# ssi-research/FQSS

Measured on AMD Instinct MI355X. Metric: QAT-step samples/sec + SI-SDR, ConvTasNet 2spk 8kHz W8A8, higher is better.
Workload: dtype f32

## Files before the change

fqss_amd/_lib.py:

```python
import ctypes as C
import os

_HERE = os.path.dirname(os.path.abspath(__file__))
SO_PATH = os.environ.get("FQSS_LIB") or os.path.join(_HERE, "csrc", "libfqss_hip.so")

P, I64, I32, F32, F64 = C.c_void_p, C.c_int64, C.c_int, C.c_float, C.c_double

_PROTOS = {
    "fqss_version": [],
    "fqss_last_error": [],
    "fqss_selftest_div": [P, I64, F32, P, P],
    "fqss_actq_fwd": [P, P, P, I64, I64, I64, I64, I64, I32, P, I32, P, P, P, P],
    "fqss_obs_reset": [P, I64, P],
    "fqss_observer_ema": [P, P, P, F64, P],
    "fqss_actq_bwd": [P, P, P, I64, I64, I64, I64, I64, I32, P, I32, P, P, P, P, I64, P],
    "fqss_gluq_fwd": [P, P, I64, I64, I64, I64, I64, I32, P, P, P, P],
    "fqss_gluq_bwd": [P, P, P, I64, I64, I64, I64, I64, I64, I32, P, P, P, P],
    "fqss_actq_bwd_colbias": [P, P, P, I64, I32, I64, I64, I64, I32, P, I32, P, P, P, P, P],
    "fqss_actq2_bwd_colbias": [P, P, P, I64, I32, I64, I64, I64, P, P, P, P, P, P, P, P],
    "fqss_minmax": [P, I64, I64, I64, P, P],
    "fqss_wq_observe": [P, I64, I64, I64, P, P, P],
    "fqss_wq_fwd": [P, P, P, I64, I64, I64, P, P, P],
    "fqss_wq_bwd": [P, P, P, P, P, I64, I64, I64, P, P, I32, P],
    "fqss_gacc_flush": [P, P, P, P, P],
    "fqss_gacc_flush_multi": [P, I32, P],
    "fqss_wq_multi_fwd": [P, I32, I32, P],
    "fqss_wq_multi_bwd": [P, I32, I32, P],
    "fqss_pwconv_fwd": [P, P, P, P, I32, I32, I32, I32, I64, I64, P],
    "fqss_pwconv_fwd_x3": [P, P, P, P, I32, I32, I32, I32, I64, I64, P],
    "fqss_pwconv_fwd_x3s": [P, P, P, P, I32, I32, I32, I32, I64, I64, P],
    "fqss_pwconv_fwd_wq": [P, P, P, P, P, I32, I32, I32, I32, I64, I64, P],
    "fqss_conv1d_s1_fwd": [P, P, P, P, I32, I32, I32, I32, I32, I32, I32, I32, I64, I64, I64, P],
    "fqss_conv1d_s1_bwd_w": [P, P, P, I32, I32, I32, I32, I32, I32, I32, I32, I64, I64, P],
    "fqss_halo_pack": [P, P, I64, I64, I64, I64, I64, I64, I64, I32, I32, I64, I64, P],
    "fqss_phase_pack": [P, P, I64, I64, I64, I64, I64, I64, I64, I32, I32, I32, I64, I64, P],
    "fqss_phase_unpack": [P, P, I64, I64, I64, I64, I64, I64, I64, I32, I32, I32, I64, I64, I64, I32, P, P],
    "fqss_conv2_fwd_wq": [P, P, P, P, P, I32, I32, I32, I32, I32, I32, I32, I32, I64, I64, I64, P],
    "fqss_conv2_fwd_x3s": [P, P, P, P, I32, I32, I32, I32, I32, I32, I32, I32, I64, I64, I64, P],
    "fqss_conv2_bwd_x_wq": [P, P, P, P, I32, I32, I32, I32, I32, I32, I32, I32, I64, I64, I64, P],
    "fqss_conv2_bwd_w": [P, P, P, I32, I32, I32, I32, I32, I32, I32, I32, I64, I64, P],
    "fqss_pwconv_bwd_x": [P, P, P, I32, I32, I32, I32, I64, I64, P],
    "fqss_pwconv_bwd_w": [P, P, P, I32, I32, I32, I32, I64, I64, P],
    "fqss_wq_codes": [P, P, P, P, P, I32, I32, P, P, P],
    "fqss_qpw_fwd": [P, P, P, P, P, P, P, P, I32, I32, I32, I32, I64, I64, P],
    "fqss_qpw_bwd_x": [P, P, P, P, I32, I32, I32, I32, I64, I64, P],
    "fqss_qpw_bwd_x_add": [P, P, P, P, P, I32, I32, I32, I32, I64, I64, I64, P],
    "fqss_qpw_bwd_w": [P, P, P, P, P, I32, I32, I32, I32, I64, I64, P],
    "fqss_qpw_fwdq": [P, P, P, P, P, P, P, P, P, P, I32, P, P, P, P, P, P, P, I32, I32, I32, I32, I32, I64, I64, I64, I64, I64, P, P],
    "fqss_qpw_fwdq_add": [P, P, P, P, P, P, P, P, P, P, P, P, P, P, P, P, I32, I32, I32, I32, I32, I64, I64, I64, I64, I64, P, P, P],
    "fqss_add_chain_ok": [I64, I64, I32, I32],
    "fqss_add_chain_bwd": [P, I32, P, I64, P, I64, P, I64, P, I64, P, P, I64, I64, I32, I64, I64, I64, I64, P],
    "fqss_qpw_stat_slots": [I32, I32],
    "fqss_dwq_stat_slots": [I32, I32],
    "fqss_qpw_fwd2": [P, P, P, P, P, P, P, P, P, P, I32, I32, I32, I32, I32, I64, I64, I64, P],
    "fqss_qpw_bwd_x2": [P, P, P, P, P, I32, I32, I32, I32, I32, I64, I64, I64, P],
    "fqss_qpw_bwd_w2": [P, P, P, P, P, P, I32, I32, I32, I32, I32, I64, I64, I64, P],
    "fqss_qpw_bwd_w_group_ws": [P, I32],
    "fqss_qpw_bwd_w_group": [P, I32, P, I64, P],
    "fqss_decode": [P, P, I64, I64, I64, I64, P, P, P],
    "fqss_gnq_fwd": [P, P, P, P, P, P, P, P, I32, I32, I32, I64, I64, I64, F32, P, P, P, P, I32, P],
    "fqss_gnq_bwd": [P, P, P, P, P, P, P, P, P, P, I32, I32, I32, I64, I64, I64, P, P, P, P, P],
    "fqss_ewq_bwd_p": [P, P, P, P, P, P, F32, P, P, I64, I64, I64, I64, I64, I64, I32, P, P, P, P, I32,
                       P, I64, I32, P, P, P, P, I64, P, I64, I32, P, P, P, P, I64, P],
    "fqss_gnq_bwd_p": [P, P, P, P, P, P, P, P, P, P, I32, I32, I32, I64, I64, I64, P, P, P, P, P, I64, I32, P, P, P, P],
    "fqss_dwq_fwd": [P, P, P, P, P, P, P, I32, I32, I32, I32, I32, I32, I64, I64, I64, I32, P, P, P, P, P],
    "fqss_dwq_bwd_z": [P, P, P, P, P, P, P, I32, I32, I32, I32, I32, I32, I64, I64, I64, I32, P, P, P, P, P, P],
    "fqss_ewq_fwd": [P, P, P, P, P, P, P, F32, P, P, I64, I64, I64, I64, I64, I64, I64, I32, P, P, P, P],
    "fqss_ewq_bwd": [P, P, P, P, P, P, P, F32, P, P, I64, I64, I64, I64, I64, I64, I64, I32, P, P, P, P, P],
    "fqss_dwq_bwd_w": [P, P, P, P, P, I32, I32, I32, I32, I32, I32, I64, I64, P],
    "fqss_mulq_fwd": [P, P, P, P, P, P, P, P, I32, I32, I32, I32, I64, I64, I64, I64, P, P, P],
    "fqss_mulq_bwd": [P, P, P, P, P, P, P, P, P, I32, I32, I32, I32, I64, I64, I64, I64, I64, P, P, P, P, I64, I32, P, P, P, P],
    "fqss_dwq_bwd": [P, P, P, P, P, P, P, P, I32, I32, I32, I32, I32, I32, I64, I64, I64, I32, P, P, P, P, P, P],
    "fqss_dwq_bwd_gn": [P, P, P, P, P, P, P, P, I32, I32, I32, I32, I32, I32, I64, I64, I64, I32, P, P, P, P, P, P, P, P],
    "fqss_gnq_bwd_rows": [P, P, P, P, P, P, P, I32, I32, I32, I64, I64, P, P, P, P, P],
    "fqss_gnq_bwd_apply": [P, P, P, P, P, P, P, P, P, P, I32, I32, I32, I64, I64, I64, P, P, P, P, I64, I32, P, P, P, P],
    "fqss_split3_planes": [P, P, I64, P],
    "fqss_tgemm": [P, P, I32, I32, I32, I32, I64, I32, P, P, P, F32, P, P, I32, P, P, I32, P, P, I64, P, P, I64, P],
    "fqss_tgemm_tiled": [P, P, I32, I32, I32, I32, I64, I32, P, P, P, F32, P, P, I32, P, P, I32, P, P, I64, P, P, I64, P],
    "fqss_tgemm_tiled_ok": [I32, I32, I32],
    "fqss_split3_tiles": [P, P, I32, I32, P],
    "fqss_bn_moments": [P, P, I32, I32, I32, I64, P],
    "fqss_bn_apply": [P, P, P, P, I32, I32, I32, I64, I64, P],
    "fqss_bn_bwd_reduce": [P, P, P, I32, I32, I32, I64, I64, P],
    "fqss_bn_bwd_apply": [P, P, P, P, P, P, I32, I32, I32, I64, I64, I64, P],
    "fqss_tdw": [P, P, P, P, F32, P, P, P, P, P, I32, I32, I32, I32, I32, I32, I64, I64, P],
    "fqss_tstats": [P, I32, I32, I32, I64, P, P],
    "fqss_dwconv_fwd": [P, P, P, P, I32, I32, I32, I32, I32, I32, I64, I64, P],
    "fqss_dwconv_bwd_x": [P, P, P, I32, I32, I32, I32, I32, I32, I64, I64, P],
    "fqss_dwconv_bwd_w": [P, P, P, I32, I32, I32, I32, I32, I32, I64, I64, P],
    "fqss_gn_fwd": [P, P, P, P, P, I32, I32, I32, I64, I64, F32, P, P],
    "fqss_gn_fwd_tail": [P, P, P, P, I32, I32, I32, I64, I64, F32, P, I32, P, P, I64, P],
    "fqss_gn_bwd": [P, P, P, P, P, P, P, I32, I32, I32, I64, I64, I64, P, P],
    "fqss_gnq_fwd_f": [P, P, P, P, P, P, I32, I32, I32, I64, I64, I64, F32, P, P, P, P],
    "fqss_gnq_bwd_f": [P, P, P, P, P, P, P, P, I32, I32, I32, I64, I64, I64, P, P, P, P, P],
    "fqss_axpby": [P, P, F32, F32, P, I64, I64, I64, I64, I64, P],
    "fqss_mul_bcast_fwd": [P, P, P, I32, I32, I32, I32, I64, I64, I64, P],
    "fqss_mul_bcast_bwd": [P, P, P, P, P, I32, I32, I32, I32, I64, I64, I64, I64, I64, P],
    "fqss_splitter2": [P, P, I32, I64, P, P],
    "fqss_splitter2_raw": [P, P, I32, I64, P, P],
    "fqss_frames_conv_fwd": [P, P, P, I32, I32, I32, I64, I32, I32, I32, I64, P],
    "fqss_frames_conv_add_fwd": [P, P, P, I64, P, I32, I32, I32, I64, I32, I32, I32, I64, P],
    "fqss_ola_convtr_fwd": [P, P, P, I32, I32, I32, I64, I32, I32, I64, P],
    "fqss_frames_wgrad1": [P, P, P, I32, I32, I32, I64, I64, I32, I32, P],
    "fqss_frames_wgrad1s": [P, P, I64, P, I64, I32, I32, I32, I64, I64, I32, I32, P],
    "fqss_frames_wgrad1_q": [P, P, P, P, P, I32, I32, I32, I64, I64, I32, I32, P],
    "fqss_ola_convtr_fwd_q": [P, P, P, P, P, I32, I32, I32, I64, I32, I32, I64, P],
    "fqss_ola_convtr_mul_fwd": [P, P, P, P, I32, I32, I32, I32, I64, I64, I32, I32, I64, P],
    "fqss_frames_wgrad": [P, P, P, I32, I32, I32, I32, I64, I64, I32, I32, P],
    "fqss_kd_loss": [P, P, P, I32, I64, F32, P, P, P, P, P, P],
    "fqss_kd_moments": [P, P, P, I32, I64, P, P],
    "fqss_pit_sisdr_loss": [P, P, I32, I64, P, P, P, P, P, P],
    "fqss_kd_loss_per_sample": [P, P, P, I32, I64, F32, I32, F32, P, P, P, P, P, P],
    "fqss_sumsq": [P, I64, P, P],
    "fqss_set_deterministic": [I32, P, I64, P],
    "fqss_det_finish": [P, I64, P, P],
    "fqss_adam_clip": [P, P, P, P, I64, P, F32, F32, F32, F32, F32, F32, P, P, P, P],
    "fqss_rowlin_fwd": [P, P, P, P, I64, I32, I32, I64, I64, I64, P],
    "fqss_rowlin_fwd_w3": [P, P, P, P, I64, I32, I32, I64, I64, P],
    "fqss_rowlin_bwd_x": [P, P, P, I64, I32, I32, I64, I64, I64, P],
    "fqss_rowlin_bwd_w": [P, P, P, I64, I32, I32, I64, I64, I64, P],
    "fqss_rowlin_bwd_w_batched": [P, P, P, I64, I32, I32, I64, I64, I64, I32, I64, I64, I64, P],
    "fqss_colsum": [P, P, I64, I32, I64, P],
    "fqss_layernorm_fwd": [P, P, P, P, P, I64, I32, I64, I64, F64, P],
    "fqss_layernorm_bwd": [P, P, P, P, P, P, P, I64, I32, I64, I64, I64, P],
    "fqss_layernormq_fwd": [P, P, P, P, P, P, I64, I32, I64, I64, I64, F64, P, P, P],
    "fqss_layernormq_bwd": [P, P, P, P, P, P, P, P, I64, I32, I64, I64, I64, P, P, P, P],
    "fqss_unary_fwd": [P, P, I64, I32, F64, P],
    "fqss_unary_rows_fwd": [P, P, I64, I32, I64, I64, I32, F64, P],
    "fqss_unary2_fwd": [P, P, I64, I32, F64, F64, P],
    "fqss_unary_bwd": [P, P, P, I64, I32, F64, P],
    "fqss_permute4": [P, P, I64, I64, I64, I32, I64, I64, I64, P],
    "fqss_permute4_ld": [P, P, I64, I64, I64, I32, I64, I64, I64, I64, P],
    "fqss_dp_segment_fwd": [P, P, I32, I32, I64, I64, I32, I32, P],
    "fqss_dp_segment_bwd": [P, P, I32, I32, I64, I64, I32, I32, P],
    "fqss_dp_merge_fwd": [P, P, P, I32, I32, I32, I32, I32, I64, I64, P],
    "fqss_dp_merge_bwd": [P, P, P, I32, I32, I32, I32, I32, I64, I64, I64, P],
    "fqss_ola2_fwd": [P, P, I64, I64, I64, P],
    "fqss_ola2_bwd": [P, P, I64, I64, I64, P],
    "fqss_attn_fwd": [P, P, P, P, P, I32, I32, I32, I32, I64, I64, I64, I64, P, P, P],
    "fqss_attn_bwd": [P, P, P, P, P, P, P, P, P, I32, I32, I32, I32, I64, I64, I64, I64, I64, I64, I64, I64, P],
    "fqss_add_layernorm_fwd": [P, P, P, P, P, P, P, P, I64, I32, I64, I64, I64, I64, I64, F64, P, P, P],
    "fqss_add_layernorm_bwd": [P, P, P, P, P, P, P, P, P, I64, I32, I64, I64, I64, I64, P, P, P, P],
    "fqss_addq_layernorm_fwd": [P, P, P, P, P, P, P, P, I64, I32, I64, I64, I64, I64, I64, F64, P, P, P, P, P],
    "fqss_addq_layernorm_bwd": [P, P, P, P, P, P, P, P, P, I64, I32, I64, I64, I64, I64, P, P, P, P, P, P, P],
    "fqss_addq_layernorm_fwd_map": [P, P, P, P, P, P, P, P, I64, I32, I64, I64, I64, F64, P, P, P, P, I64, I64, I64, I64, I64, P],
    "fqss_addq_layernorm_bwd_map": [P, P, P, P, P, P, P, P, I64, I32, I64, I64, P, P, P, P, P, P, I64, I64, I64, I64, I64, P],
    "fqss_mha_prep_fwd": [P, P, P, P, I64, I32, I64, F64, P, P],
    "fqss_mha_prep_fwd_c": [P, P, P, P, I64, I32, I64, F64, P, P],
    "fqss_mha_prep_bwd": [P, P, P, P, P, I64, I32, I64, I64, F64, P, P, P],
    "fqss_lstm_fwd": [P, P, P, P, P, P, I32, I32, I32, P],
    "fqss_lstm_bwd": [P, P, P, P, P, I32, I32, I32, P],
    "fqss_lstm_gate_fn": [P, P, P, I64, P],
    "fqss_lstm_bwd_b": [P, P, P, P, P, P, I32, I32, I32, P],
    "fqss_lstm_bwd_b4": [P, P, P, P, P, P, I32, I32, I32, P],
    "fqss_gnrows_fwd": [P, P, P, P, P, P, I64, I32, I64, I64, I32, I32, I32, F64, P],
    "fqss_gnrows_bwd": [P, P, P, P, P, P, P, P, I64, I32, I64, I64, I64, I32, I32, I32, P],
    "fqss_bcast_add": [P, P, P, I64, I64, I32, P],
    "fqss_bcast_sum": [P, P, I64, I64, I32, P],
# ... 184 lines not shown
```

fqss_amd/csrc/desc_api.hip:

```cpp
#include <cstring>

#include "fqss_dev.h"

using namespace fqss;

namespace {

struct Rows {
    void* p;
    int64_t B, C, M, ld;
};

bool rows3(const FqssTensor* t, int dtype, Rows& r, const char*& why) {
    if (t == nullptr || t->data == nullptr) { why = "null tensor"; return false; }
    if (t->dtype != dtype) { why = "wrong dtype"; return false; }
    if (t->ndim < 2 || t->ndim > 3) { why = "tensor must be [B][C][M] or [rows][cols]"; return false; }
    const int n = t->ndim;
    if (t->stride[n - 1] != 1) { why = "innermost stride must be 1"; return false; }
    for (int i = 0; i < n; ++i)
        if (t->shape[i] < 0) { why = "negative extent"; return false; }
    r.p = t->data;
    r.M = t->shape[n - 1];
    r.C = t->shape[n - 2];
    r.B = n == 3 ? t->shape[0] : 1;
// ... 38 lines not shown
}

extern "C" int fqss_add_fq_fwd(const FqssTensor* a, const FqssQParams* qa, const FqssTensor* b, const FqssQParams* qb, float sb,
                               FqssTensor* y, FqssTensor* y_out, const FqssQParams* q, void* ws, size_t ws_bytes,
                               fqss_stream_t stream) {
    (void)ws; (void)ws_bytes;
    FQSS_REQUIRE(qa && q && qa->qmin && qa->qmax && q->qmin && q->qmax, "null quantizer");
    DESC_ROWS(ra, a, FQSS_DT_U8);
    DESC_ROWS(ry, y, FQSS_DT_U8);
    FQSS_REQUIRE(same_shape(ra, ry), "a / y shapes differ");
    Rows rb{}, ro{};
    const bool b_codes = b != nullptr && b->dtype == FQSS_DT_U8;
    if (b != nullptr) {
        DESC_ROWS(rb_, b, b_codes ? FQSS_DT_U8 : FQSS_DT_F32);
        FQSS_REQUIRE(same_shape(ra, rb_), "a / b shapes differ");
        FQSS_REQUIRE(!b_codes || (qb && qb->qmin && qb->qmax), "coded b needs its quantizer");
        rb = rb_;
    }
    if (y_out != nullptr) {
        DESC_ROWS(ro_, y_out, FQSS_DT_F32);
        FQSS_REQUIRE(same_shape(ra, ro_), "a / y_out shapes differ");
        ro = ro_;
    }
    return fqss_ewq_fwd((const uint8_t*)ra.p, qa->qmin, qa->qmax, b_codes ? (const uint8_t*)rb.p : nullptr, b_codes ? qb->qmin : nullptr,
                        b_codes ? qb->qmax : nullptr, (b != nullptr && !b_codes) ? (const float*)rb.p : nullptr, sb, (uint8_t*)ry.p,
                        (float*)ro.p, ra.B * ra.C, ra.M, ra.ld, rb.ld, rb.ld, ry.ld, ro.ld, q->act, q->slope, q->qmin, q->qmax, stream);
}

extern "C" int fqss_add_fq_bwd(const FqssTensor* a, const FqssQParams* qa, const FqssTensor* b, const FqssQParams* qb, float sb,
                               const FqssTensor* g, FqssTensor* gz, const FqssQParams* q, const FqssProducer* pa, const FqssProducer* pb,
                               void* ws, size_t ws_bytes, fqss_stream_t stream) {
    (void)ws; (void)ws_bytes;
    FQSS_REQUIRE(qa && q && qa->qmin && qa->qmax && q->qmin && q->qmax && q->gacc, "null quantizer / gacc");
    DESC_ROWS(ra, a, FQSS_DT_U8);
    DESC_ROWS(rg, g, FQSS_DT_F32);
    FQSS_REQUIRE(same_shape(ra, rg), "a / g shapes differ");
    Rows rb{}, rz{};
    const bool b_codes = b != nullptr && b->dtype == FQSS_DT_U8;
    if (b != nullptr) {
        DESC_ROWS(rb_, b, b_codes ? FQSS_DT_U8 : FQSS_DT_F32);
        FQSS_REQUIRE(same_shape(ra, rb_), "a / b shapes differ");
        FQSS_REQUIRE(!b_codes || (qb && qb->qmin && qb->qmax), "coded b needs its quantizer");
        rb = rb_;
    }
    if (gz != nullptr) {
        DESC_ROWS(rz_, gz, FQSS_DT_F32);
        FQSS_REQUIRE(same_shape(ra, rz_), "a / gz shapes differ");
        rz = rz_;
    }
    if (pa == nullptr && pb == nullptr) {
        FQSS_REQUIRE(gz != nullptr, "gz missing");
        return fqss_ewq_bwd((const uint8_t*)ra.p, qa->qmin, qa->qmax, b_codes ? (const uint8_t*)rb.p : nullptr, b_codes ? qb->qmin : nullptr,
                            b_codes ? qb->qmax : nullptr, (b != nullptr && !b_codes) ? (const float*)rb.p : nullptr, sb, (const float*)rg.p,
                            (float*)rz.p, ra.B * ra.C, ra.M, ra.ld, rb.ld, rb.ld, rg.ld, rz.ld, q->act, q->slope, q->qmin, q->qmax, q->gacc,
                            stream);
    }
    FQSS_REQUIRE(b == nullptr || b_codes, "fused producers need a coded (or absent) b");
    Rows pz[2] = {{}, {}}, po[2] = {{}, {}};
    const FqssProducer* ps[2] = {pa, pb};
    for (int i = 0; i < 2; ++i) {
        if (ps[i] == nullptr) continue;
        FQSS_REQUIRE(ps[i]->gacc != nullptr, "producer gacc missing");
        DESC_ROWS(z_, ps[i]->z, FQSS_DT_F32);
        DESC_ROWS(o_, ps[i]->out, FQSS_DT_F32);
        FQSS_REQUIRE(same_shape(ra, z_) && same_shape(ra, o_), "producer shapes differ from a");
        pz[i] = z_;
        po[i] = o_;
    }
    FQSS_REQUIRE(gz != nullptr || (pa != nullptr && (b == nullptr || pb != nullptr)), "gz may only be NULL when every operand is fused");
    return fqss_ewq_bwd_p((const uint8_t*)ra.p, qa->qmin, qa->qmax, b_codes ? (const uint8_t*)rb.p : nullptr, b_codes ? qb->qmin : nullptr,
                          b_codes ? qb->qmax : nullptr, sb, (const float*)rg.p, (float*)rz.p, ra.B * ra.C, ra.M, ra.ld, rb.ld, rg.ld, rz.ld,
                          q->act, q->slope, q->qmin, q->qmax, q->gacc, (int)ra.C, (const float*)pz[0].p, pz[0].ld, pa ? pa->act : 0,
                          pa ? pa->slope : nullptr, pa ? pa->gacc : nullptr, pa ? pa->gbias : nullptr, (float*)po[0].p, po[0].ld,
                          (const float*)pz[1].p, pz[1].ld, pb ? pb->act : 0, pb ? pb->slope : nullptr, pb ? pb->gacc : nullptr,
                          pb ? pb->gbias : nullptr, (float*)po[1].p, po[1].ld, stream);
}

extern "C" int fqss_pwconv_fq_fwd(const FqssTensor* x, const FqssQParams* qx, const FqssWCodes* w, const float* bias1, const float* bias2,
                                  FqssTensor* z1, FqssTensor* z2, FqssTensor* y1, FqssTensor* y2, const FqssQParams* q1,
                                  const FqssQParams* q2, void* ws, size_t ws_bytes, fqss_stream_t stream) {
    FQSS_REQUIRE(qx && qx->qmin && qx->qmax && q1 && q1->qmin && q1->qmax, "null quantizer");
    FQSS_REQUIRE(w && w->idx && w->dw && w->rw && w->Co > 0 && w->Ci > 0, "null weight codes");
    DESC_ROWS(rx, x, FQSS_DT_U8);
    DESC_ROWS(rz1, z1, FQSS_DT_F32);
    DESC_ROWS(ry1, y1, FQSS_DT_U8);
    FQSS_REQUIRE(rx.C == w->Ci, "x channels != Ci");
    FQSS_REQUIRE(rz1.B == rx.B && rz1.M == rx.M && same_shape(rz1, ry1), "z1 / y1 shapes");
    const int Co1 = (int)rz1.C;
    int Co2 = 0;
    Rows rz2{}, ry2{};
    if (z2 != nullptr || y2 != nullptr) {
        FQSS_REQUIRE(z2 && y2 && q2 && q2->qmin && q2->qmax, "second layer: z2, y2 and q2 all needed");
        DESC_ROWS(rz2_, z2, FQSS_DT_F32);
        DESC_ROWS(ry2_, y2, FQSS_DT_U8);
        FQSS_REQUIRE(rz2_.B == rx.B && rz2_.M == rx.M && same_shape(rz2_, ry2_), "z2 / y2 shapes");
        rz2 = rz2_;
        ry2 = ry2_;
        Co2 = (int)rz2.C;
    }
    FQSS_REQUIRE(Co1 + Co2 == w->Co, "z1 + z2 channels != Co of the weight codes");
    int64_t* stats = nullptr;
    if (ws != nullptr && Co2 == 0) {
        const int64_t need = ws_bytes_of("pwconv_fq_fwd", rx.B, Co1, rx.M);
        if (need > 0) {
            FQSS_REQUIRE((int64_t)ws_bytes >= need, "workspace smaller than fqss_workspace_bytes(\"pwconv_fq_fwd\")");
            stats = (int64_t*)ws;
        }
    }
    return fqss_qpw_fwdq((const uint8_t*)rx.p, w->idx, w->dw, w->rw, bias1, bias2, qx->qmin, qx->qmax, (float*)rz1.p, (float*)rz2.p, q1->act,
                         q1->slope, q1->qmin, q1->qmax, Co2 ? q2->qmin : nullptr, Co2 ? q2->qmax : nullptr, (uint8_t*)ry1.p, (uint8_t*)ry2.p,
                         (int)rx.B, w->Ci, Co1, Co2, (int)rx.M, rx.ld, rz1.ld, rz2.ld, ry1.ld, ry2.ld, stats, stream);
}

extern "C" int fqss_gln_fq_fwd(const FqssTensor* x, const FqssQParams* qx, const float* gamma, const float* beta, float eps, FqssTensor* y,
                               FqssTensor* y_out, float* mean_rstd, const FqssQParams* q, void* ws, size_t ws_bytes, const int64_t* stats,
                               int nslots, fqss_stream_t stream) {
    FQSS_REQUIRE(qx && qx->qmin && qx->qmax && q && q->qmin && q->qmax && gamma && beta && mean_rstd, "null argument");
    DESC_ROWS(rx, x, FQSS_DT_U8);
    DESC_ROWS(ry, y, FQSS_DT_U8);
    FQSS_REQUIRE(same_shape(rx, ry), "x / y shapes differ");
    Rows ro{};
    if (y_out != nullptr) {
        DESC_ROWS(ro_, y_out, FQSS_DT_F32);
        FQSS_REQUIRE(same_shape(rx, ro_), "x / y_out shapes differ");
        ro = ro_;
    }
    if (stats == nullptr)
        FQSS_REQUIRE(ws != nullptr && (int64_t)ws_bytes >= ws_bytes_of("gln_fq_fwd", rx.B, rx.C, rx.M),
                     "workspace smaller than fqss_workspace_bytes(\"gln_fq_fwd\")");
    return fqss_gnq_fwd((const uint8_t*)rx.p, qx->qmin, qx->qmax, gamma, beta, (uint8_t*)ry.p, (float*)ro.p, mean_rstd, (int)rx.B, (int)rx.C,
                        (int)rx.M, rx.ld, ry.ld, ro.ld, eps, q->qmin, q->qmax, ws, stats, nslots, stream);
}

extern "C" int fqss_tgemm_desc(const FqssTGemmDesc* d, fqss_stream_t stream) {
    FQSS_REQUIRE(d && d->planes && d->planes->data && d->planes->dtype == FQSS_DT_U16 && d->planes->ndim == 3 && d->planes->shape[0] == 3,
                 "planes must be a [3][Co][Ci] u16 tensor");
    const int Co = (int)d->planes->shape[1], Ci = (int)d->planes->shape[2];
    FQSS_REQUIRE(d->planes->stride[2] == 1 && d->planes->stride[1] == Ci && d->planes->stride[0] == (int64_t)Co * Ci, "planes must be dense");
    DESC_ROWS(rx, d->x, FQSS_DT_F32);
    FQSS_REQUIRE(rx.C == Ci, "x channels != Ci");
    DESC_ROWS(c1, d->c1, FQSS_DT_F32);
    FQSS_REQUIRE(c1.B == rx.B && c1.M == rx.M && c1.C == (d->M1 < Co ? d->M1 : Co), "c1 shape");
    Rows c2{}, r1{}, r2{};
    if (d->M1 < Co) {
        DESC_ROWS(c2_, d->c2, FQSS_DT_F32);
        FQSS_REQUIRE(c2_.B == rx.B && c2_.M == rx.M && c2_.C == Co - d->M1, "c2 shape");
        c2 = c2_;
    }
    if (d->r1 != nullptr) {
        DESC_ROWS(r1_, d->r1, FQSS_DT_F32);
        FQSS_REQUIRE(same_shape(r1_, c1) && r1_.ld == c1.ld, "r1 must have the layout of c1");
        r1 = r1_;
    }
    if (d->r2 != nullptr) {
        DESC_ROWS(r2_, d->r2, FQSS_DT_F32);
        FQSS_REQUIRE(same_shape(r2_, c2) && r2_.ld == c2.ld, "r2 must have the layout of c2");
        r2 = r2_;
    }
    return fqss_tgemm((const uint16_t*)d->planes->data, (const float*)rx.p, (int)rx.B, Ci, Co, (int)rx.M, rx.ld, d->pro, d->pro_stats,
                      d->pro_gamma, d->pro_beta, d->pro_eps, d->pro_slope, d->bias, d->act, d->slope, d->stats_out, d->M1, (float*)c1.p,
                      (const float*)r1.p, c1.ld, (float*)c2.p, (const float*)r2.p, c2.ld, stream);
}
```

fqss_amd/csrc/fqss_dev.h:

```cpp
#pragma once
#include <hip/hip_runtime.h>
#include <stdint.h>

#include "fqss.h"

namespace fqss {

void set_error(const char* fmt, ...);
int launch_status(const char* what);

#define FQSS_REQUIRE(cond, msg)                          \
    do {                                                 \
        if (!(cond)) {                                   \
            ::fqss::set_error("%s: %s", __func__, msg);  \
            return FQSS_EINVAL;                          \
        }                                                \
    } while (0)

static inline bool aligned16(const void* p) { return (reinterpret_cast<uintptr_t>(p) & 15u) == 0; }
static inline int64_t cdiv(int64_t a, int64_t b) { return (a + b - 1) / b; }

static inline dim3 grid_rows(int64_t rows, int64_t cols, int vec, int64_t max_blocks = 8192) {
    int64_t gx = cdiv(cols, 256 * (int64_t)vec);
    if (gx < 1) gx = 1;
// ... 119 lines not shown
            v[i] = s;
        }
    }
    __syncthreads();
}

template <int N>
__device__ __forceinline__ void block_sum_f32w(const float (&p)[N], float* smem, double (&out)[N]) {
    const int lane = threadIdx.x & 63, w = threadIdx.x >> 6, nw = blockDim.x >> 6;
#pragma unroll
    for (int i = 0; i < N; ++i) {
        const float s = wave_sum63(p[i]);
        if (lane == 63) smem[i * nw + w] = s;
    }
    __syncthreads();
    if (threadIdx.x == 0) {
#pragma unroll
        for (int i = 0; i < N; ++i) {
            double s = (double)smem[i * nw];
            for (int k = 1; k < nw; ++k) s += (double)smem[i * nw + k];
            out[i] = s;
        }
    }
    __syncthreads();
}

struct QRange {
    float lo, delta, inv;
};
__device__ __forceinline__ QRange load_qrange(const float* qmin, const float* qmax) {
    const float lo = *qmin, hi = *qmax;
    QRange r;
    r.lo = lo;
    r.delta = (hi - lo) / 255.0f;
    r.inv = 1.0f / r.delta;
    return r;
}
__device__ __forceinline__ float div_by(float a, float b, float y) {
    const float q = a * y;
    const float r = fmaf(-b, q, a);
    return fmaf(r, y, q);
}
template <typename T>
__device__ __forceinline__ T sgpr(T v) {
    asm("" : "+s"(v));
    return v;
}
__device__ __forceinline__ void store16(float* p, const float4& v) {
    typedef float f32x4s __attribute__((ext_vector_type(4)));
    const f32x4s t = {v.x, v.y, v.z, v.w};
    asm volatile("global_store_dwordx4 %0, %1, off\n\ts_nop 1" : : "v"(p), "v"(t) : "memory");
}
__device__ __forceinline__ float act_neg_scale(int act, float slope) {
    return act == FQSS_ACT_PRELU ? slope : (act == FQSS_ACT_RELU ? 0.0f : 1.0f);
}
__device__ __forceinline__ float act_apply(float z, int act, float slope) {
    return z > 0.0f ? z : act_neg_scale(act, slope) * z;
}
__device__ __forceinline__ float act_bwd(float z, float gt, int act, float slope, bool valid, float& p_slope) {
    const bool neg = !(z > 0.0f);
    p_slope += (act == FQSS_ACT_PRELU && valid && neg) ? z * gt : 0.0f;
    return neg ? act_neg_scale(act, slope) * gt : gt;
}
__device__ __forceinline__ float act_apply_br(float z, int act, float slope) {
    if (act == FQSS_ACT_PRELU) return z > 0.0f ? z : slope * z;
    if (act == FQSS_ACT_RELU) return z > 0.0f ? z : 0.0f;
    return z;
}
__device__ __forceinline__ float act_bwd_br(float z, float gt, int act, float slope, bool valid, float& p_slope) {
    if (act == FQSS_ACT_PRELU) {
        const bool pos = z > 0.0f;
        if (valid && !pos) p_slope += z * gt;
        return pos ? gt : slope * gt;
    }
    if (act == FQSS_ACT_RELU) return (z > 0.0f) ? gt : 0.0f;
    return gt;
}
__device__ __forceinline__ float fq_asym(float t, const QRange& r, float& c, float& u, bool& inr) {
    u = div_by(t - r.lo, r.delta, r.inv);
    const float X = rintf(u);
    inr = (X >= 0.0f) && (X <= 255.0f);
    c = __builtin_amdgcn_fmed3f(X, 0.0f, 255.0f);
    return r.delta * c + r.lo;
}

__device__ __forceinline__ float fq_code(float t, const QRange& r) {
    return __builtin_amdgcn_fmed3f(rintf(div_by(t - r.lo, r.delta, r.inv)), 0.0f, 255.0f);
}
__device__ __forceinline__ unsigned int pack_code(float c, unsigned int byte, unsigned int word) {
    return __builtin_amdgcn_cvt_pk_u8_f32(c, byte, word);
}
__device__ __forceinline__ void code_stats4(unsigned int word, unsigned int& s, unsigned int& ss) {
    s = __builtin_amdgcn_udot4(word, 0x01010101u, s, false);
    ss = __builtin_amdgcn_udot4(word, word, ss, false);
}

#endif

constexpr int kDetSlots = 3;
struct DetCtl { long long* shadow[kDetSlots]; const float* base[kDetSlots]; long long n[kDetSlots]; };
typedef int (*det_setter_t)(const DetCtl*);
void det_register(det_setter_t fn);
#if defined(__HIPCC__) && defined(FQSS_USES_GRAD_ADD)
static __constant__ DetCtl d_det_ctl;
namespace {
struct DetRegistrar {
    DetRegistrar() {
        det_register([](const DetCtl* c) { return (int)hipMemcpyToSymbol(HIP_SYMBOL(d_det_ctl), c, sizeof(DetCtl)); });
    }
} det_registrar_;
}
__device__ __forceinline__ bool det_preload() { return d_det_ctl.shadow[0] != nullptr; }
__device__ __forceinline__ void grad_add(float* addr, float v);
__device__ __forceinline__ void grad_add(float* addr, float v, bool det_on) {
    if (det_on) grad_add(addr, v);
    else atomicAdd(addr, v);
}
__device__ __forceinline__ void grad_add(float* addr, float v) {
    if (d_det_ctl.shadow[0] != nullptr && fabsf(v) < 0x1p33f) {
        const DetCtl c = d_det_ctl;
#pragma unroll
        for (int s = 0; s < kDetSlots; ++s) {
            long long* const sh = c.shadow[s];
            const long long i = addr - c.base[s];
            if (sh != nullptr && (unsigned long long)i < (unsigned long long)c.n[s]) {
                const double dv = (double)v;
                const long long hi = __double2ll_rn(dv * 0x1p30);
                const long long lo = __double2ll_rn((dv - (double)hi * 0x1p-30) * 0x1p80);
                if (hi != 0) atomicAdd(reinterpret_cast<unsigned long long*>(sh + 2 * i), (unsigned long long)hi);
                if (lo != 0) atomicAdd(reinterpret_cast<unsigned long long*>(sh + 2 * i + 1), (unsigned long long)lo);
                return;
            }
        }
    }
    atomicAdd(addr, v);
}
#endif
}
```

fqss_amd/csrc/fused_q.hip:

```cpp
#include <cstdlib>
#include <type_traits>

#define FQSS_USES_GRAD_ADD
#include "fqss_dev.h"

namespace fqss {

constexpr int kGnSlots = 64;
constexpr int kSlots = FQSS_GACC_SLOTS;

__device__ __forceinline__ float dec(unsigned int c, const QRange& r) { return r.delta * (float)c + r.lo; }
__device__ __forceinline__ void dec4(unsigned int w, const QRange& r, float (&v)[4]) {
    v[0] = dec(w & 255u, r);
    v[1] = dec((w >> 8) & 255u, r);
    v[2] = dec((w >> 16) & 255u, r);
    v[3] = dec(w >> 24, r);
}

__global__ __launch_bounds__(256) void k_decode(const uint8_t* __restrict__ c, float* __restrict__ out, int64_t rows,
                                                 int64_t cols, int64_t ld_c, int64_t ld_o, const float* qmin,
                                                 const float* qmax) {
    const QRange r = load_qrange(qmin, qmax);
    const int64_t cstep = (int64_t)gridDim.x * 256 * 4;
    for (int64_t row = blockIdx.y; row < rows; row += gridDim.y)
// ... 85 lines not shown
        const float scale = rstd * gamma[c];
        const float shift = fmaf(-scale, mean, beta[c]);
        for (int c0 = c_first; c0 < M; c0 += cstep) {
            const uint4 v = (c0 == c_first) ? v0 : *reinterpret_cast<const uint4*>(xr + c0);
            const unsigned int w[4] = {v.x, v.y, v.z, v.w};
            unsigned int o[4];
#pragma unroll
            for (int q = 0; q < 4; ++q) {
                float xv[4], cq[4];
                dec4(w[q], rx, xv);
                unsigned int pk = 0;
#pragma unroll
                for (int e = 0; e < 4; ++e) {
                    cq[e] = fq_code(fmaf(xv[e], scale, shift), ry);
                    pk = pack_code(cq[e], e, pk);
                }
                o[q] = pk;
                if (yout != nullptr && c0 + 4 * q < M)
                    *reinterpret_cast<float4*>(yout + (int64_t)row * ld_o + c0 + 4 * q) =
                        make_float4(ry.delta * cq[0] + ry.lo, ry.delta * cq[1] + ry.lo, ry.delta * cq[2] + ry.lo, ry.delta * cq[3] + ry.lo);
            }
            *reinterpret_cast<uint4*>(yc + (int64_t)row * ld_yc + c0) = make_uint4(o[0], o[1], o[2], o[3]);
        }
    }
}

template <int RPW>
__global__ __launch_bounds__(256) void k_gnq_apply_t(const uint8_t* __restrict__ xc, const float* __restrict__ gamma,
                                                      const float* __restrict__ beta, uint8_t* __restrict__ yc,
                                                      float* __restrict__ yout, float* __restrict__ mean_rstd,
                                                      const long long* __restrict__ ws, int nslots, float eps, int B, int C,
                                                      int M, int64_t ld_xc, int64_t ld_yc, int64_t ld_o, const float* qmin_x,
                                                      const float* qmax_x, const float* qmin, const float* qmax) {
    __shared__ long long red[2 * 4];
    __shared__ float mr[2];
    __shared__ __attribute__((aligned(16))) uint8_t tab[RPW][256];
    const QRange rx = load_qrange(qmin_x, qmax_x), ry = load_qrange(qmin, qmax);
    const int row0 = blockIdx.x * RPW;
    const int b = row0 / C, c0 = row0 - b * C;
    const int m_first = threadIdx.x * 16;
    uint4 v0[RPW];
#pragma unroll
    for (int r = 0; r < RPW; ++r) {
        v0[r] = make_uint4(0, 0, 0, 0);
        if (m_first < M) v0[r] = *reinterpret_cast<const uint4*>(xc + (int64_t)(row0 + r) * ld_xc + m_first);
    }
    gnq_sample_stats(ws, nslots, b, (int64_t)C * M, eps, rx, red, mr);
    if (c0 == 0 && threadIdx.x == 0) {
        mean_rstd[2 * b] = mr[0];
        mean_rstd[2 * b + 1] = mr[1];
    }
    const float mean = mr[0], rstd = mr[1];
    const float xt = dec(threadIdx.x, rx);
#pragma unroll
    for (int r = 0; r < RPW; ++r) {
        const float scale = rstd * gamma[c0 + r];
        const float shift = fmaf(-scale, mean, beta[c0 + r]);
        tab[r][threadIdx.x] = (uint8_t)fq_code(fmaf(xt, scale, shift), ry);
    }
    __syncthreads();
#pragma unroll
    for (int r = 0; r < RPW; ++r) {
        const uint8_t* xr = xc + (int64_t)(row0 + r) * ld_xc;
        uint8_t* yr = yc + (int64_t)(row0 + r) * ld_yc;
        for (int m = m_first; m < M; m += 4096) {
            const uint4 v = (m == m_first) ? v0[r] : *reinterpret_cast<const uint4*>(xr + m);
            const unsigned int w[4] = {v.x, v.y, v.z, v.w};
            unsigned int o[4];
#pragma unroll
            for (int q = 0; q < 4; ++q) {
                const unsigned int t0 = tab[r][w[q] & 255u], t1 = tab[r][(w[q] >> 8) & 255u], t2 = tab[r][(w[q] >> 16) & 255u],
                                   t3 = tab[r][w[q] >> 24];
                o[q] = t0 | (t1 << 8) | (t2 << 16) | (t3 << 24);
                if (yout != nullptr && m + 4 * q < M)
                    *reinterpret_cast<float4*>(yout + (int64_t)(row0 + r) * ld_o + m + 4 * q) =
                        make_float4(ry.delta * (float)t0 + ry.lo, ry.delta * (float)t1 + ry.lo, ry.delta * (float)t2 + ry.lo,
                                    ry.delta * (float)t3 + ry.lo);
            }
            *reinterpret_cast<uint4*>(yr + m) = make_uint4(o[0], o[1], o[2], o[3]);
        }
    }
}

__device__ __forceinline__ void gn_coef_from_sums(const double (&sv)[2], float mean, float rstd, int C, int M, double& c2d, double& c3d) {
    const double md = (double)mean, rd = (double)rstd;
    const double inv_n = 1.0 / ((double)C * (double)M);
    c2d = (sv[1] * md - sv[0]) * rd * rd * rd * inv_n;
    c3d = -c2d * md - sv[1] * rd * inv_n;
}

__global__ __launch_bounds__(256) void k_gnq_bwd_rows(const uint8_t* __restrict__ xc, const float* __restrict__ g,
                                                       const float* __restrict__ gamma, const float* __restrict__ beta,
                                                       const float* __restrict__ mean_rstd, int C, int M, int64_t ld_xc,
                                                       int64_t ld_g, double* ws, const float* qmin_x, const float* qmax_x,
                                                       const float* qmin, const float* qmax, double* gacc) {
    __shared__ float redf[4 * 4];
    const QRange rx = load_qrange(qmin_x, qmax_x), ry = load_qrange(qmin, qmax);
    const int b = blockIdx.y, c = blockIdx.x;
    const int64_t row = (int64_t)b * C + c;
    const float mean = mean_rstd[2 * b], rstd = mean_rstd[2 * b + 1];
    const float scale = rstd * gamma[c];
    const float shift = fmaf(-scale, mean, beta[c]);
    const uint8_t* xr = xc + row * ld_xc;
    const float* gr = g + row * ld_g;
    float ds = 0.f, db = 0.f, p_du = 0.f, p_out = 0.f;
    for (int m0 = threadIdx.x * 4; m0 < M; m0 += 4096) {
        unsigned int wq_[4];
        float4 gq[4];
#pragma unroll
        for (int i = 0; i < 4; ++i) {
            const int m = m0 + 1024 * i;
            if (m < M) {
                wq_[i] = *reinterpret_cast<const unsigned int*>(xr + m);
                gq[i] = *reinterpret_cast<const float4*>(gr + m);
            }
        }
#pragma unroll
        for (int i = 0; i < 4; ++i) {
            const int m = m0 + 1024 * i;
            if (m >= M) break;
            const unsigned int w = wq_[i];
            const float gv[4] = {gq[i].x, gq[i].y, gq[i].z, gq[i].w};
#pragma unroll
            for (int e = 0; e < 4; ++e) {
                if (m + e < M) {
                    const float x = dec((w >> (8 * e)) & 255u, rx);
                    const float z = fmaf(x, scale, shift);
                    float cq, u;
                    bool inr;
                    (void)fq_asym(z, ry, cq, u, inr);
                    const float gz = inr ? div_by(gv[e] * ry.delta, ry.delta, ry.inv) : 0.0f;
                    p_du += gv[e] * (inr ? (cq - u) : cq);
                    p_out += inr ? 0.0f : gv[e];
                    ds = fmaf(gz, x, ds);
                    db += gz;
                }
            }
        }
    }
    double v[4];
    {
        const float pf[4] = {ds, db, p_du, p_out};
        block_sum_f32w<4>(pf, redf, v);
    }
    if (threadIdx.x == 0) {
        ws[2 * row] = v[0];
        ws[2 * row + 1] = v[1];
        double* slot = gacc + 3 * (row % kSlots);
        const double dmax = v[2] / 255.0;
        atomicAdd(&slot[0], v[3] - dmax);
        atomicAdd(&slot[1], dmax);
    }
}

struct GnProducer {
    const float* pz; int64_t ld_pz;
    int act; const float* slope;
    const float *qmin, *qmax;
    double* gacc; float* gbias;
};

template <bool FUSE>
__global__ __launch_bounds__(256) void k_gnq_bwd_apply(const uint8_t* __restrict__ xc, const float* __restrict__ g,
                                                        const float* __restrict__ gamma, const float* __restrict__ beta,
                                                        const float* __restrict__ mean_rstd, float* __restrict__ gx, int B,
                                                        int C, int M, int64_t ld_xc, int64_t ld_g, int64_t ld_gx,
                                                        const double* ws, const float* qmin_x, const float* qmax_x,
                                                        const float* qmin, const float* qmax, GnProducer P, float* ggamma,
                                                        float* gbeta) {
    __shared__ float predf[4 * 4];
    const bool det_on = det_preload();
    const QRange rp = FUSE ? load_qrange(P.qmin, P.qmax) : QRange{0.f, 1.f, 1.f};
    const float pslope = (FUSE && P.act == FQSS_ACT_PRELU) ? *P.slope : 0.0f;
    float p_du = 0.f, p_out = 0.f, p_slope = 0.f, p_bias = 0.f;
    const QRange rx = load_qrange(qmin_x, qmax_x), ry = load_qrange(qmin, qmax);
    const int c = blockIdx.x, b = blockIdx.y;
    const int64_t row = (int64_t)b * C + c;
    const float mean = mean_rstd[2 * b], rstd = mean_rstd[2 * b + 1];
    const float scale = rstd * gamma[c];
    const float shift = fmaf(-scale, mean, beta[c]);
    __shared__ double cred[2 * 4];
    __shared__ float c23[2];
    float c2, c3;
    auto gamma_beta_grads = [&]() {
        double gg = 0.0, gb = 0.0;
        for (int bb = 0; bb < B; ++bb) {
            const double ds = ws[2 * ((int64_t)bb * C + c)], db = ws[2 * ((int64_t)bb * C + c) + 1];
            gg += (ds - db * (double)mean_rstd[2 * bb]) * (double)mean_rstd[2 * bb + 1];
            gb += db;
        }
        ggamma[c] += (float)gg;
        gbeta[c] += (float)gb;
    };
    {
        double sv[2] = {0.0, 0.0};
        for (int cc = threadIdx.x; cc < C; cc += 256) {
            const double gmm = (double)gamma[cc];
            sv[0] += gmm * ws[2 * ((int64_t)b * C + cc)];
            sv[1] += gmm * ws[2 * ((int64_t)b * C + cc) + 1];
        }
        block_sum<double, 2>(sv, cred);
        if (threadIdx.x == 0) {
            double c2d, c3d;
            gn_coef_from_sums(sv, mean, rstd, C, M, c2d, c3d);
            c23[0] = (float)c2d;
            c23[1] = (float)c3d;
            if (b == 0) gamma_beta_grads();
        }
        __syncthreads();
        c2 = c23[0];
        c3 = c23[1];
    }
    const uint8_t* xr = xc + row * ld_xc;
    const float* gr = g + row * ld_g;
    const float* pzr = FUSE ? P.pz + row * P.ld_pz : nullptr;
    float* orow = gx + row * ld_gx;
    for (int m0 = threadIdx.x * 4; m0 < M; m0 += 4096) {
        unsigned int wq_[4];
        float4 gq[4], pq[4];
#pragma unroll
        for (int i = 0; i < 4; ++i) {
            const int m = m0 + 1024 * i;
            if (m < M) {
                wq_[i] = *reinterpret_cast<const unsigned int*>(xr + m);
                gq[i] = *reinterpret_cast<const float4*>(gr + m);
                if (FUSE) pq[i] = *reinterpret_cast<const float4*>(pzr + m);
            }
        }
#pragma unroll
        for (int i = 0; i < 4; ++i) {
            const int m = m0 + 1024 * i;
            if (m >= M) break;
            const float gv[4] = {gq[i].x, gq[i].y, gq[i].z, gq[i].w};
            const float pzv[4] = {FUSE ? pq[i].x : 0.f, FUSE ? pq[i].y : 0.f, FUSE ? pq[i].z : 0.f, FUSE ? pq[i].w : 0.f};
            float xv[4], o[4];
            dec4(wq_[i], rx, xv);
#pragma unroll
            for (int e = 0; e < 4; ++e) {
                const float x = xv[e];
                const float z = fmaf(x, scale, shift);
                float cq, u;
                bool inr;
                (void)fq_asym(z, ry, cq, u, inr);
                const float gz = inr ? div_by(gv[e] * ry.delta, ry.delta, ry.inv) : 0.0f;
                o[e] = fmaf(gz, scale, fmaf(x, c2, c3));
                if (FUSE) {
                    const bool valid = (m + e < M);
                    const float gj = valid ? o[e] : 0.0f;
                    const float t = act_apply(pzv[e], P.act, pslope);
                    float pc, pu;
                    bool pin;
                    (void)fq_asym(t, rp, pc, pu, pin);
                    const float gt = pin ? div_by(gj * rp.delta, rp.delta, rp.inv) : 0.0f;
                    p_du += gj * (pin ? (pc - pu) : pc);
                    p_out += pin ? 0.0f : gj;
                    const float gzj = act_bwd(pzv[e], gt, P.act, pslope, valid, p_slope);
                    o[e] = gzj;
                    p_bias += valid ? gzj : 0.0f;
                }
            }
            *reinterpret_cast<float4*>(orow + m) = make_float4(o[0], o[1], o[2], o[3]);
        }
    }
    if (FUSE) {
        double v[4];
        {
            const float pf[4] = {p_du, p_out, p_slope, p_bias};
            block_sum_f32w<4>(pf, predf, v);
        }
        if (threadIdx.x == 0 && P.gbias != nullptr) grad_add(&P.gbias[c], (float)v[3], det_on);
        if (threadIdx.x == 0) {
            double* slot = P.gacc + 3 * (row % kSlots);
            const double dmax = v[0] / 255.0;
            atomicAdd(&slot[0], v[1] - dmax);
            atomicAdd(&slot[1], dmax);
            if (P.act == FQSS_ACT_PRELU) atomicAdd(&slot[2], v[2]);
        }
    }
}

constexpr int kTaps = 8;

__device__ __forceinline__ unsigned int load_codes4(const uint8_t* __restrict__ xr, int s0, int ld) {
    const int a0 = s0 & ~3;
    const unsigned int sh = (unsigned int)(s0 - a0);
    const unsigned int lo = (a0 >= 0 && a0 < ld) ? *reinterpret_cast<const unsigned int*>(xr + a0) : 0u;
    if (sh == 0) return lo;
    const unsigned int hi = (a0 + 4 >= 0 && a0 + 4 < ld) ? *reinterpret_cast<const unsigned int*>(xr + a0 + 4) : 0u;
    return __builtin_amdgcn_alignbyte(hi, lo, sh);
}

__device__ __forceinline__ unsigned int load_codes4_clamped(const uint8_t* __restrict__ xr, int s0, int M) {
    unsigned int w = 0;
#pragma unroll
    for (int j = 0; j < 4; ++j) {
        const int p = min(max(s0 + j, 0), M - 1);
        w |= (unsigned int)xr[p] << (8 * j);
    }
    return w;
}

__device__ __forceinline__ unsigned int load_codes4_unaligned(const uint8_t* __restrict__ p) {
    unsigned int w;
    __builtin_memcpy(&w, p, 4);
    return w;
}

__device__ __forceinline__ void dwq_z4(const uint8_t* __restrict__ xr, int m, int M, int ld_c, const float* wk, int K,
                                        int dil, int pad, float bv, const QRange& rx, float (&z)[4]) {
    float acc[4] = {0.f, 0.f, 0.f, 0.f};
    if (m - pad >= 0 && m + 3 + pad < M) {
#pragma unroll
        for (int k = 0; k < kTaps; ++k) {
            if (k < K) {
                float v[4];
                dec4(load_codes4_unaligned(xr + (m + k * dil - pad)), rx, v);
#pragma unroll
                for (int j = 0; j < 4; ++j) acc[j] = fmaf(wk[k], v[j], acc[j]);
            }
        }
    } else {
        unsigned int wv[kTaps];
#pragma unroll
        for (int k = 0; k < kTaps; ++k)
            if (k < K) wv[k] = load_codes4_clamped(xr, m + k * dil - pad, M);
#pragma unroll
        for (int k = 0; k < kTaps; ++k) {
            if (k < K) {
                const int s0 = m + k * dil - pad;
                float v[4];
#pragma unroll
                for (int j = 0; j < 4; ++j) v[j] = (s0 + j >= 0 && s0 + j < M) ? dec((wv[k] >> (8 * j)) & 255u, rx) : 0.0f;
#pragma unroll
                for (int j = 0; j < 4; ++j) acc[j] = fmaf(wk[k], v[j], acc[j]);
            }
        }
    }
#pragma unroll
    for (int j = 0; j < 4; ++j) z[j] = acc[j] + bv;
}

template <int KT>
__global__ __launch_bounds__(256) void k_dwq_fwd(const uint8_t* __restrict__ xc, const float* __restrict__ w,
// ... 1446 lines not shown
```

fqss_amd/csrc/qgemm.hip:

```cpp
#include <cstdlib>
#include <type_traits>

#define FQSS_USES_GRAD_ADD
#include "fqss_dev.h"

namespace fqss {

typedef float f32x16 __attribute__((ext_vector_type(16)));
typedef __bf16 bf16x8 __attribute__((ext_vector_type(8)));
typedef short s16x4 __attribute__((ext_vector_type(4)));
typedef short s16x8 __attribute__((ext_vector_type(8)));

constexpr int QBM = 128, QBN = 64, QBK = 32;
constexpr int LDK = 40;
constexpr int LDN = 96;
constexpr int LDT = 36;
constexpr int WGRAD_BLOCKS = 256;

__device__ __forceinline__ unsigned short f2bf_trunc(float f) { return (unsigned short)(__float_as_uint(f) >> 16); }
__device__ __forceinline__ float bf_trunc(float f) { return __uint_as_float(__float_as_uint(f) & 0xFFFF0000u); }
__device__ __forceinline__ unsigned int bf_rne_word(float f) {
    const unsigned int u = __float_as_uint(f);
    return u + 0x7FFFu + ((u >> 16) & 1u);
}

__device__ __forceinline__ void split3(float g, unsigned short& b1, unsigned short& b2, unsigned short& b3) {
    const float h1 = bf_trunc(g);
    const float r1 = g - h1;
    const float h2 = bf_trunc(r1);
    const float r2 = r1 - h2;
    b1 = f2bf_trunc(h1);
    b2 = f2bf_trunc(h2);
    b3 = f2bf_trunc(r2);
}

typedef float f32x4 __attribute__((ext_vector_type(4)));
typedef uint32_t u32x4 __attribute__((ext_vector_type(4)));
typedef uint32_t u32x2 __attribute__((ext_vector_type(2)));
struct QStage {
    f32x4 a[4];
    f32x4 b[2];
    u32x2 bq;
    int kch;
};
__device__ __forceinline__ void q_load16(f32x4& d, const void* p) { asm volatile("global_load_dwordx4 %0, %1, off" : "=v"(d) : "v"(p) : "memory"); }
__device__ __forceinline__ void q_load8(u32x2& d, const void* p) { asm volatile("global_load_dwordx2 %0, %1, off" : "=v"(d) : "v"(p) : "memory"); }
template <int MODE, int N>
__device__ __forceinline__ void q_wait(QStage& st) {
    if constexpr (MODE == 0)
        asm volatile("s_waitcnt vmcnt(%2)" : "+v"(st.a[0]), "+v"(st.bq) : "n"(N) : "memory");
    else if constexpr (MODE == 1)
        asm volatile("s_waitcnt vmcnt(%3)" : "+v"(st.a[0]), "+v"(st.b[0]), "+v"(st.b[1]) : "n"(N) : "memory");
    else
        asm volatile("s_waitcnt vmcnt(%6)"
                     : "+v"(st.a[0]), "+v"(st.a[1]), "+v"(st.a[2]), "+v"(st.a[3]), "+v"(st.b[0]), "+v"(st.b[1])
                     : "n"(N)
                     : "memory");
}

__device__ __forceinline__ float dec(unsigned int c, const QRange& r) { return r.delta * (float)c + r.lo; }

struct QGemmArgs {
    const void* A;
    const void* B;
    float* C;
    int M, N, K;
    int64_t lda, ldb, ldc;
    int64_t sAb, sBb, sCb;
    const float* dw;
    const float* rw;
    const float* bias;
    const float* qmin_x;
    const float* qmax_x;
    int ksplit, kchunk;
    int tiles_m, tiles_n, batches;
    int M1;
    float* C2; int64_t ldc2, sC2b;
    const float* bias2;
    const void* A2; int64_t lda2, sA2b;
    int K1;
    const void* B2; int64_t ldb2, sB2b;
    unsigned char* Q1; unsigned char* Q2; int64_t ldq1, ldq2, sQ1b, sQ2b;
    const float *qy_min1, *qy_max1, *qy_min2, *qy_max2;
    int qact; const float* qslope;
    long long* stats;
    const unsigned char* AD1; const unsigned char* AD2; int64_t ldad1, ldad2;
    unsigned char* S1; unsigned char* S2; int64_t lds1, lds2;
    const float *ad_min1, *ad_max1, *ad_min2, *ad_max2;
    const float *s_min1, *s_max1, *s_min2, *s_max2;
    int imp_taps, imp_kw, imp_base, imp_row_step, imp_col_step, imp_cmax;
    float imp_inv_taps, imp_inv_kw;
};

template <int MODE, int GP = 3, bool IMP = false>
__global__ __launch_bounds__(256, 2) void k_qgemm(QGemmArgs g) {
    static_assert(!IMP || MODE == 1 || MODE == 3 || MODE == 4, "implicit convolution: float B operands");
    static_assert(MODE == 0 || MODE == 1 || MODE == 3 || MODE == 4, "unknown q-GEMM mode");
    static_assert(GP == 3 || (GP == 2 && MODE != 0 && MODE != 4), "two gradient pieces: dgrad only");
    constexpr bool ACODES = MODE < 2 || MODE == 4;
    constexpr int WMODE = MODE == 4 ? 1 : MODE;
    constexpr bool SIX = MODE == 3 && GP == 2;
    constexpr int NA = (MODE == 3) ? 3 : 1;
    constexpr int NB = (MODE == 1) ? GP : (MODE == 3 || MODE == 4) ? 3 : 1;
    constexpr int BROWS = QBK, BLD = LDN;
    constexpr int A_BYTES = NA * QBM * LDK * 2, B_BYTES = NB * BROWS * BLD * 2;
    constexpr int T_BYTES = 4 * 32 * LDT * 4;
    constexpr int SMEM = (A_BYTES + B_BYTES > T_BYTES) ? A_BYTES + B_BYTES : T_BYTES;
    __shared__ __attribute__((aligned(16))) unsigned char smem[SMEM];
    typedef unsigned short (*AsT)[QBM][LDK];
    typedef unsigned short (*BsT)[BROWS][BLD];
    AsT As = reinterpret_cast<AsT>(smem);
    BsT Bs = reinterpret_cast<BsT>(smem + A_BYTES);

    const int tid = threadIdx.x, lane = tid & 63;
    const int wave = __builtin_amdgcn_readfirstlane(tid >> 6);
    const int wm = wave >> 1, wn = wave & 1;
    const int lr = lane & 31, lh = lane >> 5;
    int panel, mt;
    if (!xcd_tile(g.tiles_n * g.batches, g.tiles_m, panel, mt)) return;
    const int b = panel / g.tiles_n;
    const int kbeg = 0, kend = g.K;
    const int i0 = mt * QBM, j0 = (panel % g.tiles_n) * QBN;

    f32x16 acc[2];
#pragma unroll
    for (int mi = 0; mi < 2; ++mi)
#pragma unroll
        for (int r = 0; r < 16; ++r) acc[mi][r] = 0.f;

    __shared__ float rowc[3][QBM];
    if constexpr (MODE == 0 || MODE == 3 || MODE == 4) {
        if (tid < QBM) {
            const int row = i0 + tid;
            const bool ok = row < g.M;
            rowc[0][tid] = ((MODE == 0 || MODE == 4) && ok) ? g.dw[row] : 1.0f;
            rowc[1][tid] = (MODE == 0 && ok) ? g.rw[row] : 0.0f;
            rowc[2][tid] = (ok && g.bias != nullptr) ? (row < g.M1 ? g.bias[row] : g.bias2[row - g.M1]) : 0.0f;
        }
    }

    constexpr int NLOADS = (MODE == 0) ? 2 : (WMODE == 1) ? 3 : 6;
    const int a_row = tid >> 1, a_k = (tid & 1) * 16;
    const int bk_row = tid >> 3, bk_n = (tid & 7) * 8;
    const int a_row_c = min(i0 + a_row, g.M - 1);

    __shared__ float dws[(MODE == 1) ? 1024 : 1];
    if constexpr (MODE == 1) {
        for (int k = tid; k < (IMP ? g.K / g.imp_taps : g.K); k += 256) dws[k] = g.dw[k];
    }

    constexpr int BEL = (MODE == 0) ? 1 : 4;
    const char* const gB1 = sgpr((const char*)g.B + (int64_t)b * g.sBb * BEL);
    const char* const gB2 = (MODE == 0) ? gB1 : sgpr((const char*)g.B2 + (int64_t)b * g.sB2b * BEL);
    const int64_t gldb1 = sgpr(g.ldb), gldb2 = (MODE == 0) ? gldb1 : sgpr(g.ldb2);
    auto load_tiles = [&](QStage& st, int k0) {
        if constexpr (ACODES) {
            q_load16(st.a[0], (const signed char*)g.A + (int64_t)a_row_c * g.lda + min(k0 + a_k, g.K - 16));
        } else {
            const float* A = (const float*)g.A + (int64_t)b * g.sAb + (int64_t)a_row_c * g.lda;
#pragma unroll
            for (int q = 0; q < 4; ++q) q_load16(st.a[q], A + min(k0 + a_k + 4 * q, g.K - 4));
        }
        const int kk = min(k0 + bk_row, g.K - 1);
        if constexpr (IMP) {
            int ci = (int)((float)kk * g.imp_inv_taps);
            int t = kk - ci * g.imp_taps;
            if (t < 0) { ci -= 1; t += g.imp_taps; }
            if (t >= g.imp_taps) { ci += 1; t -= g.imp_taps; }
            int th = (int)((float)t * g.imp_inv_kw);
            int tw = t - th * g.imp_kw;
            if (tw < 0) { th -= 1; tw += g.imp_kw; }
            if (tw >= g.imp_kw) { th += 1; tw -= g.imp_kw; }
            st.kch = ci;
            const float* Bp = (const float*)gB1 + (int64_t)ci * gldb1 + (g.imp_base + th * g.imp_row_step + tw * g.imp_col_step);
            const int c0 = min(j0 + bk_n, g.imp_cmax);
            q_load16(st.b[0], Bp + c0);
            q_load16(st.b[1], Bp + c0 + 4);
        } else if constexpr (MODE == 0) {
            const unsigned char* Bp = (const unsigned char*)gB1 + (int64_t)kk * gldb1;
            q_load8(st.bq, Bp + min(j0 + bk_n, (int)gldb1 - 8));
        } else {
            const bool h1 = kk < g.K1;
            const int ldk = (int)(h1 ? gldb1 : gldb2);
            const float* Bp = (const float*)(h1 ? gB1 : gB2) + (int64_t)(h1 ? kk : kk - g.K1) * ldk;
            q_load16(st.b[0], Bp + min(j0 + bk_n, ldk - 4));
            q_load16(st.b[1], Bp + min(j0 + bk_n + 4, ldk - 4));
        }
    };

    auto store_codes = [&](unsigned short* dst, const unsigned int* w, auto nw_tag, bool is_signed, bool zero) {
        constexpr int NW = decltype(nw_tag)::value;
        unsigned int o[2 * NW];
#pragma unroll
        for (int q = 0; q < NW; ++q) {
            float f[4];
#pragma unroll
            for (int e = 0; e < 4; ++e) {
                const unsigned int byte = (w[q] >> (8 * e)) & 0xFFu;
                f[e] = zero ? 0.0f : (is_signed ? (float)(int)(signed char)byte : (float)byte);
            }
            o[2 * q] = __builtin_amdgcn_perm(__float_as_uint(f[1]), __float_as_uint(f[0]), 0x07060302u);
            o[2 * q + 1] = __builtin_amdgcn_perm(__float_as_uint(f[3]), __float_as_uint(f[2]), 0x07060302u);
        }
#pragma unroll
        for (int h = 0; h < NW / 2; ++h)
            *reinterpret_cast<uint4*>(dst + 8 * h) = make_uint4(o[4 * h], o[4 * h + 1], o[4 * h + 2], o[4 * h + 3]);
    };

    auto store_split3 = [&](unsigned short* d1, unsigned short* d2, unsigned short* d3, const f32x4* v, float scale,
                            bool do_scale, bool zero, auto nq_tag) {
        constexpr int NQ = decltype(nq_tag)::value;
        unsigned int o1[2 * NQ], o2[2 * NQ], o3[2 * NQ];
#pragma unroll
        for (int q = 0; q < NQ; ++q) {
            float h0[4], r1[4], r2[4];
#pragma unroll
            for (int e = 0; e < 4; ++e) {
                float t = do_scale ? scale * v[q][e] : v[q][e];
                if (zero) t = 0.0f;
                h0[e] = t;
                r1[e] = t - bf_trunc(t);
                r2[e] = r1[e] - bf_trunc(r1[e]);
// ... 34 lines not shown
        }
        *reinterpret_cast<uint4*>(d1) = make_uint4(o1[0], o1[1], o1[2], o1[3]);
        *reinterpret_cast<uint4*>(d2) = make_uint4(o2[0], o2[1], o2[2], o2[3]);
    };

    auto store_tiles = [&](QStage& st, int k0) {
        q_wait<WMODE, NLOADS>(st);
        const bool kz = (k0 + bk_row) >= g.K;
        if constexpr (ACODES) {
            const unsigned int w[4] = {__float_as_uint(st.a[0][0]), __float_as_uint(st.a[0][1]), __float_as_uint(st.a[0][2]),
                                       __float_as_uint(st.a[0][3])};
            store_codes(&As[0][a_row][a_k], w, std::integral_constant<int, 4>{}, true, false);
        } else {
            store_split3(&As[0][a_row][a_k], &As[1][a_row][a_k], &As[2][a_row][a_k], st.a, 1.0f, false, false,
                         std::integral_constant<int, 4>{});
        }
        if constexpr (MODE == 0) {
            const unsigned int w[2] = {st.bq[0], st.bq[1]};
            store_codes(&Bs[0][bk_row][bk_n], w, std::integral_constant<int, 2>{}, false, kz);
        } else {
            const float sc = (MODE == 1) ? dws[IMP ? st.kch : min(k0 + bk_row, g.K - 1)] : 1.0f;
            if constexpr (NB == 2)
                store_split2(&Bs[0][bk_row][bk_n], &Bs[1][bk_row][bk_n], st.b, sc, kz);
            else
                store_split3(&Bs[0][bk_row][bk_n], &Bs[1][bk_row][bk_n], &Bs[2][bk_row][bk_n], st.b, sc, MODE == 1, kz,
                             std::integral_constant<int, 2>{});
        }
    };

    const int nkt = (kend - kbeg + QBK - 1) / QBK;
    const int gq = lane >> 4, li = lane & 15, tq = li >> 2, tp = li & 3;
    auto compute_tile = [&]() {
#pragma unroll
        for (int ks = 0; ks < 2; ++ks) {
#pragma unroll
            for (int sp = 0; sp < NA * NB; ++sp) {
                const int ia = (NA == 3) ? 2 - (sp / NB) : 0, ib = (NB > 1) ? NB - 1 - (sp % NB) : 0;
                if (SIX && ia + ib >= 3) continue;
                bf16x8 af[2], bfr;
#pragma unroll
                for (int mi = 0; mi < 2; ++mi)
                    af[mi] = *reinterpret_cast<const bf16x8*>(&As[ia][wm * 64 + mi * 32 + lr][ks * 16 + 8 * lh]);
                {
                    const int kr = ks * 16 + 8 * (gq >> 1) + tq;
                    const int nc = wn * 32 + 16 * (gq & 1) + 4 * tp;
                    union { bf16x8 v; s16x4 h[2]; } u;
                    u.h[0] = __builtin_amdgcn_ds_read_tr16_b64_v4i16(
                        (s16x4 __attribute__((address_space(3)))*)(&Bs[ib][kr][nc]));
                    u.h[1] = __builtin_amdgcn_ds_read_tr16_b64_v4i16(
                        (s16x4 __attribute__((address_space(3)))*)(&Bs[ib][kr + 4][nc]));
                    bfr = u.v;
                }
#pragma unroll
                for (int mi = 0; mi < 2; ++mi)
                    acc[mi] = __builtin_amdgcn_mfma_f32_32x32x16_bf16(af[mi], bfr, acc[mi], 0, 0, 0);
            }
        }
    };
    QStage stA, stB;
    __syncthreads();
    load_tiles(stA, 0);
    load_tiles(stB, QBK);
    store_tiles(stA, 0);
    load_tiles(stA, 2 * QBK);
    __syncthreads();
    for (int kt = 0; kt < nkt; kt += 2) {
        compute_tile();
        __syncthreads();
        if (kt + 1 < nkt) {
            store_tiles(stB, (kt + 1) * QBK);
            load_tiles(stB, (kt + 3) * QBK);
            __syncthreads();
            compute_tile();
            __syncthreads();
            if (kt + 2 < nkt) {
                store_tiles(stA, (kt + 2) * QBK);
                load_tiles(stA, (kt + 4) * QBK);
                __syncthreads();
            }
        }
    }
    q_wait<WMODE, 0>(stA);
    q_wait<WMODE, 0>(stB);

    float dx = 0.f, mnx = 0.f;
    if constexpr (MODE == 0) {
        const float lo = *g.qmin_x, hi = *g.qmax_x;
        dx = (hi - lo) / 255.0f;
        mnx = lo;
    }
    float* Cb = g.C + (int64_t)b * g.sCb;
    float* C2b = (g.C2 != nullptr) ? g.C2 + (int64_t)b * g.sC2b : nullptr;
    __shared__ uint32_t Qt[(MODE == 0) ? 4 : 1][32][8];
    const bool quant = (MODE == 0) && g.Q1 != nullptr;
    unsigned int st_s = 0, st_ss = 0;
    QRange ry1{}, ry2{};
    QRange rad1{}, rad2{}, rs1{}, rs2{};
    float qslope = 0.0f;
    if (quant) {
        ry1 = load_qrange(g.qy_min1, g.qy_max1);
        ry2 = (g.Q2 != nullptr) ? load_qrange(g.qy_min2, g.qy_max2) : ry1;
        qslope = (g.qact == FQSS_ACT_PRELU) ? *g.qslope : 0.0f;
        if (g.S1 != nullptr) { rad1 = load_qrange(g.ad_min1, g.ad_max1); rs1 = load_qrange(g.s_min1, g.s_max1); }
        if (g.S2 != nullptr) { rad2 = load_qrange(g.ad_min2, g.ad_max2); rs2 = load_qrange(g.s_min2, g.s_max2); }
    }
    {
        __syncthreads();
        float(*Tt)[LDT] = reinterpret_cast<float(*)[LDT]>(smem + wave * 32 * LDT * 4);
        const bool has_bias = g.bias != nullptr;
        const float qns = act_neg_scale(g.qact, qslope);
        const int c4 = (lane & 7) * 4;
        const int col = j0 + wn * 32 + c4;
        auto tile_epilogue = [&](int mi, auto PER_ROW) {
            const int rowt = i0 + wm * 64 + mi * 32;
            const bool tfirst = rowt < g.M1;
            uint4 ad16 = make_uint4(0u, 0u, 0u, 0u);
            const unsigned char* const adp = (MODE == 0 && quant) ? (tfirst ? g.AD1 : g.AD2) : nullptr;
            if constexpr (MODE == 0) {
                if (adp != nullptr) {
                    const int64_t ldad = tfirst ? g.ldad1 : g.ldad2;
                    const int orow = rowt + (lane >> 1) - (tfirst ? 0 : g.M1), ocol = j0 + wn * 32 + 16 * (lane & 1);
                    const int rows_o = tfirst ? g.M1 : g.M - g.M1;
                    if (rowt + (lane >> 1) < g.M && ocol < ldad)
                        ad16 = *reinterpret_cast<const uint4*>(adp + ((int64_t)b * rows_o + orow) * ldad + ocol);
                }
            }
#pragma unroll
            for (int r = 0; r < 16; ++r) {
                const int rl = (r & 3) + 8 * (r >> 2) + 4 * lh;
                const int rb = wm * 64 + mi * 32 + rl;
                const float S = acc[mi][r];
                float v = S;
                if constexpr (MODE == 0) {
                    v = rowc[0][rb] * (dx * S + mnx * rowc[1][rb]);
                    if (has_bias) v = v + rowc[2][rb];
                } else if constexpr (MODE == 3) {
                    if (has_bias) v = S + rowc[2][rb];
                } else if constexpr (MODE == 4) {
                    v = rowc[0][rb] * S;
                    if (has_bias) v = v + rowc[2][rb];
                }
                Tt[rl][lr] = v;
            }
            const QRange ry = tfirst ? ry1 : ry2;
#pragma unroll
            for (int pass = 0; pass < 4; ++pass) {
                const int rl = pass * 8 + (lane >> 3);
                const int row = rowt + rl;
                float4 t = *reinterpret_cast<const float4*>(&Tt[rl][c4]);
                if constexpr (MODE == 1) {
                    if (C2b != nullptr && row < g.M && col < g.N) {
                        const float4 r = *reinterpret_cast<const float4*>(C2b + (int64_t)row * g.ldc2 + col);
                        t.x += r.x; t.y += r.y; t.z += r.z; t.w += r.w;
                    }
                }
                if (row < g.M && col < g.N) {
                    const bool first = decltype(PER_ROW)::value ? row < g.M1 : tfirst;
                    const int64_t ldc = first ? g.ldc : g.ldc2;
                    float* dst = (first ? Cb + (int64_t)row * ldc : C2b + (int64_t)(row - g.M1) * ldc) + col;
                    if (col + 3 < g.N || col + 3 < ldc) {
                        store16(dst, t);
                    } else {
                        dst[0] = t.x;
                        if (col + 1 < g.N) dst[1] = t.y;
                        if (col + 2 < g.N) dst[2] = t.z;
                    }
                }
                if constexpr (MODE == 0) {
                    if (quant) {
                        const float tv[4] = {t.x, t.y, t.z, t.w};
                        uint32_t pk = 0;
#pragma unroll
                        for (int e = 0; e < 4; ++e) pk = pack_code(fq_code(tv[e] > 0.0f ? tv[e] : qns * tv[e], ry), e, pk);
                        Qt[wave][rl][lane & 7] = pk;
                        if (g.stats != nullptr) {
                            const int nl = g.N - col;
                            const uint32_t live = (row < g.M && nl > 0) ? (nl >= 4 ? 0xFFFFFFFFu : (0xFFFFFFFFu >> (8 * (4 - nl)))) : 0u;
                            code_stats4(pk & live, st_s, st_ss);
                        }
                    }
                }
            }
            if constexpr (MODE == 0) {
                if (quant) {
                    const int rl = lane >> 1, hf = lane & 1;
                    const int qcol = j0 + wn * 32 + 16 * hf;
                    const uint4 c16 = *reinterpret_cast<const uint4*>(&Qt[wave][rl][4 * hf]);
                    const int64_t ldq = tfirst ? g.ldq1 : g.ldq2;
                    if (rowt + rl < g.M && qcol < ldq) {
                        unsigned char* qb = tfirst ? g.Q1 + (int64_t)b * g.sQ1b + (int64_t)(rowt + rl) * ldq
                                                   : g.Q2 + (int64_t)b * g.sQ2b + (int64_t)(rowt + rl - g.M1) * ldq;
                        *reinterpret_cast<uint4*>(qb + qcol) = c16;
                    }
                    if (adp != nullptr) {
                        const QRange ra = tfirst ? rad1 : rad2, rs = tfirst ? rs1 : rs2;
                        const unsigned int wa[4] = {ad16.x, ad16.y, ad16.z, ad16.w}, wy[4] = {c16.x, c16.y, c16.z, c16.w};
                        unsigned int o[4];
#pragma unroll
                        for (int w4 = 0; w4 < 4; ++w4) {
                            unsigned int pk = 0;
#pragma unroll
                            for (int e = 0; e < 4; ++e) {
                                float z = dec((wa[w4] >> (8 * e)) & 255u, ra);
                                z = z + 1.0f * dec((wy[w4] >> (8 * e)) & 255u, ry);
                                pk = pack_code(fq_code(z, rs), e, pk);
                            }
                            o[w4] = pk;
                        }
                        const int64_t lds_ = tfirst ? g.lds1 : g.lds2;
                        const int rows_o = tfirst ? g.M1 : g.M - g.M1;
                        if (rowt + rl < g.M && qcol < lds_) {
                            unsigned char* sb_ = (tfirst ? g.S1 : g.S2) + ((int64_t)b * rows_o + (rowt + rl - (tfirst ? 0 : g.M1))) * lds_;
                            *reinterpret_cast<uint4*>(sb_ + qcol) = make_uint4(o[0], o[1], o[2], o[3]);
                        }
                    }
                }
            }
        };
        if (MODE != 0 || (g.M1 & 31) == 0 || g.M1 >= g.M) {
#pragma unroll
            for (int mi = 0; mi < 2; ++mi) tile_epilogue(mi, std::false_type{});
        } else {
#pragma unroll
            for (int mi = 0; mi < 2; ++mi) tile_epilogue(mi, std::true_type{});
        }
        if constexpr (MODE == 0) {
            if (quant && g.stats != nullptr) {
                __shared__ unsigned int sst[2][4];
                st_s = wave_sum(st_s);
                st_ss = wave_sum(st_ss);
                if (lane == 0) { sst[0][wave] = st_s; sst[1][wave] = st_ss; }
                __syncthreads();
                if (tid == 0) {
                    long long* slot = g.stats + 2 * (((int64_t)b * g.tiles_m + mt) * g.tiles_n + (panel % g.tiles_n));
                    slot[0] = (long long)sst[0][0] + sst[0][1] + sst[0][2] + sst[0][3];
                    slot[1] = (long long)sst[1][0] + sst[1][1] + sst[1][2] + sst[1][3];
                }
            }
        }
    }
}

typedef float f32x4 __attribute__((ext_vector_type(4)));
typedef uint32_t u32x4 __attribute__((ext_vector_type(4)));
__device__ __forceinline__ void wg_load16(f32x4& d, const void* p) {
    asm volatile("global_load_dwordx4 %0, %1, off" : "=v"(d) : "v"(p) : "memory");
}
__device__ __forceinline__ void wg_load16(u32x4& d, const void* p) {
    asm volatile("global_load_dwordx4 %0, %1, off" : "=v"(d) : "v"(p) : "memory");
}

constexpr int W2_TM = 64, W2_TN = 128, W2_TK = 64, W2_LD = 72, W2_RING = 4;
struct W2Stage {
    f32x4 a[2];
    u32x4 b;
};
template <int N>
__device__ __forceinline__ void w2_wait(W2Stage& st) {
    asm volatile("s_waitcnt vmcnt(%3)" : "+v"(st.a[0]), "+v"(st.a[1]), "+v"(st.b) : "n"(N) : "memory");
}

template <int GP>
__global__ __launch_bounds__(512, 1) void k_qwgrad2(QGemmArgs g) {
    __shared__ __attribute__((aligned(16))) unsigned short As[2][GP][W2_TM][W2_LD];
    __shared__ __attribute__((aligned(16))) unsigned short Bs[2][W2_TN][W2_LD];
    __shared__ float rsum[W2_TM];
    const int tid = threadIdx.x, lane = tid & 63;
    const int wave = __builtin_amdgcn_readfirstlane(tid >> 6);
    const int wr = wave >> 2, wc = wave & 3, lr = lane & 31, lh = lane >> 5;
    int slice, t;
    if (!xcd_tile(g.batches * g.ksplit, g.tiles_m * g.tiles_n, slice, t)) return;
    const int b = slice / g.ksplit, ks_id = slice % g.ksplit;
    const int kbeg = ks_id * g.kchunk, kend = min(g.K, kbeg + g.kchunk);
    const int row0 = (t / g.tiles_n) * W2_TM, col0 = (t % g.tiles_n) * W2_TN;
    const int nst = (kend - kbeg + W2_TK - 1) / W2_TK;

    const int ar = tid >> 4, ac = (tid & 15) * 4;
    const int br = tid >> 2, bc = (tid & 3) * 16;
    const float* Ap[2];
    bool aok[2];
#pragma unroll
    for (int i = 0; i < 2; ++i) {
        const int row = row0 + ar + 32 * i;
        aok[i] = row < g.M;
        const int rc = aok[i] ? row : 0;
        Ap[i] = (rc < g.M1) ? (const float*)g.A + (int64_t)b * g.sAb + (int64_t)rc * g.lda
                            : (const float*)g.A2 + (int64_t)b * g.sA2b + (int64_t)(rc - g.M1) * g.lda2;
    }
    const unsigned char* Bp = (const unsigned char*)g.B + (int64_t)b * g.sBb + (int64_t)min(col0 + br, g.N - 1) * g.ldb;
    const int ka_last = (kend - 1) & ~3, kb_last = (kend - 1) & ~15;

    auto load = [&](W2Stage& st, int s) {
        const int k = kbeg + s * W2_TK;
#pragma unroll
        for (int i = 0; i < 2; ++i) wg_load16(st.a[i], Ap[i] + min(k + ac, ka_last));
        wg_load16(st.b, Bp + min(k + bc, kb_last));
    };
    float rs_part[2] = {0.f, 0.f};
    auto convert_store = [&](W2Stage& st, int s) {
        const int buf = s & 1;
        const int k = kbeg + s * W2_TK + ac;
#pragma unroll
        for (int i = 0; i < 2; ++i) {
            float x[4];
#pragma unroll
            for (int e = 0; e < 4; ++e) x[e] = (aok[i] && k + e < kend) ? st.a[i][e] : 0.0f;
            rs_part[i] += (x[0] + x[1]) + (x[2] + x[3]);
            uint32_t o1[2], o2[2], o3[2];
#pragma unroll
            for (int e = 0; e < 2; ++e) {
                const float a0 = x[2 * e], a1 = x[2 * e + 1];
                const float r0 = a0 - bf_trunc(a0), r1 = a1 - bf_trunc(a1);
                o1[e] = __builtin_amdgcn_perm(__float_as_uint(a1), __float_as_uint(a0), 0x07060302u);
                if constexpr (GP == 3) {
                    const float s0 = r0 - bf_trunc(r0), s1 = r1 - bf_trunc(r1);
                    o2[e] = __builtin_amdgcn_perm(__float_as_uint(r1), __float_as_uint(r0), 0x07060302u);
                    o3[e] = __builtin_amdgcn_perm(__float_as_uint(s1), __float_as_uint(s0), 0x07060302u);
                } else {
                    o2[e] = __builtin_amdgcn_perm(bf_rne_word(r1), bf_rne_word(r0), 0x07060302u);
                }
            }
            const int row = ar + 32 * i;
// ... 316 lines not shown
        asm volatile("s_waitcnt vmcnt(0)" ::: "memory");
    }
    __syncthreads();
}

template <int GP>
__global__ __launch_bounds__(512, 1) void k_qwgrad_group(WGroupArgs ga) {
    __shared__ __attribute__((aligned(16))) unsigned short As_raw[2 * GP * W2_TM * W2_LD];
    __shared__ __attribute__((aligned(16))) unsigned short Bs_raw[2 * 256 * W2_LD];
    __shared__ float rsum[W2_TM];
    __shared__ unsigned ticket_s;
    const int L = blockIdx.x, xcd = L % kXcds, slot = L / kXcds;
    const int team = (slot / WGR_TEAM) * kXcds + xcd, member = slot % WGR_TEAM;
    int u0 = team * ga.chunk;
    const int u1 = min(ga.total, u0 + ga.chunk);
    while (u0 < u1) {
        int jn = 0;
        for (int q = 1; q < ga.njobs; ++q) jn = (ga.j[q].ubeg <= u0) ? q : jn;
        const WJob& J = ga.j[jn];
        const int rel = u0 - J.ubeg, grp = rel / J.nstages, s0 = rel - grp * J.nstages;
        const int n = min(J.nstages - s0, u1 - u0);
        const int g0 = J.ubeg + grp * J.nstages;
        const int t_first = g0 / ga.chunk, nparts = (g0 + J.nstages - 1) / ga.chunk - t_first + 1, part = team - t_first;
        u0 += n;
        const int tile = grp * WGR_TEAM + member;
        if (tile >= J.ntiles) continue;
        if (J.wide) wgr_segment<GP, true>(ga, J, tile, s0, n, nparts, part, As_raw, Bs_raw, rsum, &ticket_s);
        else wgr_segment<GP, false>(ga, J, tile, s0, n, nparts, part, As_raw, Bs_raw, rsum, &ticket_s);
    }
}

__global__ __launch_bounds__(256) void k_wq_codes(const float* __restrict__ w, signed char* __restrict__ idx,
                                                   signed char* __restrict__ idxT, float* dw, float* rw, int Co, int Ci,
                                                   const float* __restrict__ qmin, const float* __restrict__ qmax) {
    __shared__ float red[4];
    const int co = blockIdx.x;
    const float a = fmaxf(fabsf(qmin[co]), fabsf(qmax[co]));
    const float delta = (2.0f * a) / 255.0f;
    float s = 0.0f;
    for (int ci = threadIdx.x; ci < Ci; ci += 256) {
        const float X = rintf(w[(int64_t)co * Ci + ci] / delta);
        const float q = fminf(fmaxf(X, -128.0f), 127.0f);
        idx[(int64_t)co * Ci + ci] = (signed char)q;
        idxT[(int64_t)ci * Co + co] = (signed char)q;
        s += q;
    }
    float v[1] = {s};
    block_sum<float, 1>(v, red);
    if (threadIdx.x == 0) {
        dw[co] = delta;
        rw[co] = v[0];
    }
}

}

using namespace fqss;

static int grad_pieces() {
    const char* e = getenv("FQSS_GRAD_PIECES");
    return (e != nullptr && e[0] == '2') ? 2 : 3;
}

extern "C" int fqss_wq_codes(const float* w, int8_t* idx, int8_t* idxT, float* dw, float* rw, int Co, int Ci,
                             const float* qmin, const float* qmax, fqss_stream_t stream) {
    FQSS_REQUIRE(w && idx && idxT && dw && rw && qmin && qmax && Co > 0 && Ci > 0, "bad args");
    hipLaunchKernelGGL(k_wq_codes, dim3((unsigned)Co), dim3(256), 0, (hipStream_t)stream, w, (signed char*)idx,
                       (signed char*)idxT, dw, rw, Co, Ci, qmin, qmax);
    return launch_status("fqss_wq_codes");
}

struct QpwQuant {
    int act; const float* slope; const float *min1, *max1, *min2, *max2; uint8_t *yc1, *yc2; int64_t ld1, ld2;
    long long* stats;
    const FqssAddAfter *add1, *add2;
};

static int qpw_fwd_impl(const char* who, const uint8_t* xc, const int8_t* wi, const float* dw, const float* rw, const float* bias1,
                        const float* bias2, const float* qmin_x, const float* qmax_x, float* z1, float* z2, int B, int Ci, int Co1,
                        int Co2, int M, int64_t ld_xc, int64_t ld_z1, int64_t ld_z2, fqss_stream_t stream,
                        const QpwQuant* qq = nullptr) {
    if (B == 0 || M == 0) return FQSS_OK;
    const int Co = Co1 + Co2;
    FQSS_REQUIRE(xc && wi && dw && rw && qmin_x && qmax_x && z1 && (Co2 == 0 || z2), "null tensor");
    FQSS_REQUIRE(B >= 0 && Ci > 0 && Co1 > 0 && Co2 >= 0 && M >= 0 && ld_xc >= M && ld_z1 >= M && (Co2 == 0 || ld_z2 >= M), "bad shape");
    FQSS_REQUIRE(Ci % 16 == 0 && Ci <= 512 && ld_xc % 16 == 0 && aligned16(xc) && aligned16(wi),
                 "q-GEMM needs Ci % 16 == 0, Ci <= 512 (exact fp32 integer sum) and 16-B aligned code rows");
    FQSS_REQUIRE(aligned16(z1) && ld_z1 % 4 == 0 && (Co2 == 0 || (aligned16(z2) && ld_z2 % 4 == 0)), "output rows must be 16-B aligned");
    FQSS_REQUIRE((bias1 == nullptr) == (bias2 == nullptr) || Co2 == 0, "paired layers: both or neither with bias");
    if (qq != nullptr) FQSS_REQUIRE(Co2 == 0 || Co1 % 32 == 0, "fused quantizer of a pair needs Co1 % 32 == 0");
    QGemmArgs g{};
    g.A = wi; g.B = xc; g.C = z1; g.M = Co; g.N = M; g.K = Ci;
    g.lda = Ci; g.ldb = ld_xc; g.ldc = ld_z1;
    g.sAb = 0; g.sBb = (int64_t)Ci * ld_xc; g.sCb = (int64_t)Co1 * ld_z1;
    g.M1 = Co1; g.C2 = z2; g.ldc2 = ld_z2; g.sC2b = (int64_t)Co2 * ld_z2; g.bias2 = bias2; g.K1 = Ci;
    g.dw = dw; g.rw = rw; g.bias = bias1; g.qmin_x = qmin_x; g.qmax_x = qmax_x; g.ksplit = 1; g.kchunk = Ci;
    if (qq != nullptr) {
        FQSS_REQUIRE(qq->min1 && qq->max1 && qq->yc1 && (Co2 == 0 || (qq->min2 && qq->max2 && qq->yc2)), "fused quantizer: null pointer");
        FQSS_REQUIRE(qq->ld1 % 16 == 0 && qq->ld1 >= M && aligned16(qq->yc1) && (Co2 == 0 || (qq->ld2 % 16 == 0 && qq->ld2 >= M && aligned16(qq->yc2))),
                     "output code rows must be 16-B aligned");
        FQSS_REQUIRE(qq->act != FQSS_ACT_PRELU || qq->slope, "PReLU needs a slope");
        g.Q1 = qq->yc1; g.Q2 = qq->yc2; g.ldq1 = qq->ld1; g.ldq2 = qq->ld2;
        g.sQ1b = (int64_t)Co1 * qq->ld1; g.sQ2b = (int64_t)Co2 * qq->ld2;
        g.qy_min1 = qq->min1; g.qy_max1 = qq->max1; g.qy_min2 = qq->min2; g.qy_max2 = qq->max2;
        g.qact = qq->act; g.qslope = qq->slope;
        FQSS_REQUIRE(!qq->stats || Co2 == 0, "output statistics: single-output launches only");
        g.stats = qq->stats;
        const FqssAddAfter* ad[2] = {qq->add1, qq->add2};
        for (int i = 0; i < 2; ++i) {
            const FqssAddAfter* a = ad[i];
            if (a == nullptr) continue;
            FQSS_REQUIRE(i == 0 || Co2 > 0, "fused AddQ behind a second output that does not exist");
            FQSS_REQUIRE(qq->act == FQSS_ACT_NONE, "fused AddQ: the conv in front of it has no activation (Conv1dQ)");
            FQSS_REQUIRE(a->a && a->y && a->amin && a->amax && a->qmin && a->qmax, "fused AddQ: null pointer");
            FQSS_REQUIRE(a->ld_a % 16 == 0 && a->ld_a >= M && a->ld_y % 16 == 0 && a->ld_y >= M && aligned16(a->a) && aligned16(a->y),
                         "fused AddQ: code rows must be 16-B aligned");
            if (i == 0) {
                g.AD1 = a->a; g.ldad1 = a->ld_a; g.S1 = a->y; g.lds1 = a->ld_y;
                g.ad_min1 = a->amin; g.ad_max1 = a->amax; g.s_min1 = a->qmin; g.s_max1 = a->qmax;
            } else {
                g.AD2 = a->a; g.ldad2 = a->ld_a; g.S2 = a->y; g.lds2 = a->ld_y;
                g.ad_min2 = a->amin; g.ad_max2 = a->amax; g.s_min2 = a->qmin; g.s_max2 = a->qmax;
            }
        }
    }
    g.tiles_n = (int)cdiv(M, QBN); g.tiles_m = (int)cdiv(Co, QBM); g.batches = B;
    hipLaunchKernelGGL((k_qgemm<0>), dim3(xcd_grid((int64_t)g.tiles_n * B, g.tiles_m)), dim3(256), 0, (hipStream_t)stream, g);
    return launch_status(who);
}

extern "C" int fqss_qpw_fwd(const uint8_t* xc, const int8_t* wi, const float* dw, const float* rw, const float* bias,
                            const float* qmin_x, const float* qmax_x, float* z, int B, int Ci, int Co, int M,
                            int64_t ld_xc, int64_t ld_z, fqss_stream_t stream) {
    return qpw_fwd_impl("fqss_qpw_fwd", xc, wi, dw, rw, bias, nullptr, qmin_x, qmax_x, z, nullptr, B, Ci, Co, 0, M, ld_xc, ld_z, 0, stream);
}

extern "C" int fqss_qpw_fwd2(const uint8_t* xc, const int8_t* wi, const float* dw, const float* rw, const float* bias1,
                             const float* bias2, const float* qmin_x, const float* qmax_x, float* z1, float* z2, int B, int Ci,
                             int Co1, int Co2, int M, int64_t ld_xc, int64_t ld_z1, int64_t ld_z2, fqss_stream_t stream) {
    FQSS_REQUIRE(Co2 > 0, "second layer missing");
    return qpw_fwd_impl("fqss_qpw_fwd2", xc, wi, dw, rw, bias1, bias2, qmin_x, qmax_x, z1, z2, B, Ci, Co1, Co2, M, ld_xc, ld_z1, ld_z2, stream);
}

extern "C" int fqss_qpw_fwdq(const uint8_t* xc, const int8_t* wi, const float* dw, const float* rw, const float* bias1,
                             const float* bias2, const float* qmin_x, const float* qmax_x, float* z1, float* z2, int act,
                             const float* slope, const float* qmin1, const float* qmax1, const float* qmin2, const float* qmax2,
                             uint8_t* yc1, uint8_t* yc2, int B, int Ci, int Co1, int Co2, int M, int64_t ld_xc, int64_t ld_z1,
                             int64_t ld_z2, int64_t ld_yc1, int64_t ld_yc2, int64_t* stats1, fqss_stream_t stream) {
    QpwQuant qq{act, slope, qmin1, qmax1, qmin2, qmax2, yc1, yc2, ld_yc1, ld_yc2, (long long*)stats1, nullptr, nullptr};
    return qpw_fwd_impl("fqss_qpw_fwdq", xc, wi, dw, rw, bias1, bias2, qmin_x, qmax_x, z1, z2, B, Ci, Co1, Co2, M, ld_xc, ld_z1, ld_z2,
                        stream, &qq);
}

extern "C" int fqss_qpw_fwdq_add(const uint8_t* xc, const int8_t* wi, const float* dw, const float* rw, const float* bias1,
                                 const float* bias2, const float* qmin_x, const float* qmax_x, float* z1, float* z2, const float* qmin1,
                                 const float* qmax1, const float* qmin2, const float* qmax2, uint8_t* yc1, uint8_t* yc2, int B, int Ci,
                                 int Co1, int Co2, int M, int64_t ld_xc, int64_t ld_z1, int64_t ld_z2, int64_t ld_yc1, int64_t ld_yc2,
                                 const FqssAddAfter* add1, const FqssAddAfter* add2, fqss_stream_t stream) {
    QpwQuant qq{FQSS_ACT_NONE, nullptr, qmin1, qmax1, qmin2, qmax2, yc1, yc2, ld_yc1, ld_yc2, nullptr, add1, add2};
    return qpw_fwd_impl("fqss_qpw_fwdq_add", xc, wi, dw, rw, bias1, bias2, qmin_x, qmax_x, z1, z2, B, Ci, Co1, Co2, M, ld_xc, ld_z1,
                        ld_z2, stream, &qq);
}

static int qpw_bwd_x_impl(const char* who, const float* gz1, const float* gz2, const int8_t* wiT, const float* dw, float* gx, int B,
                          int Ci, int Co1, int Co2, int M, int64_t ld_gz1, int64_t ld_gz2, int64_t ld_gx, fqss_stream_t stream,
                          const float* addend = nullptr, int64_t ld_add = 0) {
    if (B == 0 || M == 0) return FQSS_OK;
    const int Co = Co1 + Co2;
    FQSS_REQUIRE(gz1 && wiT && dw && gx && (Co2 == 0 || gz2), "null tensor");
    FQSS_REQUIRE(B >= 0 && Ci > 0 && Co1 > 0 && Co2 >= 0 && M >= 0 && ld_gz1 >= M && ld_gx >= M, "bad shape");
    FQSS_REQUIRE(Co1 % 16 == 0 && Co2 % 16 == 0 && ld_gz1 % 4 == 0 && aligned16(gz1) && aligned16(wiT) && ld_gz1 >= ((M + 3) & ~3),
                 "q-GEMM dgrad needs Co % 16 == 0 and 16-B aligned gradient rows");
    FQSS_REQUIRE(Co2 == 0 || (ld_gz2 % 4 == 0 && aligned16(gz2) && ld_gz2 >= ((M + 3) & ~3)), "second gradient: 16-B aligned rows");
    FQSS_REQUIRE(aligned16(gx) && ld_gx % 4 == 0, "output rows must be 16-B aligned");
    FQSS_REQUIRE(Co <= 1024, "dgrad stages delta_w of at most 1024 output channels in LDS");
    if (B == 0 || M == 0) return FQSS_OK;
    QGemmArgs g{};
    g.A = wiT; g.B = gz1; g.C = gx; g.M = Ci; g.N = M; g.K = Co;
    g.lda = Co; g.ldb = ld_gz1; g.ldc = ld_gx;
    g.sAb = 0; g.sBb = (int64_t)Co1 * ld_gz1; g.sCb = (int64_t)Ci * ld_gx;
    g.M1 = Ci; g.K1 = Co1; g.B2 = gz2; g.ldb2 = ld_gz2; g.sB2b = (int64_t)Co2 * ld_gz2;
    g.dw = dw; g.ksplit = 1; g.kchunk = Co;
    if (addend != nullptr) {
        FQSS_REQUIRE(aligned16(addend) && ld_add % 4 == 0 && ld_add >= ((M + 3) & ~3), "addend rows must be 16-B aligned and padded to 4");
        g.C2 = const_cast<float*>(addend); g.ldc2 = ld_add; g.sC2b = (int64_t)Ci * ld_add;
    }
    g.tiles_n = (int)cdiv(M, QBN); g.tiles_m = (int)cdiv(Ci, QBM); g.batches = B;
    if (grad_pieces() == 3)
        hipLaunchKernelGGL((k_qgemm<1, 3>), dim3(xcd_grid((int64_t)g.tiles_n * B, g.tiles_m)), dim3(256), 0, (hipStream_t)stream, g);
    else
        hipLaunchKernelGGL((k_qgemm<1, 2>), dim3(xcd_grid((int64_t)g.tiles_n * B, g.tiles_m)), dim3(256), 0, (hipStream_t)stream, g);
    return launch_status(who);
}

extern "C" int fqss_qpw_bwd_x(const float* gz, const int8_t* wiT, const float* dw, float* gx, int B, int Ci, int Co,
                              int M, int64_t ld_gz, int64_t ld_gx, fqss_stream_t stream) {
    return qpw_bwd_x_impl("fqss_qpw_bwd_x", gz, nullptr, wiT, dw, gx, B, Ci, Co, 0, M, ld_gz, 0, ld_gx, stream);
}

extern "C" int fqss_qpw_bwd_x_add(const float* gz, const int8_t* wiT, const float* dw, const float* addend, float* gx, int B, int Ci, int Co,
                                  int M, int64_t ld_gz, int64_t ld_add, int64_t ld_gx, fqss_stream_t stream) {
    FQSS_REQUIRE(addend, "null addend");
    return qpw_bwd_x_impl("fqss_qpw_bwd_x_add", gz, nullptr, wiT, dw, gx, B, Ci, Co, 0, M, ld_gz, 0, ld_gx, stream, addend, ld_add);
}

extern "C" int fqss_qpw_bwd_x2(const float* gz1, const float* gz2, const int8_t* wiT, const float* dw, float* gx, int B, int Ci,
                               int Co1, int Co2, int M, int64_t ld_gz1, int64_t ld_gz2, int64_t ld_gx, fqss_stream_t stream) {
    FQSS_REQUIRE(Co2 > 0, "second layer missing");
    return qpw_bwd_x_impl("fqss_qpw_bwd_x2", gz1, gz2, wiT, dw, gx, B, Ci, Co1, Co2, M, ld_gz1, ld_gz2, ld_gx, stream);
}

static int qpw_bwd_w_impl(const char* who, const float* gz1, const float* gz2, const uint8_t* xc, const float* qmin_x,
                          const float* qmax_x, float* gw, int B, int Ci, int Co1, int Co2, int M, int64_t ld_gz1, int64_t ld_gz2,
                          int64_t ld_xc, fqss_stream_t stream) {
    if (B == 0 || M == 0) return FQSS_OK;
    const int Co = Co1 + Co2;
    FQSS_REQUIRE(gz1 && xc && qmin_x && qmax_x && gw && (Co2 == 0 || gz2), "null tensor");
    FQSS_REQUIRE(B >= 0 && Ci > 0 && Co1 > 0 && Co2 >= 0 && M >= 0 && ld_gz1 >= M && ld_xc >= M, "bad shape");
    FQSS_REQUIRE(ld_gz1 % 4 == 0 && ld_xc % 16 == 0 && aligned16(gz1) && aligned16(xc) && ld_gz1 >= ((M + 3) & ~3),
                 "q-GEMM wgrad needs 16-B aligned gradient and code rows");
    FQSS_REQUIRE(Co2 == 0 || (ld_gz2 % 4 == 0 && aligned16(gz2) && ld_gz2 >= ((M + 3) & ~3)), "second gradient: 16-B aligned rows");
    if (B == 0 || M == 0) return FQSS_OK;
    QGemmArgs g{};
    g.A = gz1; g.B = xc; g.C = gw; g.M = Co; g.N = Ci; g.K = M;
    g.lda = ld_gz1; g.ldb = ld_xc; g.ldc = Ci;
    g.sAb = (int64_t)Co1 * ld_gz1; g.sBb = (int64_t)Ci * ld_xc; g.sCb = 0;
    g.M1 = Co1; g.A2 = gz2; g.lda2 = ld_gz2; g.sA2b = (int64_t)Co2 * ld_gz2; g.K1 = M;
    g.qmin_x = qmin_x; g.qmax_x = qmax_x;
    const int64_t tiles = cdiv(Co, 64) * cdiv(Ci, 128) * B;
    int want = (int)((WGRAD_BLOCKS + tiles / 2) / tiles);
    if (want < 1) want = 1;
    g.tiles_n = (int)cdiv(Ci, 128); g.tiles_m = (int)cdiv(Co, 64); g.batches = B;
    const int kchunk = (int)cdiv(cdiv(M, want), W2_RING * W2_TK) * W2_RING * W2_TK;
    g.kchunk = kchunk;
    g.ksplit = (int)cdiv(M, kchunk);
    if (grad_pieces() == 3)
        hipLaunchKernelGGL(k_qwgrad2<3>, dim3(xcd_grid((int64_t)B * g.ksplit, (int64_t)g.tiles_m * g.tiles_n)), dim3(512), 0, (hipStream_t)stream, g);
    else
        hipLaunchKernelGGL(k_qwgrad2<2>, dim3(xcd_grid((int64_t)B * g.ksplit, (int64_t)g.tiles_m * g.tiles_n)), dim3(512), 0, (hipStream_t)stream, g);
    return launch_status(who);
}

extern "C" int fqss_qpw_bwd_w(const float* gz, const uint8_t* xc, const float* qmin_x, const float* qmax_x, float* gw,
                              int B, int Ci, int Co, int M, int64_t ld_gz, int64_t ld_xc, fqss_stream_t stream) {
    return qpw_bwd_w_impl("fqss_qpw_bwd_w", gz, nullptr, xc, qmin_x, qmax_x, gw, B, Ci, Co, 0, M, ld_gz, 0, ld_xc, stream);
}
// ... 190 lines not shown
```

fqss_amd/kernels.py:

```python
import os

import torch

from . import _lib

Q_BYPASS, Q_OBSERVE, Q_QUANT = 0, 1, 2
ACT_NONE, ACT_PRELU, ACT_RELU = 0, 1, 2
ACT_GELU = 3
ACT_POST_RELU = 4

GACC_DOUBLES = 2048 * 3
USE_X3 = True
LD_ALIGN = 16


def _p(t):
    return None if t is None else t.data_ptr()


import ctypes as _C

DESC_ABI = os.environ.get("FQSS_FLAT_ABI", "0") == "0"
_DT = {torch.float32: _lib.DT_F32, torch.uint8: _lib.DT_U8, torch.int8: _lib.DT_I8, torch.float64: _lib.DT_F64, torch.int16: _lib.DT_U16,
       torch.int64: _lib.DT_I64}
# ... 322 lines not shown
    gz, B, Co, M, ld_gz = _bcm(gz)
    gx = empty_act((B, Ci, M), gz.device)
    _lib.call("fqss_pwconv_bwd_x", _p(gz), _p(w), _p(gx), B, Ci, Co, M, ld_gz, rowmat(gx)[2], _stream())
    return gx


def pwconv_bwd_w(gz, x, gw):
    _need_gpu(gz, x, gw)
    gz, B, Co, M, ld_gz = _bcm(gz)
    x, _, Ci, _, ld_x = _bcm(x)
    assert gw.is_contiguous() and gw.numel() == Co * Ci
    _lib.call("fqss_pwconv_bwd_w", _p(gz), _p(x), _p(gw), B, Ci, Co, M, ld_gz, ld_x, _stream())


class WCodes:
    __slots__ = ("idx", "idxT", "dw", "rw", "Co", "Ci")


def wq_codes(w, qmin, qmax):
    _need_gpu(w, qmin, qmax)
    Co, Ci = w.shape[0], w.shape[1]
    assert w.numel() == Co * Ci and w.is_contiguous()
    c = WCodes()
    c.Co, c.Ci = Co, Ci
    c.idx = torch.empty(Co, Ci, device=w.device, dtype=torch.int8)
    c.idxT = torch.empty(Ci, Co, device=w.device, dtype=torch.int8)
    c.dw = torch.empty(Co, device=w.device, dtype=torch.float32)
    c.rw = torch.empty(Co, device=w.device, dtype=torch.float32)
    _lib.call("fqss_wq_codes", _p(w), _p(c.idx), _p(c.idxT), _p(c.dw), _p(c.rw), Co, Ci, _p(qmin), _p(qmax), _stream())
    return c


def q_eligible(Ci, Co):
    return _lib.BACKEND != "cpu" and Ci % 16 == 0 and Co % 16 == 0 and Ci <= 512


def qpw_fwd(xc, wc, bias, qmin_x, qmax_x):
    B, Ci, M = xc.shape
    rm = rowmat(xc)
    assert rm is not None and rm[2] % 16 == 0
    z = empty_act((B, wc.Co, M), xc.device)
    _lib.call("fqss_qpw_fwd", _p(xc), _p(wc.idx), _p(wc.dw), _p(wc.rw), _p(bias), _p(qmin_x), _p(qmax_x), _p(z),
              B, Ci, wc.Co, M, rm[2], rowmat(z)[2], _stream())
    return z


def qpw_bwd_x(gz, wc, add=None):
    assert wc.idxT is not None, "this layer's codes live in a concatenated pair image: use qpw_bwd_x2"
    gz, B, Co, M, ld_gz = _bcm(gz)
    if ld_gz % 4 != 0 or gz.data_ptr() % 16 != 0:
        c = empty_act(tuple(gz.shape), gz.device)
        c.copy_(gz)
        gz, ld_gz = c, rowmat(c)[2]
    gx = empty_act((B, wc.Ci, M), gz.device)
    if add is not None:
        assert tuple(add.shape) == (B, wc.Ci, M)
        add, ld_add = _aligned_grad(add)
        _lib.call("fqss_qpw_bwd_x_add", _p(gz), _p(wc.idxT), _p(wc.dw), _p(add), _p(gx), B, wc.Ci, Co, M, ld_gz, ld_add, rowmat(gx)[2], _stream())
    else:
        _lib.call("fqss_qpw_bwd_x", _p(gz), _p(wc.idxT), _p(wc.dw), _p(gx), B, wc.Ci, Co, M, ld_gz, rowmat(gx)[2], _stream())
    return gx


def qpw_bwd_w(gz, xc, qmin_x, qmax_x, gw):
    gz, B, Co, M, ld_gz = _bcm(gz)
    if ld_gz % 4 != 0 or gz.data_ptr() % 16 != 0:
        c = empty_act(tuple(gz.shape), gz.device)
        c.copy_(gz)
        gz, ld_gz = c, rowmat(c)[2]
    Ci = xc.shape[1]
    _lib.call("fqss_qpw_bwd_w", _p(gz), _p(xc), _p(qmin_x), _p(qmax_x), _p(gw), B, Ci, Co, M, ld_gz, rowmat(xc)[2], _stream())


def qpw_fwd2(xc, wc, bias1, bias2, qmin_x, qmax_x, Co1):
    B, Ci, M = xc.shape
    rm = rowmat(xc)
    assert rm is not None and Ci == wc.Ci and 0 < Co1 < wc.Co
    z1, z2 = empty_act((B, Co1, M), xc.device), empty_act((B, wc.Co - Co1, M), xc.device)
    _lib.call("fqss_qpw_fwd2", _p(xc), _p(wc.idx), _p(wc.dw), _p(wc.rw), _p(bias1), _p(bias2), _p(qmin_x), _p(qmax_x), _p(z1), _p(z2),
              B, Ci, Co1, wc.Co - Co1, M, rm[2], rowmat(z1)[2], rowmat(z2)[2], _stream())
    return z1, z2


def qpw_fwdq(xc, wc, bias1, bias2, qmin_x, qmax_x, Co1, act, slope, r1, r2=None, stats=None, adds=None):
    B, Ci, M = xc.shape
    rm = rowmat(xc)
    Co2 = wc.Co - Co1
    assert rm is not None and Ci == wc.Ci and Co2 >= 0 and (Co2 == 0) == (r2 is None)
    z1, yc1 = empty_act((B, Co1, M), xc.device), empty_codes((B, Co1, M), xc.device)
    z2 = yc2 = None
    if Co2:
        z2, yc2 = empty_act((B, Co2, M), xc.device), empty_codes((B, Co2, M), xc.device)
    if adds is not None and any(a is not None for a in adds):
        assert act == ACT_NONE and stats is None and (adds[1] is None or Co2)
        sums, recs = [], []
        for a, Co in zip(adds, (Co1, Co2)):
            if a is None:
                sums.append(None); recs.append(None)
                continue
            ac, amin, amax, qmin, qmax = a
            assert tuple(ac.shape) == (B, Co, M) and rowmat(ac) is not None
            sc = empty_codes((B, Co, M), xc.device)
            r = _lib.FqssAddAfter()
            r.a, r.ld_a, r.amin, r.amax, r.qmin, r.qmax, r.y, r.ld_y = _p(ac), rowmat(ac)[2], _p(amin), _p(amax), _p(qmin), _p(qmax), _p(sc), rowmat(sc)[2]
            sums.append(sc); recs.append(r)
        _lib.call("fqss_qpw_fwdq_add", _p(xc), _p(wc.idx), _p(wc.dw), _p(wc.rw), _p(bias1), _p(bias2), _p(qmin_x), _p(qmax_x), _p(z1), _p(z2),
                  _p(r1[0]), _p(r1[1]), _p(r2[0]) if r2 else None, _p(r2[1]) if r2 else None, _p(yc1), _p(yc2),
                  B, Ci, Co1, Co2, M, rm[2], rowmat(z1)[2], rowmat(z2)[2] if Co2 else 0, rowmat(yc1)[2], rowmat(yc2)[2] if Co2 else 0,
                  _ref(recs[0]) if recs[0] is not None else None, _ref(recs[1]) if recs[1] is not None else None, _stream())
        return ((z1, z2, yc1, yc2) if Co2 else (z1, yc1)) + (tuple(sums),)
    if DESC_ABI:
        w = _lib.FqssWCodes()
        w.idx, w.idxT, w.dw, w.rw, w.Co, w.Ci = _p(wc.idx), _p(wc.idxT), _p(wc.dw), _p(wc.rw), wc.Co, wc.Ci
        dx, dz1, dz2, dy1, dy2 = _desc(xc), _desc(z1), _desc(z2), _desc(yc1), _desc(yc2)
        qx, q1 = _qparams(qmin_x, qmax_x), _qparams(r1[0], r1[1], act, slope)
        q2 = _qparams(r2[0], r2[1], act, slope) if r2 else None
        ws, nws = (_p(stats.ws), stats.ws.numel() * stats.ws.element_size()) if stats is not None else (None, 0)
        _lib.call("fqss_pwconv_fq_fwd", _ref(dx), _ref(qx), _ref(w), _p(bias1), _p(bias2), _ref(dz1), _ref(dz2), _ref(dy1), _ref(dy2),
                  _ref(q1), _ref(q2), ws, nws, _stream())
        return (z1, z2, yc1, yc2) if Co2 else (z1, yc1)
    _lib.call("fqss_qpw_fwdq", _p(xc), _p(wc.idx), _p(wc.dw), _p(wc.rw), _p(bias1), _p(bias2), _p(qmin_x), _p(qmax_x), _p(z1), _p(z2),
              act, _p(slope), _p(r1[0]), _p(r1[1]), _p(r2[0]) if r2 else None, _p(r2[1]) if r2 else None, _p(yc1), _p(yc2),
              B, Ci, Co1, Co2, M, rm[2], rowmat(z1)[2], rowmat(z2)[2] if Co2 else 0, rowmat(yc1)[2], rowmat(yc2)[2] if Co2 else 0,
              _p(stats.ws) if stats is not None else None, _stream())
    return (z1, z2, yc1, yc2) if Co2 else (z1, yc1)


def qpw_bwd_x2(gz1, gz2, wc):
    gz1, ld1 = _aligned_grad(gz1)
    gz2, ld2 = _aligned_grad(gz2)
    B, Co1, M = gz1.shape
    Co2 = gz2.shape[1]
    assert Co1 + Co2 == wc.Co and gz2.shape[0] == B and gz2.shape[2] == M
    gx = empty_act((B, wc.Ci, M), gz1.device)
    _lib.call("fqss_qpw_bwd_x2", _p(gz1), _p(gz2), _p(wc.idxT), _p(wc.dw), _p(gx), B, wc.Ci, Co1, Co2, M, ld1, ld2, rowmat(gx)[2], _stream())
    return gx


def qpw_bwd_w2(gz1, gz2, xc, qmin_x, qmax_x, gw):
    gz1, ld1 = _aligned_grad(gz1)
    gz2, ld2 = _aligned_grad(gz2)
    B, Co1, M = gz1.shape
    Co2 = gz2.shape[1]
    Ci = xc.shape[1]
    assert gw.is_contiguous() and gw.numel() == (Co1 + Co2) * Ci
    _lib.call("fqss_qpw_bwd_w2", _p(gz1), _p(gz2), _p(xc), _p(qmin_x), _p(qmax_x), _p(gw), B, Ci, Co1, Co2, M, ld1, ld2, rowmat(xc)[2],
              _stream())


class WgradQueue:

    def __init__(self):
        self.jobs, self.ws = [], None

    def push(self, gz1, gz2, xc, qmin_x, qmax_x, gw):
        gz1, ld1 = _aligned_grad(gz1)
        ld2 = 0
        if gz2 is not None:
            gz2, ld2 = _aligned_grad(gz2)
        assert gw.is_contiguous()
        if any(j[5].data_ptr() == gw.data_ptr() for j in self.jobs):
            if gz2 is not None:
                qpw_bwd_w2(gz1, gz2, xc, qmin_x, qmax_x, gw)
            else:
                qpw_bwd_w(gz1, xc, qmin_x, qmax_x, gw)
            return
        self.jobs.append((gz1, gz2, xc, qmin_x, qmax_x, gw, ld1, ld2))

    def flush(self):
        if not self.jobs:
            return
        n = len(self.jobs)
        arr = (_lib.FqssWgradJob * n)()
        for j, (gz1, gz2, xc, lo, hi, gw, ld1, ld2) in zip(arr, self.jobs):
            B, Co1, M = gz1.shape
            j.gz1, j.gz2, j.xc, j.qmin_x, j.qmax_x, j.gw = _p(gz1), _p(gz2), _p(xc), _p(lo), _p(hi), _p(gw)
            j.B, j.Ci, j.Co1, j.Co2, j.M = B, xc.shape[1], Co1, (gz2.shape[1] if gz2 is not None else 0), M
            j.ld_gz1, j.ld_gz2, j.ld_xc = ld1, ld2, rowmat(xc)[2]
            assert gw.numel() == (j.Co1 + j.Co2) * j.Ci
        need = _lib.query("fqss_qpw_bwd_w_group_ws", arr, n)
        if need < 0:
            raise _lib.FqssError("fqss_qpw_bwd_w_group_ws: " + _lib.load().fqss_last_error().decode())
        if self.ws is None or self.ws.numel() < need:
            self.ws = torch.zeros(need, dtype=torch.uint8, device=self.jobs[0][0].device)
        _lib.call("fqss_qpw_bwd_w_group", arr, n, _p(self.ws), self.ws.numel(), _stream())
        self.jobs = []


def _codes3(xc):
    rm = rowmat(xc)
    assert xc.dim() == 3 and rm is not None and rm[2] % 16 == 0 and xc.data_ptr() % 16 == 0, "bad code layout"
    return xc.shape[0], xc.shape[1], xc.shape[2], rm[2]


def decode(xc, qmin, qmax):
    rm = rowmat(xc)
    out = empty_act(tuple(xc.shape), xc.device)
    _lib.call("fqss_decode", _p(xc), _p(out), rm[0], rm[1], rm[2], rowmat(out)[2], _p(qmin), _p(qmax), _stream())
    return out


class CodeStats:
    __slots__ = ("ws", "nslots")

    def __init__(self, ws, nslots):
        self.ws, self.nslots = ws, nslots


_STAT_SLOTS = {}


def stat_slots(kind, C, M):
    key = (kind, C, M)
    v = _STAT_SLOTS.get(key)
    if v is None:
        v = _STAT_SLOTS[key] = _lib.query("fqss_qpw_stat_slots" if kind == "qpw" else "fqss_dwq_stat_slots", C, M)
    return v


def new_stats(kind, B, C, M, device):
    n = stat_slots(kind, C, M)
    return CodeStats(torch.empty(B * n * 2, device=device, dtype=torch.int64), n) if n else None


def gnq_fwd(xc, qmin_x, qmax_x, gamma, beta, eps, qmin, qmax, write_out, stats=None):
    B, C, M, ld_xc = _codes3(xc)
    yc = empty_codes((B, C, M), xc.device)
    out = empty_act((B, C, M), xc.device)
    mean_rstd = torch.empty(B, 2, device=xc.device, dtype=torch.float32)
    ws = torch.empty(2 * 64 * B, device=xc.device, dtype=torch.int64) if stats is None else None
    _lib.call("fqss_gnq_fwd", _p(xc), _p(qmin_x), _p(qmax_x), _p(gamma), _p(beta), _p(yc), _p(out) if write_out else None,
              _p(mean_rstd), B, C, M, ld_xc, rowmat(yc)[2], rowmat(out)[2], float(eps), _p(qmin), _p(qmax), _p(ws),
              _p(stats.ws) if stats is not None else None, stats.nslots if stats is not None else 0, _stream())
    return out, yc, mean_rstd


def _aligned_grad(g):
    g, _, _, ld = as_rowmat(g)
    if ld % 4 != 0 or g.data_ptr() % 16 != 0:
        c = empty_act(tuple(g.shape), g.device)
        c.copy_(g)
        g, ld = c, rowmat(c)[2]
    return g, ld


def gnq_bwd(xc, qmin_x, qmax_x, g, gamma, beta, mean_rstd, qmin, qmax, gacc, ggamma, gbeta, producer=None):
    B, C, M, ld_xc = _codes3(xc)
    g, ld_g = _aligned_grad(g)
    gx = empty_act((B, C, M), xc.device)
    ws = torch.empty(2 * B * C + 2 * B, device=xc.device, dtype=torch.float64)
    if producer is None:
        _lib.call("fqss_gnq_bwd", _p(xc), _p(qmin_x), _p(qmax_x), _p(g), _p(gamma), _p(beta), _p(mean_rstd), _p(gx),
                  _p(ggamma), _p(gbeta), B, C, M, ld_xc, ld_g, rowmat(gx)[2], _p(qmin), _p(qmax), _p(gacc), _p(ws), _stream())
    else:
        pz, pact, pslope, pgacc, pgbias = producer
        rz = rowmat(pz)
        assert tuple(pz.shape) == (B, C, M) and rz is not None
        _lib.call("fqss_gnq_bwd_p", _p(xc), _p(qmin_x), _p(qmax_x), _p(g), _p(gamma), _p(beta), _p(mean_rstd), _p(gx),
                  _p(ggamma), _p(gbeta), B, C, M, ld_xc, ld_g, rowmat(gx)[2], _p(qmin), _p(qmax), _p(gacc), _p(ws),
                  _p(pz), rz[2], pact, _p(pslope), _p(pgacc), _p(pgbias), _stream())
    return gx


def gnq_bwd_rows(xc, qmin_x, qmax_x, g, gamma, beta, mean_rstd, qmin, qmax, gacc):
    B, C, M, ld_xc = _codes3(xc)
    g, ld_g = _aligned_grad(g)
    ws = torch.empty(2 * B * C, device=xc.device, dtype=torch.float64)
    _lib.call("fqss_gnq_bwd_rows", _p(xc), _p(qmin_x), _p(qmax_x), _p(g), _p(gamma), _p(beta), _p(mean_rstd), B, C, M, ld_xc, ld_g,
              _p(qmin), _p(qmax), _p(gacc), _p(ws), _stream())
    return g, ws


def gnq_bwd_apply(xc, qmin_x, qmax_x, g, gamma, beta, mean_rstd, qmin, qmax, ws, ggamma, gbeta, producer=None):
    B, C, M, ld_xc = _codes3(xc)
    g, ld_g = _aligned_grad(g)
    gx = empty_act((B, C, M), xc.device)
    pz, pact, pslope, pgacc, pgbias = producer if producer is not None else (None, 0, None, None, None)
    ld_pz = 0
    if pz is not None:
        rz = rowmat(pz)
        assert tuple(pz.shape) == (B, C, M) and rz is not None
        ld_pz = rz[2]
    _lib.call("fqss_gnq_bwd_apply", _p(xc), _p(qmin_x), _p(qmax_x), _p(g), _p(gamma), _p(beta), _p(mean_rstd), _p(gx), _p(ggamma),
              _p(gbeta), B, C, M, ld_xc, ld_g, rowmat(gx)[2], _p(qmin), _p(qmax), _p(ws), _p(pz), ld_pz, pact, _p(pslope), _p(pgacc),
              _p(pgbias), _stream())
    return gx


def dwq_fwd(xc, qmin_x, qmax_x, w, bias, dil, pad, act, slope, qmin, qmax, write_out, stats=None):
    B, C, M, ld_xc = _codes3(xc)
    yc = empty_codes((B, C, M), xc.device)
    out = empty_act((B, C, M), xc.device)
    _lib.call("fqss_dwq_fwd", _p(xc), _p(qmin_x), _p(qmax_x), _p(w), _p(bias), _p(yc), _p(out) if write_out else None,
              B, C, M, w.shape[-1], dil, pad, ld_xc, rowmat(yc)[2], rowmat(out)[2], act, _p(slope), _p(qmin), _p(qmax),
              _p(stats.ws) if stats is not None else None, _stream())
    return out, yc


def dwq_bwd_z(xc, qmin_x, qmax_x, w, bias, g, dil, pad, act, slope, qmin, qmax, gacc, gbias):
    B, C, M, ld_xc = _codes3(xc)
    g, ld_g = _aligned_grad(g)
    gz = empty_act((B, C, M), xc.device)
    _lib.call("fqss_dwq_bwd_z", _p(xc), _p(qmin_x), _p(qmax_x), _p(w), _p(bias), _p(g), _p(gz), B, C, M, w.shape[-1], dil,
              pad, ld_xc, ld_g, rowmat(gz)[2], act, _p(slope), _p(qmin), _p(qmax), _p(gacc), _p(gbias), _stream())
    return gz


def _codes2(xc):
    rm = rowmat(xc)
    assert rm is not None and rm[2] % 16 == 0 and xc.data_ptr() % 16 == 0, "bad code layout"
    return rm


def ewq_fwd(ac, amin, amax, bc, bmin, bmax, bf, sb, act, slope, qmin, qmax, write_out):
    rows, cols, ld_a = _codes2(ac)
    ld_b = _codes2(bc)[2] if bc is not None else 0
    ld_bf = 0
    if bf is not None:
        bf, ld_bf = _aligned_grad(bf)
    yc = empty_codes(tuple(ac.shape), ac.device)
    out = empty_act(tuple(ac.shape), ac.device)
    _lib.call("fqss_ewq_fwd", _p(ac), _p(amin), _p(amax), _p(bc), _p(bmin), _p(bmax), _p(bf), float(sb), _p(yc),
              _p(out) if write_out else None, rows, cols, ld_a, ld_b, ld_bf, rowmat(yc)[2], rowmat(out)[2], act, _p(slope),
              _p(qmin), _p(qmax), _stream())
    return out, yc


ADD_CHAIN_MAX = 24


def add_chain_ok(rows, cols, C, nlev):
    return bool(_lib.query("fqss_add_chain_ok", rows, cols, C, nlev))


def add_chain_bwd(levels, g, prod_a=None):
    ac0 = levels[0]["ac"]
    B, C, M = ac0.shape
    rows, cols, ld_a = _codes2(ac0)
    ld_b = _codes2(levels[0]["bc"])[2]
    g, ld_g = _aligned_grad(g)
    arr = (_lib.FqssAddChainLevel * len(levels))()
    outs, keep = [], []
    ld_bz = ld_bout = None
    for r, lv in zip(arr, levels):
        z, pact, pslope, pgacc, pgbias = lv["prod_b"]
        assert pact == ACT_NONE and tuple(lv["ac"].shape) == (B, C, M) and tuple(lv["bc"].shape) == (B, C, M) and tuple(z.shape) == (B, C, M)
        o = empty_act((B, C, M), ac0.device)
        outs.append(o)
        assert _codes2(lv["ac"])[2] == ld_a and _codes2(lv["bc"])[2] == ld_b
        lz, lo = rowmat(z)[2], rowmat(o)[2]
        assert (ld_bz is None or (ld_bz, ld_bout) == (lz, lo))
        ld_bz, ld_bout = lz, lo
        r.ac, r.bc, r.bz, r.bout = _p(lv["ac"]), _p(lv["bc"]), _p(z), _p(o)
        r.amin, r.amax, r.bmin, r.bmax, r.qmin, r.qmax = (_p(lv[k]) for k in ("amin", "amax", "bmin", "bmax", "qmin", "qmax"))
        r.gacc, r.bgacc, r.bgbias = _p(lv["gacc"]), _p(pgacc), _p(pgbias)
    ga = aout = az = agacc = agbias = None
    ld_ga = ld_az = ld_aout = 0
    if prod_a is not None:
        az, pact, pslope, agacc, agbias = prod_a
        assert pact == ACT_NONE and tuple(az.shape) == (B, C, M)
        aout = empty_act((B, C, M), ac0.device)
        ld_az, ld_aout = rowmat(az)[2], rowmat(aout)[2]
    else:
        ga = empty_act((B, C, M), ac0.device)
        ld_ga = rowmat(ga)[2]
    _lib.call("fqss_add_chain_bwd", arr, len(levels), _p(g), ld_g, _p(ga), ld_ga, _p(az), ld_az, _p(aout), ld_aout, _p(agacc), _p(agbias),
              rows, cols, C, ld_a, ld_b, ld_bz, ld_bout, _stream())
    return outs, (aout if prod_a is not None else ga)

# ... 1756 lines not shown
```

fqss_amd/ops.py:

```python
import os

import torch
from torch.autograd import Function

from . import kernels as K

Q_BYPASS, Q_OBSERVE, Q_QUANT = K.Q_BYPASS, K.Q_OBSERVE, K.Q_QUANT
ACT_NONE, ACT_PRELU, ACT_RELU = K.ACT_NONE, K.ACT_PRELU, K.ACT_RELU


class QCtx:
    __slots__ = ("qmode", "qmin", "qmax", "obs_ws", "gacc", "owner", "idx", "carrier", "keep_out", "prod", "no_codes", "stats", "hand", "presum", "chain", "link")

    def __init__(self, qmode=Q_BYPASS, qmin=None, qmax=None, obs_ws=None, gacc=None, owner=None):
        self.qmode, self.qmin, self.qmax, self.obs_ws, self.gacc, self.owner = qmode, qmin, qmax, obs_ws, gacc, owner
        self.idx = None
        self.carrier = False
        self.keep_out = False
        self.prod = None
        self.no_codes = False
        self.stats = None
        self.hand = None
        self.presum = None
        self.chain = False
        self.link = None


class ActCodes:
    __slots__ = ("idx", "qmin", "qmax")

    def __init__(self, idx, qmin, qmax):
        self.idx, self.qmin, self.qmax = idx, qmin, qmax


def tag_codes(y, q):
    if q.idx is not None and not CODED:
        assert not q.carrier, "codes-only carriers need the coded dataflow"
        q.idx = q.prod = q.stats = q.hand = q.presum = q.link = None
    if q.idx is not None:
        y._fqss_q = ActCodes(q.idx, q.qmin.detach(), q.qmax.detach())
        y._fqss_carrier = q.carrier
        q.idx = None
        if q.prod is not None:
            y._fqss_prod, q.prod = q.prod, None
        if q.stats is not None:
            y._fqss_stats, q.stats = q.stats, None
        if q.hand is not None:
            y._fqss_hand, q.hand = q.hand, None
        if q.presum is not None:
            y._fqss_presum, q.presum = q.presum, None
        if q.link is not None:
            y._fqss_chain, q.link = q.link, None
    return y


class _Producer:
    __slots__ = ("z", "act", "slope", "slope_param", "q", "bias_param", "bias", "fused")

    def __init__(self, z, act, slope, slope_param, q, bias_param, bias):
        self.z, self.act, self.slope, self.slope_param, self.q, self.bias_param, self.bias = z, act, slope, slope_param, q, bias_param, bias
        self.fused = False


class _GnHand:
    __slots__ = ("kind", "fwd", "rec")

    def __init__(self, kind, fwd=None):
        self.kind, self.fwd, self.rec = kind, fwd, None


FUSE_GN_BWD_DW = os.environ.get("FQSS_FUSE_GN_BWD_DW", "1") != "0"
_GN_HAND = os.environ.get("FQSS_GN_HAND", "both")
FUSE_GN = os.environ.get("FQSS_FUSE_GN", "1") != "0"
FUSE_EW = os.environ.get("FQSS_FUSE_EW", "1") != "0"
FUSE_ADD_FWD = os.environ.get("FQSS_FUSE_ADD_FWD", "1") != "0"


FUSE_ADD_CHAIN = os.environ.get("FQSS_FUSE_ADD_CHAIN", "1") != "0"


class _ChainLink:
    __slots__ = ("prev", "ac", "amin", "amax", "bc", "bmin", "bmax", "qmin", "qmax", "q", "prod_a", "prod_b", "pre", "dummy")

    def __init__(self, prev, ac, amin, amax, bc, bmin, bmax, qmin, qmax, q, prod_a, prod_b):
        self.prev, self.ac, self.amin, self.amax, self.bc, self.bmin, self.bmax = prev, ac, amin, amax, bc, bmin, bmax
        self.qmin, self.qmax, self.q, self.prod_a, self.prod_b = qmin, qmax, q, prod_a, prod_b
        self.pre = self.dummy = None


class _PreSum:
    __slots__ = ("codes", "a_idx", "owner")

    def __init__(self, codes, a_idx, owner):
        self.codes, self.a_idx, self.owner = codes, a_idx, owner
FUSE_STATS = os.environ.get("FQSS_FUSE_STATS", "1") != "0"
NEXT_IS_GROUPNORM = False
NEXT_IS_DW3 = False


NEXT_TAKES_PRODUCER = False
FUSE_MULQ_PROD = os.environ.get("FQSS_FUSE_MULQ_PROD", "1") != "0"


def _producer_args(pr):
    if pr is None or pr.q.gacc is None:
        return None
    pgb, direct = (None, True) if pr.bias is None else _grad_buf(pr.bias_param, pr.bias)
    return (pr.z, pr.act, pr.slope, pr.q.gacc, pgb) if direct else None


def codes_of(x):
    return getattr(x, "_fqss_q", None)


def is_carrier(x):
    return getattr(x, "_fqss_carrier", False)


FAST = False
CODED = True
DEBUG_POISON = bool(int(__import__("os").environ.get("FQSS_DEBUG_CARRIER", "0")))


DEFER = None


class deferred:
    def __init__(self, tables):
        self.t = tables

    def __enter__(self):
        global DEFER
        self.prev, DEFER = DEFER, self.t

    def __exit__(self, *a):
        global DEFER
        DEFER = self.prev


class fast_codes:
    def __init__(self, on=True):
        self.on = on

    def __enter__(self):
        global FAST
        self.prev, FAST = FAST, self.on

    def __exit__(self, *a):
        global FAST
        FAST = self.prev


class coded_dataflow:

    def __init__(self, on=True):
        self.on = on

    def __enter__(self):
        global CODED
        self.prev, CODED = CODED, self.on

    def __exit__(self, *a):
        global CODED
        CODED = self.prev


class poison_carriers:

    def __init__(self, on=True):
        self.on = on

    def __enter__(self):
        global DEBUG_POISON
        self.prev, DEBUG_POISON = DEBUG_POISON, self.on

    def __exit__(self, *a):
        global DEBUG_POISON
        DEBUG_POISON = self.prev


def _carrier(out):
    if DEBUG_POISON:
        out.fill_(float("nan"))
    return out


class Materialize(Function):

    @staticmethod
    def forward(ctx, x, xq):
        return K.decode(xq.idx, xq.qmin, xq.qmax)
# ... 185 lines not shown
    if q.qmode == Q_BYPASS:
        return g, None, None, None, None
    return _epilogue_bwd(z, g, ACT_NONE, None, None, q)


class _Lin:
    __slots__ = ("kind", "stride", "dil", "pad", "w_param", "b_param", "slope_param", "six", "taps", "wc_dgrad")

    def __init__(self, kind, stride=1, dil=1, pad=0, w_param=None, b_param=None, slope_param=None, six=False, taps=1):
        self.kind, self.stride, self.dil, self.pad = kind, stride, dil, pad
        self.six = six
        self.taps = taps
        self.wc_dgrad = None
        self.w_param, self.b_param, self.slope_param = w_param, b_param, slope_param


FRAME_CODES_FWD = os.environ.get("FQSS_FRAME_CODES_FWD", "1") != "0"


def _lin_fwd(L, x, w, bias):
    if L.kind == "pw":
        if L.wc_dgrad is not None and FRAME_CODES_FWD and x.dim() == 3:
            z = K.pwconv_fwd_wq(x, L.wc_dgrad, bias)
            if z is not None:
                return z
        return K.pwconv_fwd(x, w, bias, L.six)
    if L.kind == "conv1":
        return K.conv1d_s1_fwd(x, w.reshape(w.shape[0], -1), bias, L.taps, L.dil, L.pad)
    if L.kind == "dw":
        return K.dwconv_fwd(x, w, bias, L.dil, L.pad)
    if L.kind == "frames":
        assert bias is None
        return K.frames_conv_fwd(x, w, L.stride)
    if L.kind == "convtr":
        assert bias is None and w.shape[1] == 1
        return K.ola_convtr_fwd(x, w, L.stride)
    raise NotImplementedError(L.kind)


def _lin_bwd_x(L, gz, w, x_shape):
    if L.kind == "pw":
        return K.pwconv_bwd_x(gz, w, x_shape[1])
    if L.kind == "conv1":
        Co, Ci, T = w.shape[0], x_shape[1], L.taps
        wt = w.reshape(Co, Ci, T).flip(2).permute(1, 0, 2).reshape(Ci, Co * T).contiguous()
        return K.conv1d_s1_fwd(gz, wt, None, T, L.dil, L.dil * (T - 1) - L.pad)
    if L.kind == "dw":
        return K.dwconv_bwd_x(gz, w, L.dil, L.pad)
    if L.kind == "frames":
        parts = [K.ola_convtr_fwd(gz, w[:, ci, :].contiguous(), L.stride) for ci in range(x_shape[1])]
        return parts[0] if len(parts) == 1 else torch.cat(parts, dim=1)
    if L.kind == "convtr":
        return K.frames_conv_fwd(gz, w.reshape(w.shape[0], 1, w.shape[2]), L.stride)
    raise NotImplementedError(L.kind)


def _lin_bwd_w(L, gz, x, gw):
    if L.kind == "pw":
        K.pwconv_bwd_w(gz, x, gw)
    elif L.kind == "conv1":
        K.conv1d_s1_bwd_w(gz, x, gw, L.taps, L.dil, L.pad)
    elif L.kind == "dw":
        K.dwconv_bwd_w(gz, x, gw, L.dil, L.pad)
    elif L.kind == "frames":
        K.frames_wgrad(gz, x, gw, L.stride)
    elif L.kind == "convtr":
        K.frames_wgrad(x, gz, gw, L.stride)
    else:
        raise NotImplementedError(L.kind)


FRAME_CODES_DGRAD = os.environ.get("FQSS_FRAME_CODES_DGRAD", "1") != "0"
PLAIN_BIAS_SUM = os.environ.get("FQSS_PLAIN_BIAS_SUM", "1") != "0"


class LinearActQ(Function):

    @staticmethod
    def forward(ctx, x, w, bias, slope, qmin, qmax, L, act, q, xq=None, wc=None):
        ctx.xq = xq if (L.kind == "pw" and xq is not None and K.q_eligible(w.shape[1], w.shape[0])) else None
        ctx.wc = wc if (L.kind == "pw" and wc is not None and K.q_eligible(w.shape[1], w.shape[0])) else None
        ctx.plain = (q.qmode == Q_BYPASS and act == ACT_NONE)
        ctx.xq_tr = xq if (L.kind == "convtr" and xq is not None and bias is None and K.ola_convtr_ok(w, L.stride)) else None
        if ctx.xq is not None and ctx.wc is not None and _fuse_out_quant(q):
            q.stats = K.new_stats("qpw", x.shape[0], ctx.wc.Co, x.shape[-1], x.device) if (FUSE_STATS and NEXT_IS_GROUPNORM) else None
            z, q.idx = K.qpw_fwdq(ctx.xq.idx, ctx.wc, bias, None, ctx.xq.qmin, ctx.xq.qmax, ctx.wc.Co, act, slope, (q.qmin, q.qmax),
                                  stats=q.stats)
            q.carrier = True
            out = _carrier(K.empty_act(tuple(z.shape), z.device))
        else:
            if ctx.xq is not None and ctx.wc is not None:
                z = K.qpw_fwd(ctx.xq.idx, ctx.wc, bias, ctx.xq.qmin, ctx.xq.qmax)
            elif ctx.xq_tr is not None:
                z = K.ola_convtr_fwd_q(ctx.xq_tr.idx, ctx.xq_tr.qmin, ctx.xq_tr.qmax, w, L.stride)
            else:
                z = _lin_fwd(L, x, w, bias)
            out = z if ctx.plain else _epilogue_fwd(z, act, slope, q)
        ctx.prod = None
        if ((FUSE_GN and NEXT_IS_GROUPNORM) or (FUSE_MULQ_PROD and NEXT_TAKES_PRODUCER and act in (ACT_NONE, ACT_RELU, ACT_PRELU))) \
                and DEFER is not None and q.qmode == Q_QUANT and not ctx.plain and q.owner is not None \
                and getattr(q.owner, "_fqss_deferred", False):
            ctx.prod = q.prod = _Producer(z, act, slope, L.slope_param, q, L.b_param, bias)
        ctx.x_shape = x.shape
        ctx.fork = getattr(x, "_fqss_fork", None) if ((ctx.wc is not None and ctx.wc.idxT is not None) or L.kind == "convtr") else None
        ctx.save_for_backward(None if ((ctx.xq is not None and ctx.wc is not None) or ctx.xq_tr is not None) else x, w,
                              None if ctx.plain else z, slope)
        ctx.L, ctx.act, ctx.q, ctx.has_bias = L, act, q, bias is not None
        ctx.bias_like = bias
        ctx.C = z.shape[1]
        return out

    @staticmethod
    def backward(ctx, g):
        x, w, z, slope = ctx.saved_tensors
        L, act, q = ctx.L, ctx.act, ctx.q
        if ctx.prod is not None and ctx.prod.fused:
            gz, g_slope, g_min, g_max, g_bias = g, None, None, None, None
            _touch(L.slope_param if act == ACT_PRELU else None, q.owner.min_range, q.owner.max_range, L.b_param)
        elif ctx.plain and not ctx.has_bias:
            gz, g_slope, g_min, g_max, g_bias = g, None, None, None, None
        elif ctx.plain and PLAIN_BIAS_SUM and g.dim() == 3 and g.is_cuda and L.kind in ("pw", "conv1") and K.rowmat(g) is not None \
                and K.rowmat(g)[2] % 4 == 0 and g.data_ptr() % 16 == 0:
            gb, gb_direct = _grad_buf(L.b_param, ctx.bias_like)
            K.chan_sum(g, gb)
            gz, g_slope, g_min, g_max, g_bias = g, None, None, None, (None if gb_direct else gb)
        else:
            gz, g_slope, g_min, g_max, g_bias = _epilogue_bwd(
                g if ctx.plain else z, g, act, slope, L.slope_param, q, bias_param=L.b_param,
                bias_like=ctx.bias_like if ctx.has_bias else None, C=ctx.C)
        gx = None
        if ctx.needs_input_grad[0]:
            fk = ctx.fork
            other = fk[0].take(fk[1], ctx.x_shape) if (fk is not None and (ctx.wc is not None or L.kind == "convtr")) else None
            if ctx.wc is not None and other is not None:
                gx = K.qpw_bwd_x(gz, ctx.wc, add=other)
            elif L.kind == "convtr" and other is not None:
                gx = K.frames_conv_fwd(gz, w.reshape(w.shape[0], 1, w.shape[2]), L.stride, add=other)
            elif ctx.wc is not None:
                gx = K.qpw_bwd_x(gz, ctx.wc)
            elif L.kind == "pw" and L.wc_dgrad is not None and FRAME_CODES_DGRAD and gz.dim() == 3:
                gx = K.qpw_bwd_x(gz, L.wc_dgrad)
            else:
                gx = _lin_bwd_x(L, gz, w, ctx.x_shape)
        gw = None
        gwq = getattr(w, "_fqss_gwq", None)
        if ctx.needs_input_grad[1] or gwq is not None:
            gw = gwq if gwq is not None else _wgrad_temp(w)
            if ctx.xq is not None:
                wq = getattr(DEFER, "wgrad_queue", None) if (gwq is not None and getattr(w, "_fqss_gwq_done", None) is None) else None
                if wq is not None:
                    wq.push(gz, None, ctx.xq.idx, ctx.xq.qmin, ctx.xq.qmax, gw)
                else:
                    K.qpw_bwd_w(gz, ctx.xq.idx, ctx.xq.qmin, ctx.xq.qmax, gw)
            else:
                if x is None and K.frames_wgrad1_q(ctx.xq_tr.idx, ctx.xq_tr.qmin, ctx.xq_tr.qmax, gz, gw, L.stride):
                    pass
                else:
                    if x is None:
                        x = K.decode(ctx.xq_tr.idx, ctx.xq_tr.qmin, ctx.xq_tr.qmax)
                    _lin_bwd_w(L, gz, x, gw)
            _wgrad_temp_done(gw, gwq)
            if L.w_param is not None and w is L.w_param:
                L.w_param._fqss_touched = True
            if gwq is not None:
                gw = None
                done = getattr(w, "_fqss_gwq_done", None)
                if done is not None:
                    done()
        return gx, gw, g_bias, g_slope, g_min, g_max, None, None, None, None, None


class LinearActQPair(Function):

    @staticmethod
    def forward(ctx, x, b1, b2, qmin1, qmax1, qmin2, qmax2, L1, L2, q1, q2, xq, pair, sole_ew=False, adds=None):
        Co1 = pair.Co1
        if _fuse_out_quant(q1) and _fuse_out_quant(q2) and Co1 % 32 == 0:
            kadds = None
            if adds is not None and FUSE_ADD_FWD:
                kadds = tuple(None if a is None else (a[0].idx, a[0].qmin, a[0].qmax, a[1].min_range, a[1].max_range) for a in adds)
            res = K.qpw_fwdq(xq.idx, pair.wc, b1, b2, xq.qmin, xq.qmax, Co1, ACT_NONE, None, (q1.qmin, q1.qmax), (q2.qmin, q2.qmax),
                             adds=kadds)
            z1, z2, q1.idx, q2.idx = res[:4]
            if kadds is not None and len(res) == 5:
                q1.presum, q2.presum = (None if sc is None else _PreSum(sc, a[0].idx, a[1]) for sc, a in zip(res[4], adds))
            q1.carrier = q2.carrier = True
            out1 = _carrier(K.empty_act(tuple(z1.shape), z1.device))
            out2 = _carrier(K.empty_act(tuple(z2.shape), z2.device))
        else:
            z1, z2 = K.qpw_fwd2(xq.idx, pair.wc, b1, b2, xq.qmin, xq.qmax, Co1)
            out1 = _epilogue_fwd(z1, ACT_NONE, None, q1)
            out2 = _epilogue_fwd(z2, ACT_NONE, None, q2)
        ctx.save_for_backward(z1, z2)
        ctx.L, ctx.q, ctx.b, ctx.xq, ctx.pair = (L1, L2), (q1, q2), (b1, b2), xq, pair
        ctx.prods = (None, None)
        if FUSE_EW and sole_ew and all(getattr(q.owner, "_fqss_deferred", False) for q in (q1, q2)):
            ctx.prods = (_Producer(z1, ACT_NONE, None, None, q1, L1.b_param, b1), _Producer(z2, ACT_NONE, None, None, q2, L2.b_param, b2))
            q1.prod, q2.prod = ctx.prods
        return out1, out2

    @staticmethod
    def backward(ctx, g1, g2):
        z = ctx.saved_tensors
        g_in = (g1, g2)
        gs, gz, gbias, gmin, gmax = [g1, g2], [], [], [], []
        for i in range(2):
            if gs[i] is None:
                gs[i] = K.empty_act(tuple(z[i].shape), z[i].device).zero_()
            L, q, b = ctx.L[i], ctx.q[i], ctx.b[i]
            if ctx.prods[i] is not None and ctx.prods[i].fused and g_in[i] is not None:
                _touch(q.owner.min_range, q.owner.max_range, L.b_param)
                gz.append(gs[i]); gbias.append(None); gmin.append(None); gmax.append(None)
                continue
            gzi, _, g_min, g_max, g_bias = _epilogue_bwd(z[i], gs[i], ACT_NONE, None, None, q, bias_param=L.b_param,
                                                          bias_like=b, C=z[i].shape[1])
            gz.append(gzi); gbias.append(g_bias); gmin.append(g_min); gmax.append(g_max)
        gx = K.qpw_bwd_x2(gz[0], gz[1], ctx.pair.wc) if ctx.needs_input_grad[0] else None
        wq = getattr(DEFER, "wgrad_queue", None)
        if wq is not None:
            wq.push(gz[0], gz[1], ctx.xq.idx, ctx.xq.qmin, ctx.xq.qmax, ctx.pair.gw)
        else:
            K.qpw_bwd_w2(gz[0], gz[1], ctx.xq.idx, ctx.xq.qmin, ctx.xq.qmax, ctx.pair.gw)
        return gx, gbias[0], gbias[1], gmin[0], gmax[0], gmin[1], gmax[1], None, None, None, None, None, None, None, None


FUSE_GNQ_F = os.environ.get("FQSS_FUSE_GNQ_F", "1") != "0"


class GroupNormActQ(Function):

    @staticmethod
    def forward(ctx, x, gamma, beta, qmin, qmax, eps, q, gamma_param, beta_param, xq=None):
        ctx.q, ctx.gp, ctx.bp = q, gamma_param, beta_param
        ctx.coded = xq is not None and q.qmode == Q_QUANT
        ctx.prod = getattr(x, "_fqss_prod", None) if ctx.coded else None
        ctx.hand_in = ctx.hand_out = None
        if ctx.coded:
            h = getattr(x, "_fqss_hand", None)
            ctx.hand_in = h if (h is not None and h.kind == "after") else None
            q.carrier = FAST and not q.keep_out
            st = getattr(x, "_fqss_stats", None)
            out, q.idx, mean_rstd = K.gnq_fwd(xq.idx, xq.qmin, xq.qmax, gamma, beta, eps, qmin, qmax, write_out=not q.carrier, stats=st)
            ctx.save_for_backward(gamma, beta, mean_rstd, xq.idx, xq.qmin, xq.qmax, qmin, qmax)
            if FUSE_GN_BWD_DW and _GN_HAND != "after" and NEXT_IS_DW3 and q.gacc is not None and x.dim() == 3 and x.shape[-1] <= K.DWQ_ROW_MAX:
                ctx.hand_out = q.hand = _GnHand("before", dict(xc0=xq.idx, qmin0=xq.qmin, qmax0=xq.qmax, gamma=gamma, beta=beta,
                                                                mean_rstd=mean_rstd, gacc=q.gacc))
            return _carrier(out) if q.carrier else out
        ctx.fused_f = FUSE_GNQ_F and q.qmode == Q_QUANT and q.gacc is not None and x.dim() == 3 and x.is_cuda
        if ctx.fused_f:
            out, q.idx, mean_rstd = K.gnq_fwd_f(x, gamma, beta, eps, qmin, qmax, want_idx=not q.no_codes)
            q.carrier = False
            ctx.save_for_backward(x, gamma, beta, mean_rstd, qmin, qmax)
            return out
        z, mean_rstd = K.gn_fwd(x, gamma, beta, eps)
        plain = q.qmode == Q_BYPASS
        out = z if plain else _epilogue_fwd(z, ACT_NONE, None, q)
        ctx.save_for_backward(x, gamma, None if plain else z, mean_rstd)
        return out

    @staticmethod
    def backward(ctx, g):
        q = ctx.q
        if ctx.coded:
            gamma, beta, mean_rstd, xc, xmin, xmax, qmin, qmax = ctx.saved_tensors
            gg, gg_direct = _grad_buf(ctx.gp, gamma)
            gb, gb_direct = _grad_buf(ctx.bp, gamma)
            producer = _producer_args(ctx.prod) if ctx.needs_input_grad[0] else None
            if producer is not None:
                ctx.prod.fused = True
            hi, ho = ctx.hand_in, ctx.hand_out
            if hi is not None and producer is None and gg_direct and gb_direct and ctx.needs_input_grad[0]:
                gx, ws = K.gnq_bwd_rows(xc, xmin, xmax, g, gamma, beta, mean_rstd, qmin, qmax, q.gacc)
                hi.rec = dict(gamma=gamma, beta=beta, mean_rstd=mean_rstd, ws=ws, qmin=qmin, qmax=qmax, ggamma=gg, gbeta=gb)
            elif ho is not None and ho.rec is not None:
                gx = K.gnq_bwd_apply(xc, xmin, xmax, g, gamma, beta, mean_rstd, qmin, qmax, ho.rec["ws"], gg, gb, producer=producer)
                ho.rec = None
            else:
                gx = K.gnq_bwd(xc, xmin, xmax, g, gamma, beta, mean_rstd, qmin, qmax, q.gacc, gg, gb, producer=producer)
            _, g_min, g_max = _flush_ranges(q, None, None, ACT_NONE)
            return gx, (None if gg_direct else gg), (None if gb_direct else gb), g_min, g_max, None, None, None, None, None
        if ctx.fused_f:
            x, gamma, beta, mean_rstd, qmin, qmax = ctx.saved_tensors
            gg, gg_direct = _grad_buf(ctx.gp, gamma)
            gb, gb_direct = _grad_buf(ctx.bp, gamma)
            gx = K.gnq_bwd_f(g.contiguous(), x, gamma, beta, mean_rstd, qmin, qmax, q.gacc, gg, gb)
            g_min, g_max = _ranges_after(q, q.gacc)
            return gx, (None if gg_direct else gg), (None if gb_direct else gb), g_min, g_max, None, None, None, None, None
        x, gamma, z, mean_rstd = ctx.saved_tensors
        gz, _, g_min, g_max, _ = _plain_or_bwd(z, g, q)
        gg, gg_direct = _grad_buf(ctx.gp, gamma)
        gb, gb_direct = _grad_buf(ctx.bp, gamma)
        gx = K.gn_bwd(gz, x, gamma, mean_rstd, gg, gb)
        return gx, (None if gg_direct else gg), (None if gb_direct else gb), g_min, g_max, None, None, None, None, None


class DwConvQ(Function):

    @staticmethod
    def forward(ctx, x, w, bias, slope, qmin, qmax, L, act, q, xq):
        q.carrier = FAST and not q.keep_out
        q.stats = K.new_stats("dwq", x.shape[0], x.shape[1], x.shape[2], x.device) if (FUSE_STATS and NEXT_IS_GROUPNORM) else None
        out, q.idx = K.dwq_fwd(xq.idx, xq.qmin, xq.qmax, w, bias, L.dil, L.pad, act, slope, qmin, qmax, write_out=not q.carrier,
                               stats=q.stats)
        ctx.save_for_backward(w, bias, slope, xq.idx, xq.qmin, xq.qmax, qmin, qmax)
        ctx.L, ctx.act, ctx.q = L, act, q
        ctx.hand_a = ctx.hand_b = None
        if FUSE_GN_BWD_DW and w.shape[-1] == 3 and x.shape[-1] <= K.DWQ_ROW_MAX and q.gacc is not None:
            h = getattr(x, "_fqss_hand", None)
            ctx.hand_b = h if (h is not None and h.kind == "before") else None
            if NEXT_IS_GROUPNORM and q.qmode == Q_QUANT and _GN_HAND != "before":
                ctx.hand_a = q.hand = _GnHand("after")
        return _carrier(out) if q.carrier else out

    @staticmethod
    def backward(ctx, g):
        w, bias, slope, xc, xmin, xmax, qmin, qmax = ctx.saved_tensors
        L, act, q = ctx.L, ctx.act, ctx.q
        gb, gb_direct = (None, True)
        if bias is not None:
            gb, gb_direct = _grad_buf(L.b_param, bias)
        gw = None
        gwq = getattr(w, "_fqss_gwq", None)
        want_gw = ctx.needs_input_grad[1] or gwq is not None
        if want_gw:
            gw = gwq if gwq is not None else _wgrad_temp(w)
        if xc.shape[-1] <= K.DWQ_ROW_MAX:
            after = before = None
            if ctx.hand_a is not None and ctx.hand_a.rec is not None:
                after, ctx.hand_a.rec = ctx.hand_a.rec, None
            if ctx.hand_b is not None and ctx.needs_input_grad[0]:
                before = dict(ctx.hand_b.fwd)
            gx = K.dwq_bwd(xc, xmin, xmax, w, bias, g, L.dil, L.pad, act, slope, qmin, qmax, q.gacc, gb, gw,
                           want_gx=ctx.needs_input_grad[0], after=after, before=before)
            if before is not None:
                ctx.hand_b.rec = dict(ws=before["ws"])
        else:
            gz = K.dwq_bwd_z(xc, xmin, xmax, w, bias, g, L.dil, L.pad, act, slope, qmin, qmax, q.gacc, gb)
            gx = K.dwconv_bwd_x(gz, w, L.dil, L.pad) if ctx.needs_input_grad[0] else None
            if want_gw:
                K.dwq_bwd_w(gz, xc, xmin, xmax, gw, L.dil, L.pad)
        g_slope, g_min, g_max = _flush_ranges(q, slope, L.slope_param, act)
        if want_gw:
            _wgrad_temp_done(gw, gwq)
            if L.w_param is not None and w is L.w_param:
                L.w_param._fqss_touched = True
            if gwq is not None:
                gw = None
        return gx, gw, (None if gb_direct else gb), g_slope, g_min, g_max, None, None, None, None


class EwQ(Function):

    @staticmethod
    def forward(ctx, a, b, slope, qmin, qmax, sb, act, q, aq_, bq_, slope_param):
        q.carrier = FAST and not q.keep_out
        bf = None if (b is None or bq_ is not None) else b
# ... 319 lines not shown
```

include/fqss.h:

```cpp
#ifndef FQSS_H
#define FQSS_H

#include <stddef.h>
#include <stdint.h>

#ifdef __cplusplus
extern "C" {
#endif

#define FQSS_VERSION 100

#define FQSS_OK 0
#define FQSS_EINVAL (-22)
#define FQSS_ELAUNCH (-5)

#define FQSS_Q_BYPASS 0
#define FQSS_Q_OBSERVE 1
#define FQSS_Q_QUANT 2

#define FQSS_ACT_NONE 0
#define FQSS_ACT_PRELU 1
#define FQSS_ACT_RELU 2
#define FQSS_ACT_GELU 3
#define FQSS_ACT_POST_RELU 4
// ... 155 lines not shown
                   const float* qmax, double* gacc, fqss_stream_t stream);

int fqss_decode(const uint8_t* codes, float* out, int64_t rows, int64_t cols, int64_t ld_c,
                int64_t ld_out, const float* qmin, const float* qmax, fqss_stream_t stream);
int fqss_gnq_fwd(const uint8_t* xc, const float* qmin_x, const float* qmax_x, const float* gamma,
                 const float* beta, uint8_t* yc, float* yout, float* mean_rstd, int B, int C, int M,
                 int64_t ld_xc, int64_t ld_yc, int64_t ld_out, float eps, const float* qmin,
                 const float* qmax, void* ws, const int64_t* stats, int nslots, fqss_stream_t stream);
int fqss_gnq_bwd(const uint8_t* xc, const float* qmin_x, const float* qmax_x, const float* g,
                 const float* gamma, const float* beta, const float* mean_rstd, float* gx,
                 float* ggamma, float* gbeta, int B, int C, int M, int64_t ld_xc, int64_t ld_g,
                 int64_t ld_gx, const float* qmin, const float* qmax, double* gacc, double* ws,
                 fqss_stream_t stream);
int fqss_gnq_bwd_p(const uint8_t* xc, const float* qmin_x, const float* qmax_x, const float* g,
                   const float* gamma, const float* beta, const float* mean_rstd, float* gz, float* ggamma,
                   float* gbeta, int B, int C, int M, int64_t ld_xc, int64_t ld_g, int64_t ld_gz,
                   const float* qmin, const float* qmax, double* gacc, double* ws, const float* pz,
                   int64_t ld_pz, int pact, const float* pslope, double* pgacc, float* pgbias,
                   fqss_stream_t stream);

int fqss_dwq_fwd(const uint8_t* xc, const float* qmin_x, const float* qmax_x, const float* w,
                 const float* bias, uint8_t* yc, float* yout, int B, int C, int M, int K, int dil,
                 int pad, int64_t ld_xc, int64_t ld_yc, int64_t ld_out, int act, const float* slope,
                 const float* qmin, const float* qmax, int64_t* stats, fqss_stream_t stream);
int fqss_dwq_bwd_z(const uint8_t* xc, const float* qmin_x, const float* qmax_x, const float* w,
                   const float* bias, const float* g, float* gz, int B, int C, int M, int K, int dil,
                   int pad, int64_t ld_xc, int64_t ld_g, int64_t ld_gz, int act, const float* slope,
                   const float* qmin, const float* qmax, double* gacc, float* gbias,
                   fqss_stream_t stream);
int fqss_ewq_fwd(const uint8_t* ac, const float* amin, const float* amax, const uint8_t* bc,
                 const float* bmin, const float* bmax, const float* bf, float sb, uint8_t* yc, float* yout,
                 int64_t rows, int64_t cols, int64_t ld_a, int64_t ld_b, int64_t ld_bf, int64_t ld_y,
                 int64_t ld_out, int act, const float* slope, const float* qmin, const float* qmax,
                 fqss_stream_t stream);
int fqss_ewq_bwd(const uint8_t* ac, const float* amin, const float* amax, const uint8_t* bc,
                 const float* bmin, const float* bmax, const float* bf, float sb, const float* g, float* gz,
                 int64_t rows, int64_t cols, int64_t ld_a, int64_t ld_b, int64_t ld_bf, int64_t ld_g,
                 int64_t ld_gz, int act, const float* slope, const float* qmin, const float* qmax,
                 double* gacc, fqss_stream_t stream);
int fqss_ewq_bwd_p(const uint8_t* ac, const float* amin, const float* amax, const uint8_t* bc,
                   const float* bmin, const float* bmax, float sb, const float* g, float* gz, int64_t rows,
                   int64_t cols, int64_t ld_a, int64_t ld_b, int64_t ld_g, int64_t ld_gz, int act,
                   const float* slope, const float* qmin, const float* qmax, double* gacc, int C,
                   const float* pa_z, int64_t ld_paz, int pa_act, const float* pa_slope, double* pa_gacc,
                   float* pa_gbias, float* pa_out, int64_t ld_pa_out, const float* pb_z, int64_t ld_pbz,
                   int pb_act, const float* pb_slope, double* pb_gacc, float* pb_gbias, float* pb_out,
                   int64_t ld_pb_out, fqss_stream_t stream);
int fqss_mulq_fwd(const uint8_t* mc, const float* mmin, const float* mmax, const uint8_t* fc, const float* fmin,
                  const float* fmax, uint8_t* yc, float* yout, int B, int S, int C, int M, int64_t ld_m, int64_t ld_f,
                  int64_t ld_y, int64_t ld_out, const float* qmin, const float* qmax, fqss_stream_t stream);
int fqss_mulq_bwd(const uint8_t* mc, const float* mmin, const float* mmax, const uint8_t* fc, const float* fmin,
                  const float* fmax, const float* g, float* gmask, float* gfeat, int B, int S, int C, int M, int64_t ld_m,
                  int64_t ld_f, int64_t ld_g, int64_t ld_gm, int64_t ld_gf, const float* qmin, const float* qmax,
                  double* gacc, const float* pz, int64_t ld_pz, int pact, const float* pslope, double* pgacc,
                  float* pgbias, fqss_stream_t stream);
int fqss_dwq_bwd_w(const float* gz, const uint8_t* xc, const float* qmin_x, const float* qmax_x,
                   float* gw, int B, int C, int M, int K, int dil, int pad, int64_t ld_gz,
                   int64_t ld_xc, fqss_stream_t stream);
int fqss_dwq_bwd(const uint8_t* xc, const float* qmin_x, const float* qmax_x, const float* w,
                 const float* bias, const float* g, float* gx, float* gw, int B, int C, int M, int K,
                 int dil, int pad, int64_t ld_xc, int64_t ld_g, int64_t ld_gx, int act, const float* slope,
                 const float* qmin, const float* qmax, double* gacc, float* gbias, fqss_stream_t stream);

typedef struct FqssGnAfter {
    const float* gamma; const float* beta; const float* mean_rstd;
    const double* ws;
    const float* qmin; const float* qmax;
    float* ggamma; float* gbeta;
} FqssGnAfter;
typedef struct FqssGnBefore {
    const uint8_t* xc0; int64_t ld_xc0; const float* qmin0; const float* qmax0;
    const float* gamma; const float* beta; const float* mean_rstd;
    double* ws;
    double* gacc;
} FqssGnBefore;
int fqss_gnq_bwd_rows(const uint8_t* xc, const float* qmin_x, const float* qmax_x, const float* g, const float* gamma,
                      const float* beta, const float* mean_rstd, int B, int C, int M, int64_t ld_xc, int64_t ld_g,
                      const float* qmin, const float* qmax, double* gacc, double* ws, fqss_stream_t stream);
int fqss_gnq_bwd_apply(const uint8_t* xc, const float* qmin_x, const float* qmax_x, const float* g, const float* gamma,
                       const float* beta, const float* mean_rstd, float* gx, float* ggamma, float* gbeta, int B, int C, int M,
                       int64_t ld_xc, int64_t ld_g, int64_t ld_gx, const float* qmin, const float* qmax, const double* ws,
                       const float* pz, int64_t ld_pz, int pact, const float* pslope, double* pgacc, float* pgbias,
                       fqss_stream_t stream);
int fqss_dwq_bwd_gn(const uint8_t* xc, const float* qmin_x, const float* qmax_x, const float* w, const float* bias,
                    const float* g, float* gx, float* gw, int B, int C, int M, int K, int dil, int pad, int64_t ld_xc,
                    int64_t ld_g, int64_t ld_gx, int act, const float* slope, const float* qmin, const float* qmax,
                    double* gacc, float* gbias, const FqssGnAfter* after, const FqssGnBefore* before, fqss_stream_t stream);

#define FQSS_TSTAT_SLOTS 32
#define FQSS_TSTAT_STRIDE 16
int fqss_split3_planes(const float* w, uint16_t* planes, int64_t n, fqss_stream_t stream);
int fqss_tgemm(const uint16_t* planes, const float* x, int B, int Ci, int Co, int M, int64_t ld_x, int pro,
               const double* pro_stats, const float* pro_gamma, const float* pro_beta, float pro_eps,
               const float* pro_slope, const float* bias, int act, const float* slope, double* stats_out,
               int M1, float* c1, const float* r1, int64_t ld_c1, float* c2, const float* r2,
               int64_t ld_c2, fqss_stream_t stream);
int fqss_tgemm_tiled_ok(int Ci, int Co, int M1);
int fqss_split3_tiles(const float* w, uint16_t* tiles, int Co, int Ci, fqss_stream_t stream);
int fqss_tgemm_tiled(const uint16_t* tiles, const float* x, int B, int Ci, int Co, int M, int64_t ld_x, int pro,
                     const double* pro_stats, const float* pro_gamma, const float* pro_beta, float pro_eps,
                     const float* pro_slope, const float* bias, int act, const float* slope, double* stats_out,
                     int M1, float* c1, const float* r1, int64_t ld_c1, float* c2, const float* r2,
                     int64_t ld_c2, fqss_stream_t stream);
int fqss_tdw(const float* x, const double* stats_in, const float* gamma, const float* beta, float eps,
             const float* w, const float* bias, const float* slope, float* y, double* stats_out, int B,
             int C, int M, int K, int dil, int pad, int64_t ld_x, int64_t ld_y, fqss_stream_t stream);
int fqss_tstats(const float* x, int B, int C, int M, int64_t ld, double* ws, fqss_stream_t stream);

int fqss_bn_moments(const float* x, double* out, int B, int C, int M, int64_t ld_x, fqss_stream_t stream);
int fqss_bn_apply(const float* x, const float* a, const float* b, float* y, int B, int C, int M, int64_t ld_x,
                  int64_t ld_y, fqss_stream_t stream);
int fqss_bn_bwd_reduce(const float* g, const float* x, double* out, int B, int C, int M, int64_t ld_g, int64_t ld_x,
                       fqss_stream_t stream);
int fqss_bn_bwd_apply(const float* g, const float* x, const float* c1, const float* c2, const float* c3, float* gx,
                      int B, int C, int M, int64_t ld_g, int64_t ld_x, int64_t ld_gx, fqss_stream_t stream);

int fqss_axpby(const float* a, const float* b, float sa, float sb, float* z, int64_t rows,
               int64_t cols, int64_t ld_a, int64_t ld_b, int64_t ld_z, fqss_stream_t stream);
int fqss_mul_bcast_fwd(const float* mask, const float* feat, float* z, int B, int S, int C, int M,
                       int64_t ld_mask, int64_t ld_feat, int64_t ld_z, fqss_stream_t stream);
int fqss_mul_bcast_bwd(const float* gz, const float* mask, const float* feat, float* gmask,
                       float* gfeat, int B, int S, int C, int M, int64_t ld_gz, int64_t ld_mask,
                       int64_t ld_feat, int64_t ld_gmask, int64_t ld_gfeat, fqss_stream_t stream);

int fqss_splitter2(const float* x, float* out, int B, int64_t T, const uint32_t* obs_ws,
                   fqss_stream_t stream);
int fqss_splitter2_raw(const float* x, float* out, int B, int64_t T, const uint32_t* obs_ws, fqss_stream_t stream);
int fqss_frames_conv_fwd(const float* x, const float* w, float* z, int N, int Ci, int Co,
                         int64_t T, int K, int stride, int M, int64_t ld_z, fqss_stream_t stream);
int fqss_frames_conv_add_fwd(const float* x, const float* w, const float* add, int64_t ld_add, float* z, int N, int Ci,
                             int Co, int64_t T, int K, int stride, int M, int64_t ld_z, fqss_stream_t stream);
int fqss_ola_convtr_fwd(const float* x, const float* w, float* out, int N, int C, int M,
                        int64_t ld_x, int K, int stride, int64_t T, fqss_stream_t stream);
int fqss_ola_convtr_fwd_q(const uint8_t* xc, const float* qmin, const float* qmax, const float* w, float* out, int N,
                          int C, int M, int64_t ld_x, int K, int stride, int64_t T, fqss_stream_t stream);
int fqss_ola_convtr_mul_fwd(const float* mask, const float* feat, const float* w, float* out, int N, int NS, int C, int M,
                            int64_t ld_m, int64_t ld_f, int K, int stride, int64_t T, fqss_stream_t stream);
int fqss_frames_wgrad(const float* a, const float* x, float* gw, int N, int C, int Ci, int M,
                      int64_t ld_a, int64_t T, int K, int stride, fqss_stream_t stream);
int fqss_frames_wgrad1(const float* a, const float* sig, float* gw, int N, int C, int M, int64_t ld_a, int64_t T, int K,
                       int stride, fqss_stream_t stream);
int fqss_frames_wgrad1s(const float* a, const float* sig, int64_t sig_ns, float* gw, int64_t ld_gw, int N, int C, int M,
                        int64_t ld_a, int64_t T, int K, int stride, fqss_stream_t stream);
int fqss_frames_wgrad1_q(const uint8_t* ac, const float* qmin, const float* qmax, const float* sig, float* gw, int N, int C,
                         int M, int64_t ld_a, int64_t T, int K, int stride, fqss_stream_t stream);

int fqss_kd_loss(const float* est, const float* fest, const float* tgt, int B, int64_t T,
                 float kd_lambda, double* stats, float* out, float* w_out, float* sisdr_out,
                 float* gest, fqss_stream_t stream);

int fqss_kd_loss_per_sample(const float* est, const float* fest, const float* tgt, int B, int64_t T,
                            float kd_lambda, int use_threshold, float threshold, double* stats, float* out,
                            float* w_out, float* sisdr_out, float* gest, fqss_stream_t stream);
int fqss_pit_sisdr_loss(const float* est, const float* tgt, int B, int64_t T, double* stats, float* out, float* w_out,
                        float* sisdr_out, float* gest, fqss_stream_t stream);
int fqss_kd_moments(const float* est, const float* fest, const float* tgt, int B, int64_t T, double* stats,
                    fqss_stream_t stream);

int fqss_set_deterministic(int slot, const float* grad_base, int64_t n, void* shadow);
int fqss_det_finish(float* grad_base, int64_t n, void* shadow, fqss_stream_t stream);
int fqss_sumsq(const float* g, int64_t n, double* sumsq, fqss_stream_t stream);
int fqss_adam_clip(float* p, const float* g, float* m, float* v, int64_t n, const double* sumsq,
                   float max_norm, float grad_scale, float lr, float beta1, float beta2, float eps,
                   int32_t* step_t, const int32_t* t0, float* gnorm_out, fqss_stream_t stream);


// ... 278 lines not shown
```

Before: 614.2.

## Recompute pointwise-conv pre-activation inside GroupNorm backward instead of storing it

The quantized pointwise conv forward can now skip writing its float pre-activation z when the next layer is GroupNorm. The GN backward apply kernel recomputes z on the fly with a fused q-GEMM main loop and applies the producer's activation/quant backward. This removes a large float activation write and read in exchange for redoing the GEMM in backward. Other paths rebuild z lazily when needed.

```diff
diff --git a/fqss_amd/_lib.py b/fqss_amd/_lib.py
--- a/fqss_amd/_lib.py
+++ b/fqss_amd/_lib.py
@@ -74,6 +74,8 @@
     "fqss_dwq_bwd_gn": [P, P, P, P, P, P, P, P, I32, I32, I32, I32, I32, I32, I64, I64, I64, I32, P, P, P, P, P, P, P, P],
     "fqss_gnq_bwd_rows": [P, P, P, P, P, P, P, I32, I32, I32, I64, I64, P, P, P, P, P],
     "fqss_gnq_bwd_apply": [P, P, P, P, P, P, P, P, P, P, I32, I32, I32, I64, I64, I64, P, P, P, P, I64, I32, P, P, P, P],
+    "fqss_gnq_bwd_apply_rz": [P, P, P, P, P, P, P, P, P, P, I32, I32, I32, I64, I64, I64, P, P, P, P, I32, I64, P, P, P, P, P, P,
+                              I32, P, P, P, P],
     "fqss_split3_planes": [P, P, I64, P],
     "fqss_tgemm": [P, P, I32, I32, I32, I32, I64, I32, P, P, P, F32, P, P, I32, P, P, I32, P, P, I64, P, P, I64, P],
     "fqss_tgemm_tiled": [P, P, I32, I32, I32, I32, I64, I32, P, P, P, F32, P, P, I32, P, P, I32, P, P, I64, P, P, I64, P],
diff --git a/fqss_amd/csrc/desc_api.hip b/fqss_amd/csrc/desc_api.hip
--- a/fqss_amd/csrc/desc_api.hip
+++ b/fqss_amd/csrc/desc_api.hip
@@ -144,23 +144,32 @@
     FQSS_REQUIRE(qx && qx->qmin && qx->qmax && q1 && q1->qmin && q1->qmax, "null quantizer");
     FQSS_REQUIRE(w && w->idx && w->dw && w->rw && w->Co > 0 && w->Ci > 0, "null weight codes");
     DESC_ROWS(rx, x, FQSS_DT_U8);
-    DESC_ROWS(rz1, z1, FQSS_DT_F32);
     DESC_ROWS(ry1, y1, FQSS_DT_U8);
     FQSS_REQUIRE(rx.C == w->Ci, "x channels != Ci");
-    FQSS_REQUIRE(rz1.B == rx.B && rz1.M == rx.M && same_shape(rz1, ry1), "z1 / y1 shapes");
-    const int Co1 = (int)rz1.C;
+    FQSS_REQUIRE(ry1.B == rx.B && ry1.M == rx.M, "y1 shape");
+    const bool no_z = z1 == nullptr;
+    Rows rz1{};
+    if (!no_z) {
+        DESC_ROWS(rz1_, z1, FQSS_DT_F32);
+        FQSS_REQUIRE(same_shape(rz1_, ry1), "z1 / y1 shapes");
+        rz1 = rz1_;
+    }
+    const int Co1 = (int)ry1.C;
     int Co2 = 0;
     Rows rz2{}, ry2{};
     if (z2 != nullptr || y2 != nullptr) {
-        FQSS_REQUIRE(z2 && y2 && q2 && q2->qmin && q2->qmax, "second layer: z2, y2 and q2 all needed");
-        DESC_ROWS(rz2_, z2, FQSS_DT_F32);
+        FQSS_REQUIRE(y2 && q2 && q2->qmin && q2->qmax && (z2 != nullptr) == !no_z, "second layer: y2 and q2 needed, z2 iff z1");
         DESC_ROWS(ry2_, y2, FQSS_DT_U8);
-        FQSS_REQUIRE(rz2_.B == rx.B && rz2_.M == rx.M && same_shape(rz2_, ry2_), "z2 / y2 shapes");
-        rz2 = rz2_;
+        FQSS_REQUIRE(ry2_.B == rx.B && ry2_.M == rx.M, "y2 shape");
+        if (!no_z) {
+            DESC_ROWS(rz2_, z2, FQSS_DT_F32);
+            FQSS_REQUIRE(same_shape(rz2_, ry2_), "z2 / y2 shapes");
+            rz2 = rz2_;
+        }
         ry2 = ry2_;
-        Co2 = (int)rz2.C;
-    }
-    FQSS_REQUIRE(Co1 + Co2 == w->Co, "z1 + z2 channels != Co of the weight codes");
+        Co2 = (int)ry2.C;
+    }
+    FQSS_REQUIRE(Co1 + Co2 == w->Co, "y1 + y2 channels != Co of the weight codes");
     int64_t* stats = nullptr;
     if (ws != nullptr && Co2 == 0) {
         const int64_t need = ws_bytes_of("pwconv_fq_fwd", rx.B, Co1, rx.M);
diff --git a/fqss_amd/csrc/fqss_dev.h b/fqss_amd/csrc/fqss_dev.h
--- a/fqss_amd/csrc/fqss_dev.h
+++ b/fqss_amd/csrc/fqss_dev.h
@@ -225,6 +225,37 @@
     inr = (X >= 0.0f) && (X <= 255.0f);
     c = __builtin_amdgcn_fmed3f(X, 0.0f, 255.0f);
     return r.delta * c + r.lo;
+}
+
+__device__ __forceinline__ void gn_coef_from_sums(const double (&sv)[2], float mean, float rstd, int C, int M, double& c2d, double& c3d) {
+    const double md = (double)mean, rd = (double)rstd;
+    const double inv_n = 1.0 / ((double)C * (double)M);
+    c2d = (sv[1] * md - sv[0]) * rd * rd * rd * inv_n;
+    c3d = -c2d * md - sv[1] * rd * inv_n;
+}
+template <bool FUSE>
+__device__ __forceinline__ float gnq_bwd_elem(float x, float gv, float pz, bool valid, float scale, float shift, float c2, float c3,
+                                              const QRange& ry, const QRange& rp, int pact, float pslope, float& p_du, float& p_out,
+                                              float& p_slope, float& p_bias) {
+    const float z = fmaf(x, scale, shift);
+    float cq, u;
+    bool inr;
+    (void)fq_asym(z, ry, cq, u, inr);
+    const float gz = inr ? div_by(gv * ry.delta, ry.delta, ry.inv) : 0.0f;
+    float o = fmaf(gz, scale, fmaf(x, c2, c3));
+    if (FUSE) {
+        const float gj = valid ? o : 0.0f;
+        const float t = act_apply(pz, pact, pslope);
+        float pc, pu;
+        bool pin;
+        (void)fq_asym(t, rp, pc, pu, pin);
+        const float gt = pin ? div_by(gj * rp.delta, rp.delta, rp.inv) : 0.0f;
+        p_du += gj * (pin ? (pc - pu) : pc);
+        p_out += pin ? 0.0f : gj;
+        o = act_bwd(pz, gt, pact, pslope, valid, p_slope);
+        p_bias += valid ? o : 0.0f;
+    }
+    return o;
 }
 
 __device__ __forceinline__ float fq_code(float t, const QRange& r) {
diff --git a/fqss_amd/csrc/fused_q.hip b/fqss_amd/csrc/fused_q.hip
--- a/fqss_amd/csrc/fused_q.hip
+++ b/fqss_amd/csrc/fused_q.hip
@@ -191,12 +191,6 @@
     }
 }
 
-__device__ __forceinline__ void gn_coef_from_sums(const double (&sv)[2], float mean, float rstd, int C, int M, double& c2d, double& c3d) {
-    const double md = (double)mean, rd = (double)rstd;
-    const double inv_n = 1.0 / ((double)C * (double)M);
-    c2d = (sv[1] * md - sv[0]) * rd * rd * rd * inv_n;
-    c3d = -c2d * md - sv[1] * rd * inv_n;
-}
 
 __global__ __launch_bounds__(256) void k_gnq_bwd_rows(const uint8_t* __restrict__ xc, const float* __restrict__ g,
                                                        const float* __restrict__ gamma, const float* __restrict__ beta,
@@ -345,29 +339,9 @@
             float xv[4], o[4];
             dec4(wq_[i], rx, xv);
 #pragma unroll
-            for (int e = 0; e < 4; ++e) {
-                const float x = xv[e];
-                const float z = fmaf(x, scale, shift);
-                float cq, u;
-                bool inr;
-                (void)fq_asym(z, ry, cq, u, inr);
-                const float gz = inr ? div_by(gv[e] * ry.delta, ry.delta, ry.inv) : 0.0f;
-                o[e] = fmaf(gz, scale, fmaf(x, c2, c3));
-                if (FUSE) {
-                    const bool valid = (m + e < M);
-                    const float gj = valid ? o[e] : 0.0f;
-                    const float t = act_apply(pzv[e], P.act, pslope);
-                    float pc, pu;
-                    bool pin;
-                    (void)fq_asym(t, rp, pc, pu, pin);
-                    const float gt = pin ? div_by(gj * rp.delta, rp.delta, rp.inv) : 0.0f;
-                    p_du += gj * (pin ? (pc - pu) : pc);
-                    p_out += pin ? 0.0f : gj;
-                    const float gzj = act_bwd(pzv[e], gt, P.act, pslope, valid, p_slope);
-                    o[e] = gzj;
-                    p_bias += valid ? gzj : 0.0f;
-                }
-            }
+            for (int e = 0; e < 4; ++e)
+                o[e] = gnq_bwd_elem<FUSE>(xv[e], gv[e], pzv[e], m + e < M, scale, shift, c2, c3, ry, rp, P.act, pslope, p_du, p_out,
+                                          p_slope, p_bias);
             *reinterpret_cast<float4*>(orow + m) = make_float4(o[0], o[1], o[2], o[3]);
         }
     }
diff --git a/fqss_amd/csrc/qgemm.hip b/fqss_amd/csrc/qgemm.hip
--- a/fqss_amd/csrc/qgemm.hip
+++ b/fqss_amd/csrc/qgemm.hip
@@ -59,6 +59,12 @@
 }
 
 __device__ __forceinline__ float dec(unsigned int c, const QRange& r) { return r.delta * (float)c + r.lo; }
+
+__device__ __forceinline__ float qfwd_z(float S, float dwr, float rwr, float bias, bool has_bias, float dx, float mnx) {
+    float v = dwr * (dx * S + mnx * rwr);
+    if (has_bias) v = v + bias;
+    return v;
+}
 
 struct QGemmArgs {
     const void* A;
@@ -92,52 +98,37 @@
     float imp_inv_taps, imp_inv_kw;
 };
 
-template <int MODE, int GP = 3, bool IMP = false>
-__global__ __launch_bounds__(256, 2) void k_qgemm(QGemmArgs g) {
-    static_assert(!IMP || MODE == 1 || MODE == 3 || MODE == 4, "implicit convolution: float B operands");
-    static_assert(MODE == 0 || MODE == 1 || MODE == 3 || MODE == 4, "unknown q-GEMM mode");
-    static_assert(GP == 3 || (GP == 2 && MODE != 0 && MODE != 4), "two gradient pieces: dgrad only");
-    constexpr bool ACODES = MODE < 2 || MODE == 4;
-    constexpr int WMODE = MODE == 4 ? 1 : MODE;
-    constexpr bool SIX = MODE == 3 && GP == 2;
-    constexpr int NA = (MODE == 3) ? 3 : 1;
-    constexpr int NB = (MODE == 1) ? GP : (MODE == 3 || MODE == 4) ? 3 : 1;
-    constexpr int BROWS = QBK, BLD = LDN;
-    constexpr int A_BYTES = NA * QBM * LDK * 2, B_BYTES = NB * BROWS * BLD * 2;
-    constexpr int T_BYTES = 4 * 32 * LDT * 4;
-    constexpr int SMEM = (A_BYTES + B_BYTES > T_BYTES) ? A_BYTES + B_BYTES : T_BYTES;
-    __shared__ __attribute__((aligned(16))) unsigned char smem[SMEM];
+template <int MODE, int GP, bool IMP>
+struct QCfg {
+    static constexpr bool ACODES = MODE < 2 || MODE == 4;
+    static constexpr int WMODE = MODE == 4 ? 1 : MODE;
+    static constexpr bool SIX = MODE == 3 && GP == 2;
+    static constexpr int NA = (MODE == 3) ? 3 : 1;
+    static constexpr int NB = (MODE == 1) ? GP : (MODE == 3 || MODE == 4) ? 3 : 1;
+    static constexpr int BROWS = QBK, BLD = LDN;
+    static constexpr int A_BYTES = NA * QBM * LDK * 2, B_BYTES = NB * BROWS * BLD * 2;
+    static constexpr int T_BYTES = 4 * 32 * LDT * 4;
+    static constexpr int SMEM = (A_BYTES + B_BYTES > T_BYTES) ? A_BYTES + B_BYTES : T_BYTES;
+};
+
+template <int MODE, int GP, bool IMP>
+__device__ __forceinline__ void qgemm_main_loop(const QGemmArgs& g, unsigned char* smem, int b, int i0, int j0, f32x16 (&acc)[2]) {
+    typedef QCfg<MODE, GP, IMP> Q;
+    constexpr bool ACODES = Q::ACODES;
+    constexpr int WMODE = Q::WMODE;
+    constexpr bool SIX = Q::SIX;
+    constexpr int NA = Q::NA, NB = Q::NB, BROWS = Q::BROWS, BLD = Q::BLD, A_BYTES = Q::A_BYTES;
     typedef unsigned short (*AsT)[QBM][LDK];
     typedef unsigned short (*BsT)[BROWS][BLD];
     AsT As = reinterpret_cast<AsT>(smem);
     BsT Bs = reinterpret_cast<BsT>(smem + A_BYTES);
-
-    const int tid = threadIdx.x, lane = tid & 63;
+    int tid = threadIdx.x;
+    asm volatile("" : "+v"(tid));
+    const int lane = tid & 63;
     const int wave = __builtin_amdgcn_readfirstlane(tid >> 6);
     const int wm = wave >> 1, wn = wave & 1;
     const int lr = lane & 31, lh = lane >> 5;
-    int panel, mt;
-    if (!xcd_tile(g.tiles_n * g.batches, g.tiles_m, panel, mt)) return;
-    const int b = panel / g.tiles_n;
     const int kbeg = 0, kend = g.K;
-    const int i0 = mt * QBM, j0 = (panel % g.tiles_n) * QBN;
-
-    f32x16 acc[2];
-#pragma unroll
-    for (int mi = 0; mi < 2; ++mi)
-#pragma unroll
-        for (int r = 0; r < 16; ++r) acc[mi][r] = 0.f;
-
-    __shared__ float rowc[3][QBM];
-    if constexpr (MODE == 0 || MODE == 3 || MODE == 4) {
-        if (tid < QBM) {
-            const int row = i0 + tid;
-            const bool ok = row < g.M;
-            rowc[0][tid] = ((MODE == 0 || MODE == 4) && ok) ? g.dw[row] : 1.0f;
-            rowc[1][tid] = (MODE == 0 && ok) ? g.rw[row] : 0.0f;
-            rowc[2][tid] = (ok && g.bias != nullptr) ? (row < g.M1 ? g.bias[row] : g.bias2[row - g.M1]) : 0.0f;
-        }
-    }
 
     constexpr int NLOADS = (MODE == 0) ? 2 : (WMODE == 1) ? 3 : 6;
     const int a_row = tid >> 1, a_k = (tid & 1) * 16;
@@ -338,6 +329,42 @@
     }
     q_wait<WMODE, 0>(stA);
     q_wait<WMODE, 0>(stB);
+}
+
+template <int MODE, int GP = 3, bool IMP = false>
+__global__ __launch_bounds__(256, 2) void k_qgemm(QGemmArgs g) {
+    static_assert(!IMP || MODE == 1 || MODE == 3 || MODE == 4, "implicit convolution: float B operands");
+    static_assert(MODE == 0 || MODE == 1 || MODE == 3 || MODE == 4, "unknown q-GEMM mode");
+    static_assert(GP == 3 || (GP == 2 && MODE != 0 && MODE != 4), "two gradient pieces: dgrad only");
+    constexpr int SMEM = QCfg<MODE, GP, IMP>::SMEM;
+    __shared__ __attribute__((aligned(16))) unsigned char smem[SMEM];
+    const int tid = threadIdx.x, lane = tid & 63;
+    const int wave = __builtin_amdgcn_readfirstlane(tid >> 6);
+    const int wm = wave >> 1, wn = wave & 1;
+    const int lr = lane & 31, lh = lane >> 5;
+    int panel, mt;
+    if (!xcd_tile(g.tiles_n * g.batches, g.tiles_m, panel, mt)) return;
+    const int b = panel / g.tiles_n;
+    const int i0 = mt * QBM, j0 = (panel % g.tiles_n) * QBN;
+
+    f32x16 acc[2];
+#pragma unroll
+    for (int mi = 0; mi < 2; ++mi)
+#pragma unroll
+        for (int r = 0; r < 16; ++r) acc[mi][r] = 0.f;
+
+    __shared__ float rowc[3][QBM];
+    if constexpr (MODE == 0 || MODE == 3 || MODE == 4) {
+        if (tid < QBM) {
+            const int row = i0 + tid;
+            const bool ok = row < g.M;
+            rowc[0][tid] = ((MODE == 0 || MODE == 4) && ok) ? g.dw[row] : 1.0f;
+            rowc[1][tid] = (MODE == 0 && ok) ? g.rw[row] : 0.0f;
+            rowc[2][tid] = (ok && g.bias != nullptr) ? (row < g.M1 ? g.bias[row] : g.bias2[row - g.M1]) : 0.0f;
+        }
+    }
+
+    qgemm_main_loop<MODE, GP, IMP>(g, smem, b, i0, j0, acc);
 
     float dx = 0.f, mnx = 0.f;
     if constexpr (MODE == 0) {
@@ -345,7 +372,8 @@
         dx = (hi - lo) / 255.0f;
         mnx = lo;
     }
-    float* Cb = g.C + (int64_t)b * g.sCb;
+    const bool has_z = g.C != nullptr;
+    float* Cb = has_z ? g.C + (int64_t)b * g.sCb : nullptr;
     float* C2b = (g.C2 != nullptr) ? g.C2 + (int64_t)b * g.sC2b : nullptr;
     __shared__ uint32_t Qt[(MODE == 0) ? 4 : 1][32][8];
     const bool quant = (MODE == 0) && g.Q1 != nullptr;
@@ -388,8 +416,7 @@
                 const float S = acc[mi][r];
                 float v = S;
                 if constexpr (MODE == 0) {
-                    v = rowc[0][rb] * (dx * S + mnx * rowc[1][rb]);
-                    if (has_bias) v = v + rowc[2][rb];
+                    v = qfwd_z(S, rowc[0][rb], rowc[1][rb], rowc[2][rb], has_bias, dx, mnx);
                 } else if constexpr (MODE == 3) {
                     if (has_bias) v = S + rowc[2][rb];
                 } else if constexpr (MODE == 4) {
@@ -410,7 +437,7 @@
                         t.x += r.x; t.y += r.y; t.z += r.z; t.w += r.w;
                     }
                 }
-                if (row < g.M && col < g.N) {
+                if (has_z && row < g.M && col < g.N) {
                     const bool first = decltype(PER_ROW)::value ? row < g.M1 : tfirst;
                     const int64_t ldc = first ? g.ldc : g.ldc2;
                     float* dst = (first ? Cb + (int64_t)row * ldc : C2b + (int64_t)(row - g.M1) * ldc) + col;
@@ -494,6 +521,176 @@
                 }
             }
         }
+    }
+}
+
+
+struct RzArgs {
+    const uint8_t* xc; int64_t ld_xc;
+    const float* g; int64_t ld_g;
+    float* gz; int64_t ld_gz;
+    const float *gamma, *beta, *mean_rstd;
+    const double* ws;
+    const float *qmin_y, *qmax_y;
+    const float *qmin_p, *qmax_p;
+    int act; const float* slope;
+    double* gacc; float* gbias;
+    float *ggamma, *gbeta;
+    int C, M, run, nruns;
+};
+#ifndef FQSS_RZ_RUN
+#define FQSS_RZ_RUN 4
+#endif
+constexpr int RZ_RUN = FQSS_RZ_RUN;
+
+__global__ __launch_bounds__(256, 2) void k_gnq_bwd_apply_rz(QGemmArgs g, RzArgs r) {
+    __shared__ __attribute__((aligned(16))) unsigned char smem[QCfg<0, 3, false>::SMEM];
+    __shared__ float rowc[3][QBM];
+    __shared__ float rsc[2][QBM];
+    __shared__ float sbias[2][QBM];
+    __shared__ double cred[2 * 4];
+    __shared__ float c23[2];
+    __shared__ float predf[4 * 4];
+    const int tid = threadIdx.x, lane = tid & 63;
+    const int wave = __builtin_amdgcn_readfirstlane(tid >> 6);
+    const int wm = wave >> 1, wn = wave & 1;
+    int panel, mt;
+    if (!xcd_tile(g.batches * r.nruns, g.tiles_m, panel, mt)) return;
+    const int b = panel / r.nruns, ri = panel - b * r.nruns;
+    const int t0 = ri * r.run, t1 = min(t0 + r.run, g.tiles_n);
+    const int i0 = mt * QBM;
+    const int C = r.C, M = r.M;
+    const bool det_on = det_preload();
+    const float mean = r.mean_rstd[2 * b], rstd = r.mean_rstd[2 * b + 1];
+    if (tid < QBM) {
+        const int row = i0 + tid;
+        const bool ok = row < C;
+        rowc[0][tid] = ok ? g.dw[row] : 1.0f;
+        rowc[1][tid] = ok ? g.rw[row] : 0.0f;
+        rowc[2][tid] = (ok && g.bias != nullptr) ? g.bias[row] : 0.0f;
+        const float scale = ok ? rstd * r.gamma[row] : 0.0f;
+        rsc[0][tid] = scale;
+        rsc[1][tid] = ok ? fmaf(-scale, mean, r.beta[row]) : 0.0f;
+        if (ok && b == 0 && ri == 0) {
+            double gg = 0.0, gb = 0.0;
+            for (int bb = 0; bb < g.batches; ++bb) {
+                const double ds = r.ws[2 * ((int64_t)bb * C + row)], db = r.ws[2 * ((int64_t)bb * C + row) + 1];
+                gg += (ds - db * (double)r.mean_rstd[2 * bb]) * (double)r.mean_rstd[2 * bb + 1];
+                gb += db;
+            }
+            r.ggamma[row] += (float)gg;
+            r.gbeta[row] += (float)gb;
+        }
+    }
+    float c2, c3;
+    {
+        double sv[2] = {0.0, 0.0};
+        for (int cc = tid; cc < C; cc += 256) {
+            const double gmm = (double)r.gamma[cc];
+            sv[0] += gmm * r.ws[2 * ((int64_t)b * C + cc)];
+            sv[1] += gmm * r.ws[2 * ((int64_t)b * C + cc) + 1];
+        }
+        block_sum<double, 2>(sv, cred);
+        if (tid == 0) {
+            double c2d, c3d;
+            gn_coef_from_sums(sv, mean, rstd, C, M, c2d, c3d);
+            c23[0] = (float)c2d;
+            c23[1] = (float)c3d;
+        }
+        __syncthreads();
+        c2 = c23[0];
+        c3 = c23[1];
+    }
+    const QRange rp = load_qrange(r.qmin_p, r.qmax_p), ry = load_qrange(r.qmin_y, r.qmax_y);
+    const float pslope = (r.act == FQSS_ACT_PRELU) ? *r.slope : 0.0f;
+    const float dx = (*g.qmax_x - *g.qmin_x) / 255.0f, mnx = *g.qmin_x;
+    const bool has_bias = g.bias != nullptr;
+    float p_du = 0.f, p_out = 0.f, p_slope = 0.f;
+    float pb[2][4];
+#pragma unroll
+    for (int mi = 0; mi < 2; ++mi)
+#pragma unroll
+        for (int ps = 0; ps < 4; ++ps) pb[mi][ps] = 0.f;
+    const uint8_t* xcb = r.xc + (int64_t)b * C * r.ld_xc;
+    const float* gb_ = r.g + (int64_t)b * C * r.ld_g;
+    float* gzb = r.gz + (int64_t)b * C * r.ld_gz;
+    for (int t = t0; t < t1; ++t) {
+        const int j0 = t * QBN;
+        int lane = tid & 63;
+        asm volatile("" : "+v"(lane));
+        const int lr = lane & 31, lh = lane >> 5, c4 = (lane & 7) * 4;
+        float(*Tt)[LDT] = reinterpret_cast<float(*)[LDT]>(smem + wave * 32 * LDT * 4);
+        const int col = j0 + wn * 32 + c4;
+        f32x16 acc[2];
+#pragma unroll
+        for (int mi = 0; mi < 2; ++mi)
+#pragma unroll
+            for (int e = 0; e < 16; ++e) acc[mi][e] = 0.f;
+        qgemm_main_loop<0, 3, false>(g, smem, b, i0, j0, acc);
+        __syncthreads();
+#pragma unroll
+        for (int mi = 0; mi < 2; ++mi) {
+            const int rowt = i0 + wm * 64 + mi * 32;
+            float4 gq[4];
+            unsigned int xq[4];
+#pragma unroll
+            for (int ps = 0; ps < 4; ++ps) {
+                const int row = rowt + ps * 8 + (lane >> 3);
+                gq[ps] = make_float4(0.f, 0.f, 0.f, 0.f);
+                xq[ps] = 0u;
+                if (row < C && col < M) {
+                    gq[ps] = *reinterpret_cast<const float4*>(gb_ + (int64_t)row * r.ld_g + col);
+                    xq[ps] = *reinterpret_cast<const unsigned int*>(xcb + (int64_t)row * r.ld_xc + col);
+                }
+            }
+#pragma unroll
+            for (int e = 0; e < 16; ++e) {
+                const int rl = (e & 3) + 8 * (e >> 2) + 4 * lh;
+                const int rb = wm * 64 + mi * 32 + rl;
+                Tt[rl][lr] = qfwd_z(acc[mi][e], rowc[0][rb], rowc[1][rb], rowc[2][rb], has_bias, dx, mnx);
+            }
+#pragma unroll
+            for (int ps = 0; ps < 4; ++ps) {
+                const int rl = ps * 8 + (lane >> 3);
+                const int rb = wm * 64 + mi * 32 + rl;
+                const int row = rowt + rl;
+                const float4 zt = *reinterpret_cast<const float4*>(&Tt[rl][c4]);
+                const float zv[4] = {zt.x, zt.y, zt.z, zt.w};
+                const float gv[4] = {gq[ps].x, gq[ps].y, gq[ps].z, gq[ps].w};
+                const float scale = rsc[0][rb], shift = rsc[1][rb];
+                float xv[4], o[4];
+#pragma unroll
+                for (int e = 0; e < 4; ++e) xv[e] = dec((xq[ps] >> (8 * e)) & 255u, rp);
+#pragma unroll
+                for (int e = 0; e < 4; ++e)
+                    o[e] = gnq_bwd_elem<true>(xv[e], gv[e], zv[e], row < C && col + e < M, scale, shift, c2, c3, ry, rp, r.act, pslope,
+                                              p_du, p_out, p_slope, pb[mi][ps]);
+                if (row < C && col < M) store16(gzb + (int64_t)row * r.ld_gz + col, make_float4(o[0], o[1], o[2], o[3]));
+            }
+        }
+    }
+#pragma unroll
+    for (int mi = 0; mi < 2; ++mi)
+#pragma unroll
+        for (int ps = 0; ps < 4; ++ps) {
+            float v = pb[mi][ps];
+            v += __shfl_xor(v, 1);
+            v += __shfl_xor(v, 2);
+            v += __shfl_xor(v, 4);
+            if ((lane & 7) == 0) sbias[wn][wm * 64 + mi * 32 + ps * 8 + (lane >> 3)] = v;
+        }
+    double v[4];
+    {
+        const float pf[4] = {p_du, p_out, p_slope, 0.f};
+        block_sum_f32w<4>(pf, predf, v);
+    }
+    if (tid < QBM && i0 + tid < C && r.gbias != nullptr) grad_add(&r.gbias[i0 + tid], sbias[0][tid] + sbias[1][tid], det_on);
+    if (tid == 0) {
+        double* slot = r.gacc + 3 * (blockIdx.x % FQSS_GACC_SLOTS);
+        const double dmax = v[0] / 255.0;
+        atomicAdd(&slot[0], v[1] - dmax);
+        atomicAdd(&slot[1], dmax);
+        if (r.act == FQSS_ACT_PRELU) atomicAdd(&slot[2], v[2]);
     }
 }
 
@@ -976,11 +1173,14 @@
                         const QpwQuant* qq = nullptr) {
     if (B == 0 || M == 0) return FQSS_OK;
     const int Co = Co1 + Co2;
-    FQSS_REQUIRE(xc && wi && dw && rw && qmin_x && qmax_x && z1 && (Co2 == 0 || z2), "null tensor");
-    FQSS_REQUIRE(B >= 0 && Ci > 0 && Co1 > 0 && Co2 >= 0 && M >= 0 && ld_xc >= M && ld_z1 >= M && (Co2 == 0 || ld_z2 >= M), "bad shape");
+    const bool no_z = z1 == nullptr && qq != nullptr;
+    FQSS_REQUIRE(!no_z || z2 == nullptr, "z1 == NULL: z2 must be NULL too");
+    FQSS_REQUIRE(xc && wi && dw && rw && qmin_x && qmax_x && (z1 || no_z) && (Co2 == 0 || z2 || no_z), "null tensor");
+    FQSS_REQUIRE(B >= 0 && Ci > 0 && Co1 > 0 && Co2 >= 0 && M >= 0 && ld_xc >= M && (no_z || (ld_z1 >= M && (Co2 == 0 || ld_z2 >= M))),
+                 "bad shape");
     FQSS_REQUIRE(Ci % 16 == 0 && Ci <= 512 && ld_xc % 16 == 0 && aligned16(xc) && aligned16(wi),
                  "q-GEMM needs Ci % 16 == 0, Ci <= 512 (exact fp32 integer sum) and 16-B aligned code rows");
-    FQSS_REQUIRE(aligned16(z1) && ld_z1 % 4 == 0 && (Co2 == 0 || (aligned16(z2) && ld_z2 % 4 == 0)), "output rows must be 16-B aligned");
+    FQSS_REQUIRE(no_z || (aligned16(z1) && ld_z1 % 4 == 0 && (Co2 == 0 || (aligned16(z2) && ld_z2 % 4 == 0))), "output rows must be 16-B aligned");
     FQSS_REQUIRE((bias1 == nullptr) == (bias2 == nullptr) || Co2 == 0, "paired layers: both or neither with bias");
     if (qq != nullptr) FQSS_REQUIRE(Co2 == 0 || Co1 % 32 == 0, "fused quantizer of a pair needs Co1 % 32 == 0");
     QGemmArgs g{};
@@ -1056,6 +1256,37 @@
                         ld_z2, stream, &qq);
 }
 
+extern "C" int fqss_gnq_bwd_apply_rz(const uint8_t* xc, const float* qmin_x, const float* qmax_x, const float* g, const float* gamma,
+                                     const float* beta, const float* mean_rstd, float* gz, float* ggamma, float* gbeta, int B, int C, int M,
+                                     int64_t ld_xc, int64_t ld_g, int64_t ld_gz, const float* qmin, const float* qmax, const double* ws,
+                                     const uint8_t* pxc, int Ci, int64_t ld_pxc, const float* pqmin_x, const float* pqmax_x,
+                                     const int8_t* wi, const float* dw, const float* rw, const float* pbias, int pact, const float* pslope,
+                                     double* pgacc, float* pgbias, fqss_stream_t stream) {
+    if (B == 0 || M == 0) return FQSS_OK;
+    FQSS_REQUIRE(xc && qmin_x && qmax_x && g && gamma && beta && mean_rstd && gz && ggamma && gbeta && qmin && qmax && ws, "null pointer");
+    FQSS_REQUIRE(pxc && pqmin_x && pqmax_x && wi && dw && rw && pgacc, "producer: null pointer");
+    FQSS_REQUIRE(pact != FQSS_ACT_PRELU || pslope, "PReLU needs a slope");
+    FQSS_REQUIRE(B > 0 && C > 0 && M > 0 && Ci > 0, "bad shape");
+    FQSS_REQUIRE(ld_xc % 16 == 0 && ld_xc >= M && aligned16(xc), "code rows must be 16-B aligned");
+    FQSS_REQUIRE(aligned16(g) && ld_g % 4 == 0 && ld_g >= ((M + 3) & ~3), "gradient rows must be 16-B aligned");
+    FQSS_REQUIRE(aligned16(gz) && ld_gz % 4 == 0 && ld_gz >= ((M + 3) & ~3), "gz rows must be 16-B aligned");
+    FQSS_REQUIRE(Ci % 16 == 0 && Ci <= 512 && ld_pxc % 16 == 0 && ld_pxc >= M && aligned16(pxc) && aligned16(wi),
+                 "producer q-GEMM needs Ci % 16 == 0, Ci <= 512 and 16-B aligned code rows");
+    QGemmArgs a{};
+    a.A = wi; a.B = pxc; a.M = C; a.N = M; a.K = Ci;
+    a.lda = Ci; a.ldb = ld_pxc; a.sBb = (int64_t)Ci * ld_pxc;
+    a.M1 = C; a.K1 = Ci; a.dw = dw; a.rw = rw; a.bias = pbias; a.qmin_x = pqmin_x; a.qmax_x = pqmax_x; a.ksplit = 1; a.kchunk = Ci;
+    a.tiles_n = (int)cdiv(M, QBN); a.tiles_m = (int)cdiv(C, QBM); a.batches = B;
+    RzArgs r{};
+    r.xc = xc; r.ld_xc = ld_xc; r.g = g; r.ld_g = ld_g; r.gz = gz; r.ld_gz = ld_gz;
+    r.gamma = gamma; r.beta = beta; r.mean_rstd = mean_rstd; r.ws = ws;
+    r.qmin_y = qmin; r.qmax_y = qmax; r.qmin_p = qmin_x; r.qmax_p = qmax_x;
+    r.act = pact; r.slope = pslope; r.gacc = pgacc; r.gbias = pgbias; r.ggamma = ggamma; r.gbeta = gbeta;
+    r.C = C; r.M = M; r.run = RZ_RUN; r.nruns = (int)cdiv(a.tiles_n, RZ_RUN);
+    hipLaunchKernelGGL(k_gnq_bwd_apply_rz, dim3(xcd_grid((int64_t)r.nruns * B, a.tiles_m)), dim3(256), 0, (hipStream_t)stream, a, r);
+    return launch_status("fqss_gnq_bwd_apply_rz");
+}
+
 static int qpw_bwd_x_impl(const char* who, const float* gz1, const float* gz2, const int8_t* wiT, const float* dw, float* gx, int B,
                           int Ci, int Co1, int Co2, int M, int64_t ld_gz1, int64_t ld_gz2, int64_t ld_gx, fqss_stream_t stream,
                           const float* addend = nullptr, int64_t ld_add = 0) {
diff --git a/fqss_amd/kernels.py b/fqss_amd/kernels.py
--- a/fqss_amd/kernels.py
+++ b/fqss_amd/kernels.py
@@ -428,15 +428,18 @@
     return z1, z2
 
 
-def qpw_fwdq(xc, wc, bias1, bias2, qmin_x, qmax_x, Co1, act, slope, r1, r2=None, stats=None, adds=None):
+def qpw_fwdq(xc, wc, bias1, bias2, qmin_x, qmax_x, Co1, act, slope, r1, r2=None, stats=None, adds=None, want_z=True):
     B, Ci, M = xc.shape
     rm = rowmat(xc)
     Co2 = wc.Co - Co1
     assert rm is not None and Ci == wc.Ci and Co2 >= 0 and (Co2 == 0) == (r2 is None)
-    z1, yc1 = empty_act((B, Co1, M), xc.device), empty_codes((B, Co1, M), xc.device)
+    z1 = empty_act((B, Co1, M), xc.device) if want_z else None
+    yc1 = empty_codes((B, Co1, M), xc.device)
     z2 = yc2 = None
     if Co2:
-        z2, yc2 = empty_act((B, Co2, M), xc.device), empty_codes((B, Co2, M), xc.device)
+        z2, yc2 = (empty_act((B, Co2, M), xc.device) if want_z else None), empty_codes((B, Co2, M), xc.device)
+    ldz1 = rowmat(z1)[2] if z1 is not None else 0
+    ldz2 = rowmat(z2)[2] if z2 is not None else 0
     if adds is not None and any(a is not None for a in adds):
         assert act == ACT_NONE and stats is None and (adds[1] is None or Co2)
         sums, recs = [], []
@@ -452,7 +455,7 @@
             sums.append(sc); recs.append(r)
         _lib.call("fqss_qpw_fwdq_add", _p(xc), _p(wc.idx), _p(wc.dw), _p(wc.rw), _p(bias1), _p(bias2), _p(qmin_x), _p(qmax_x), _p(z1), _p(z2),
                   _p(r1[0]), _p(r1[1]), _p(r2[0]) if r2 else None, _p(r2[1]) if r2 else None, _p(yc1), _p(yc2),
-                  B, Ci, Co1, Co2, M, rm[2], rowmat(z1)[2], rowmat(z2)[2] if Co2 else 0, rowmat(yc1)[2], rowmat(yc2)[2] if Co2 else 0,
+                  B, Ci, Co1, Co2, M, rm[2], ldz1, ldz2, rowmat(yc1)[2], rowmat(yc2)[2] if Co2 else 0,
                   _ref(recs[0]) if recs[0] is not None else None, _ref(recs[1]) if recs[1] is not None else None, _stream())
         return ((z1, z2, yc1, yc2) if Co2 else (z1, yc1)) + (tuple(sums),)
     if DESC_ABI:
@@ -467,7 +470,7 @@
         return (z1, z2, yc1, yc2) if Co2 else (z1, yc1)
     _lib.call("fqss_qpw_fwdq", _p(xc), _p(wc.idx), _p(wc.dw), _p(wc.rw), _p(bias1), _p(bias2), _p(qmin_x), _p(qmax_x), _p(z1), _p(z2),
               act, _p(slope), _p(r1[0]), _p(r1[1]), _p(r2[0]) if r2 else None, _p(r2[1]) if r2 else None, _p(yc1), _p(yc2),
-              B, Ci, Co1, Co2, M, rm[2], rowmat(z1)[2], rowmat(z2)[2] if Co2 else 0, rowmat(yc1)[2], rowmat(yc2)[2] if Co2 else 0,
+              B, Ci, Co1, Co2, M, rm[2], ldz1, ldz2, rowmat(yc1)[2], rowmat(yc2)[2] if Co2 else 0,
               _p(stats.ws) if stats is not None else None, _stream())
     return (z1, z2, yc1, yc2) if Co2 else (z1, yc1)
 
@@ -631,6 +634,20 @@
               _p(gbeta), B, C, M, ld_xc, ld_g, rowmat(gx)[2], _p(qmin), _p(qmax), _p(ws), _p(pz), ld_pz, pact, _p(pslope), _p(pgacc),
               _p(pgbias), _stream())
     return gx
+
+
+def gnq_bwd_apply_rz(xc, qmin_x, qmax_x, g, gamma, beta, mean_rstd, qmin, qmax, ws, ggamma, gbeta, producer, recipe):
+    B, C, M, ld_xc = _codes3(xc)
+    g, ld_g = _aligned_grad(g)
+    gz = empty_act((B, C, M), xc.device)
+    _, pact, pslope, pgacc, pgbias = producer
+    pxc, pqmin_x, pqmax_x, wc, pbias = recipe
+    _, Ci, _, ld_pxc = _codes3(pxc)
+    assert tuple(pxc.shape) == (B, Ci, M) and wc.Co == C and wc.Ci == Ci
+    _lib.call("fqss_gnq_bwd_apply_rz", _p(xc), _p(qmin_x), _p(qmax_x), _p(g), _p(gamma), _p(beta), _p(mean_rstd), _p(gz), _p(ggamma),
+              _p(gbeta), B, C, M, ld_xc, ld_g, rowmat(gz)[2], _p(qmin), _p(qmax), _p(ws), _p(pxc), Ci, ld_pxc, _p(pqmin_x), _p(pqmax_x),
+              _p(wc.idx), _p(wc.dw), _p(wc.rw), _p(pbias), pact, _p(pslope), _p(pgacc), _p(pgbias), _stream())
+    return gz
 
 
 def dwq_fwd(xc, qmin_x, qmax_x, w, bias, dil, pad, act, slope, qmin, qmax, write_out, stats=None):
diff --git a/fqss_amd/ops.py b/fqss_amd/ops.py
--- a/fqss_amd/ops.py
+++ b/fqss_amd/ops.py
@@ -55,11 +55,18 @@
 
 
 class _Producer:
-    __slots__ = ("z", "act", "slope", "slope_param", "q", "bias_param", "bias", "fused")
-
-    def __init__(self, z, act, slope, slope_param, q, bias_param, bias):
+    __slots__ = ("z", "act", "slope", "slope_param", "q", "bias_param", "bias", "fused", "rz")
+
+    def __init__(self, z, act, slope, slope_param, q, bias_param, bias, rz=None):
         self.z, self.act, self.slope, self.slope_param, self.q, self.bias_param, self.bias = z, act, slope, slope_param, q, bias_param, bias
         self.fused = False
+        self.rz = rz
+
+    def pz(self):
+        if self.z is None:
+            xc, lo, hi, wc, bias = self.rz
+            return K.qpw_fwd(xc, wc, bias, lo, hi)
+        return self.z
 
 
 class _GnHand:
@@ -102,11 +109,13 @@
 FUSE_MULQ_PROD = os.environ.get("FQSS_FUSE_MULQ_PROD", "1") != "0"
 
 
-def _producer_args(pr):
+def _producer_args(pr, rebuild=True):
     if pr is None or pr.q.gacc is None:
         return None
     pgb, direct = (None, True) if pr.bias is None else _grad_buf(pr.bias_param, pr.bias)
-    return (pr.z, pr.act, pr.slope, pr.q.gacc, pgb) if direct else None
+    if not direct:
+        return None
+    return (pr.pz() if rebuild else pr.z, pr.act, pr.slope, pr.q.gacc, pgb)
 
 
 def codes_of(x):
@@ -458,12 +467,20 @@
         ctx.wc = wc if (L.kind == "pw" and wc is not None and K.q_eligible(w.shape[1], w.shape[0])) else None
         ctx.plain = (q.qmode == Q_BYPASS and act == ACT_NONE)
         ctx.xq_tr = xq if (L.kind == "convtr" and xq is not None and bias is None and K.ola_convtr_ok(w, L.stride)) else None
+        want_prod = ((FUSE_GN and NEXT_IS_GROUPNORM) or (FUSE_MULQ_PROD and NEXT_TAKES_PRODUCER and act in (ACT_NONE, ACT_RELU, ACT_PRELU))) \
+            and DEFER is not None and q.qmode == Q_QUANT and not ctx.plain and q.owner is not None \
+            and getattr(q.owner, "_fqss_deferred", False)
+        rz = None
+        z_shape = None
         if ctx.xq is not None and ctx.wc is not None and _fuse_out_quant(q):
             q.stats = K.new_stats("qpw", x.shape[0], ctx.wc.Co, x.shape[-1], x.device) if (FUSE_STATS and NEXT_IS_GROUPNORM) else None
+            if want_prod and FUSE_GN and NEXT_IS_GROUPNORM:
+                rz = (ctx.xq.idx, ctx.xq.qmin, ctx.xq.qmax, ctx.wc, bias)
             z, q.idx = K.qpw_fwdq(ctx.xq.idx, ctx.wc, bias, None, ctx.xq.qmin, ctx.xq.qmax, ctx.wc.Co, act, slope, (q.qmin, q.qmax),
-                                  stats=q.stats)
+                                  stats=q.stats, want_z=rz is None)
+            z_shape = tuple(q.idx.shape)
             q.carrier = True
-            out = _carrier(K.empty_act(tuple(z.shape), z.device))
+            out = _carrier(K.empty_act(z_shape, q.idx.device))
         else:
             if ctx.xq is not None and ctx.wc is not None:
                 z = K.qpw_fwd(ctx.xq.idx, ctx.wc, bias, ctx.xq.qmin, ctx.xq.qmax)
@@ -473,17 +490,15 @@
                 z = _lin_fwd(L, x, w, bias)
             out = z if ctx.plain else _epilogue_fwd(z, act, slope, q)
         ctx.prod = None
-        if ((FUSE_GN and NEXT_IS_GROUPNORM) or (FUSE_MULQ_PROD and NEXT_TAKES_PRODUCER and act in (ACT_NONE, ACT_RELU, ACT_PRELU))) \
-                and DEFER is not None and q.qmode == Q_QUANT and not ctx.plain and q.owner is not None \
-                and getattr(q.owner, "_fqss_deferred", False):
-            ctx.prod = q.prod = _Producer(z, act, slope, L.slope_param, q, L.b_param, bias)
+        if want_prod:
+            ctx.prod = q.prod = _Producer(z, act, slope, L.slope_param, q, L.b_param, bias, rz=rz)
         ctx.x_shape = x.shape
         ctx.fork = getattr(x, "_fqss_fork", None) if ((ctx.wc is not None and ctx.wc.idxT is not None) or L.kind == "convtr") else None
         ctx.save_for_backward(None if ((ctx.xq is not None and ctx.wc is not None) or ctx.xq_tr is not None) else x, w,
                               None if ctx.plain else z, slope)
         ctx.L, ctx.act, ctx.q, ctx.has_bias = L, act, q, bias is not None
         ctx.bias_like = bias
-        ctx.C = z.shape[1]
+        ctx.C = z_shape[1] if z_shape is not None else z.shape[1]
         return out
 
     @staticmethod
@@ -501,6 +516,8 @@
             K.chan_sum(g, gb)
             gz, g_slope, g_min, g_max, g_bias = g, None, None, None, (None if gb_direct else gb)
         else:
+            if z is None and not ctx.plain:
+                z = ctx.prod.pz()
             gz, g_slope, g_min, g_max, g_bias = _epilogue_bwd(
                 g if ctx.plain else z, g, act, slope, L.slope_param, q, bias_param=L.b_param,
                 bias_like=ctx.bias_like if ctx.has_bias else None, C=ctx.C)
@@ -641,13 +658,19 @@
             gamma, beta, mean_rstd, xc, xmin, xmax, qmin, qmax = ctx.saved_tensors
             gg, gg_direct = _grad_buf(ctx.gp, gamma)
             gb, gb_direct = _grad_buf(ctx.bp, gamma)
-            producer = _producer_args(ctx.prod) if ctx.needs_input_grad[0] else None
+            producer = _producer_args(ctx.prod, rebuild=False) if ctx.needs_input_grad[0] else None
             if producer is not None:
                 ctx.prod.fused = True
             hi, ho = ctx.hand_in, ctx.hand_out
+            rz = producer is not None and producer[0] is None and ho is not None and ho.rec is not None
+            if producer is not None and producer[0] is None and not rz:
+                producer = (ctx.prod.pz(),) + producer[1:]
             if hi is not None and producer is None and gg_direct and gb_direct and ctx.needs_input_grad[0]:
                 gx, ws = K.gnq_bwd_rows(xc, xmin, xmax, g, gamma, beta, mean_rstd, qmin, qmax, q.gacc)
                 hi.rec = dict(gamma=gamma, beta=beta, mean_rstd=mean_rstd, ws=ws, qmin=qmin, qmax=qmax, ggamma=gg, gbeta=gb)
+            elif rz:
+                gx = K.gnq_bwd_apply_rz(xc, xmin, xmax, g, gamma, beta, mean_rstd, qmin, qmax, ho.rec["ws"], gg, gb, producer, ctx.prod.rz)
+                ho.rec = None
             elif ho is not None and ho.rec is not None:
                 gx = K.gnq_bwd_apply(xc, xmin, xmax, g, gamma, beta, mean_rstd, qmin, qmax, ho.rec["ws"], gg, gb, producer=producer)
                 ho.rec = None
diff --git a/include/fqss.h b/include/fqss.h
--- a/include/fqss.h
+++ b/include/fqss.h
@@ -261,6 +261,12 @@
                        int64_t ld_xc, int64_t ld_g, int64_t ld_gx, const float* qmin, const float* qmax, const double* ws,
                        const float* pz, int64_t ld_pz, int pact, const float* pslope, double* pgacc, float* pgbias,
                        fqss_stream_t stream);
+int fqss_gnq_bwd_apply_rz(const uint8_t* xc, const float* qmin_x, const float* qmax_x, const float* g, const float* gamma,
+                          const float* beta, const float* mean_rstd, float* gz, float* ggamma, float* gbeta, int B, int C, int M,
+                          int64_t ld_xc, int64_t ld_g, int64_t ld_gz, const float* qmin, const float* qmax, const double* ws,
+                          const uint8_t* pxc, int Ci, int64_t ld_pxc, const float* pqmin_x, const float* pqmax_x,
+                          const int8_t* wi, const float* dw, const float* rw, const float* pbias, int pact, const float* pslope,
+                          double* pgacc, float* pgbias, fqss_stream_t stream);
 int fqss_dwq_bwd_gn(const uint8_t* xc, const float* qmin_x, const float* qmax_x, const float* w, const float* bias,
                     const float* g, float* gx, float* gw, int B, int C, int M, int K, int dil, int pad, int64_t ld_xc,
                     int64_t ld_g, int64_t ld_gx, int act, const float* slope, const float* qmin, const float* qmax,
```

Measured after the change: 612.7, median of 2. About the same (-0.2%).
